# Samsung/iac

Hardware: AMD Instinct MI355X
Metric: Msamples/s rendered (3rd-order HOA->binaural, 48 kHz) (higher is better)
Workload: dtype f32

## Files before the change

iac_amd/__init__.py:

```python
from .hipabi import (
    FMT_F32,
    FMT_S16,
    FMT_S24,
    FMT_S32,
    KIND_DMX,
    KIND_FIR,
    KIND_H2M,
    KIND_M2M,
    PROJ_AUTO,
    PROJ_EXACT,
    PROJ_MFMA,
    SS,
    Batch,
    BatchConfig,
    DemixConfig,
    DemixFrame,
    DemixState,
    DmxFrame,
    DmxState,
    FANOUT_MAX,
    FanoutReport,
    RenderArgs,
    Resampler,
    StreamGains,
    StreamState,
    stream_gains,
    dmx_matrix,
    fir_matrix,
    IamfHipError,
    LpcmLayout,
    LpcmInput,
    Matrix,
    build,
    get_h2m_matrix,
    get_m2m_matrix,
    layout_channels,
    lib,
    lib_path,
    lpcm_unpack,
    render_fanout,
    render_fanout_lpcm,
    render_fanout_range,
    ROUTE,
    RouteRow,
    route_instances,
    route_instances_ext,
    route_reset,
    route_tally,
    route_tally_ext,
)
```

iac_amd/csrc/iamf_render.hip:

```cpp
#include <hip/hip_runtime.h>

#include <math.h>
#include <stdint.h>
#include <atomic>
#include <stdio.h>
#include <stdlib.h>
#include <string.h>

#include <new>
#include <type_traits>
#include <vector>

#include "../../include/iamf_hip.h"

#define IAMF_FFT_HOST_TABLES

#include "render_entry.hpp"

namespace {

#include "render_common.hpp"
#include "render_downmix.hpp"
#include "render_fir.hpp"
#include "render_fir16.hpp"
#include "render_fir_fft.hpp"
#include "render_fast.hpp"
#include "render_fir_launch.hpp"
#include "render_fanout.hpp"
#include "render_generic.hpp"
#include "render_nolim.hpp"
#include "render_wide.hpp"
#include "render_lfe.hpp"
#include "stream_state.hpp"

__global__ __launch_bounds__(256) void restride_kernel(const uint8_t *src, int64_t src_stream_stride, uint8_t *dst,
                                                       int64_t dst_stream_stride, int n, int ch, int sc, int bps, int stream0) {
  const int s = blockIdx.y + stream0;
  const int64_t p = (int64_t)blockIdx.x * 256 + threadIdx.x;
  const int64_t n_out = (int64_t)n * sc + (ch > sc ? ch - sc : 0);
  if (p >= n_out) return;
  const int c0 = (int)(p % sc);
  const int64_t i = p / sc;
  const uint8_t *from = nullptr;
  for (int k = (ch - 1 - c0) / sc; k >= 0 && ch > c0; --k) {
    const int64_t ii = i - k;
    if (ii >= 0 && ii < n) {
      from = src + (int64_t)s * src_stream_stride + (ii * ch + c0 + (int64_t)sc * k) * bps;
      break;
    }
  }
  if (!from && p >= (int64_t)n * sc) return;
  uint8_t *to = dst + (int64_t)s * dst_stream_stride + p * bps;
  for (int b = 0; b < bps; ++b) to[b] = from ? from[b] : 0;
}


#define HIPCHK(expr)                                                                   \
  do {                                                                                 \
    hipError_t _e = (expr);                                                            \
    if (_e != hipSuccess) {                                                            \
      fprintf(stderr, "iamf_hip: %s failed: %s (%s:%d)\n", #expr, hipGetErrorString(_e), \
              __FILE__, __LINE__);                                                     \
      return IAMF_HIP_ERR_DEVICE;                                                      \
    }                                                                                  \
  } while (0)

struct TableEntry {
  uint32_t kind, in_id, out_id;
  int32_t channels, lfe1, lfe2, m, n;
  uint32_t offset;
};

extern "C" const uint8_t _binary_rdr_tables_bin_start[];
extern "C" const uint8_t _binary_rdr_tables_bin_end[];
extern "C" const uint8_t _binary_rdr_tables_tv_bin_start[];
extern "C" const uint8_t _binary_rdr_tables_tv_bin_end[];

struct Tables {
  int n = 0;
  const TableEntry *ents = nullptr;
  const float *data = nullptr;
  bool ok = false;
  explicit Tables(bool tv) {
    const uint8_t *b = tv ? _binary_rdr_tables_tv_bin_start : _binary_rdr_tables_bin_start;
    const size_t sz = tv ? (size_t)(_binary_rdr_tables_tv_bin_end - _binary_rdr_tables_tv_bin_start)
                         : (size_t)(_binary_rdr_tables_bin_end - _binary_rdr_tables_bin_start);
    if (sz < 12 || memcmp(b, "IARDRTB1", 8) != 0) return;
    uint32_t cnt;
    memcpy(&cnt, b + 8, 4);
    n = (int)cnt;
    ents = reinterpret_cast<const TableEntry *>(b + 12);
    data = reinterpret_cast<const float *>(b + 12 + sizeof(TableEntry) * cnt);
    ok = true;
  }
};

const Tables &tables(bool tv) {
  static Tables t(false), t_tv(true);
  return tv ? t_tv : t;
}

int find_matrix(int kind, int in_id, int out_id, iamf_hip_matrix *out, bool tv = false) {
  const Tables &t = tables(tv);
  if (!t.ok || !out) return -1;
  for (int i = 0; i < t.n; ++i) {
    const TableEntry &e = t.ents[i];
    if ((int)e.kind == kind && (int)e.in_id == in_id && (int)e.out_id == out_id) {
      out->kind = kind;
      out->in_id = in_id;
      out->out_id = out_id;
      out->channels = e.channels;
      out->lfe1 = e.lfe1;
      out->lfe2 = e.lfe2;
      out->m = e.m;
      out->n = e.n;
      out->mat = t.data + e.offset;
      return 0;
    }
  }
  return -1;
}

float ease(float x) {
  if (1.0 < x) return 1.0f;
  if (x < 0) return 0.0f;
  return 1.0f - powf(x - 1, 2.0);
}

}

struct iamf_hip_batch {
  iamf_hip_batch_config cfg;
  int device = 0;
  hipEvent_t done = nullptr;
  bool rendered = false;
  int m = 0, n_feeds = 0;
  int32_t src_feed[kMaxOut];
  uint32_t nz_mask[6] = {0, 0, 0, 0, 0, 0};
  int sparse = 0;
  int32_t *d_src_feed = nullptr;
  float thr = 0.f;
  int n_atk = 0, n_end = 0;
  std::vector<int64_t> spos;
  std::vector<uint8_t> sflushed;
  bool any_rendered = false;
  bool lp_scale_ok = false;
  float *d_matrix = nullptr, *d_gains = nullptr, *d_ctab = nullptr, *d_ring_y = nullptr,
        *d_ring_pm = nullptr;
  LimState *d_lim = nullptr;
  std::vector<float> h_gains;
  bool has2 = false;
  int m2 = 0;
  float *d_matrix2 = nullptr, *d_gains2 = nullptr;
  int32_t *d_src_feed2 = nullptr, *d_dmx_tab = nullptr;
  bool dmx = false;
  int dmx_n_in = 0, dmx_n_out = 0;
  float *d_pre = nullptr;
  int pre_l = 0;
  std::vector<float> h_fm;
  float *d_matrix_pre = nullptr;
  uint32_t nz_mask_pre[6] = {0, 0, 0, 0, 0, 0};
  int sparse_pre = 0;
  bool demix = false;
  int demix_steps = 0, demix_skip = 0, demix_layout = 0, demix_gmask = 0, demix_w4 = 0;
  int32_t *d_demix_tab = nullptr;
  float *d_demix_ftab = nullptr;
  bool fir = false;
  int fir_taps = 0;
  float *d_fir_hist[2] = {nullptr, nullptr};
  void *d_fir_h16 = nullptr;
  float *d_fir_pq = nullptr, *d_fir_tw = nullptr;
  float *d_fir_zero = nullptr;
  float *d_fir_pre[2] = {nullptr, nullptr};
  size_t fir_pre_bytes = 0;
  float *d_fir_y = nullptr;
  size_t fir_y_floats = 0;
  float *d_lp_in = nullptr;
  size_t lp_in_floats = 0;
  float *d_fir_id = nullptr;
  int32_t *d_fir_id_feed = nullptr;
  float fir_inv_scale = 1.f;
  int fir_cur = 0;
  bool lfe = false;
  float lfe_a1 = 0.f, lfe_a2 = 0.f, lfe_a3 = 0.f, lfe_b1 = 0.f, lfe_b2 = 0.f;
  double lfe_div = 0.0;
  float *d_lfe_state = nullptr, *d_lfe_next = nullptr, *d_lfe_u = nullptr;
  bool lfe_shared = false;
  size_t lfe_u_floats = 0;
  uint8_t *d_nat = nullptr;
  size_t nat_bytes = 0;
  uint8_t *d_dump = nullptr;
};

namespace {

bool on_batch_device(const iamf_hip_batch *b) {
  int dev = -1;
  return hipGetDevice(&dev) == hipSuccess && dev == b->device;
}

int quiesce(iamf_hip_batch *b) {
  if (b->rendered) HIPCHK(hipEventSynchronize(b->done));
  return IAMF_HIP_OK;
}

int reset_state(iamf_hip_batch *b) {
  const int ns = b->cfg.n_streams;
  std::vector<LimState> init((size_t)ns);
  for (auto &l : init) {
    l.g = 1.0f;
    l.gs = -1.0f;
    l.ge = -1.0f;
    l.n = b->n_end;
  }
  HIPCHK(hipMemcpy(b->d_lim, init.data(), sizeof(LimState) * ns, hipMemcpyHostToDevice));
  HIPCHK(hipMemset(b->d_ring_y, 0, sizeof(float) * (size_t)ns * b->cfg.out_channels * kSave));
  HIPCHK(hipMemset(b->d_ring_pm, 0, sizeof(float) * (size_t)ns * kSave));
  if (b->fir) {
    const size_t hb = sizeof(float) * (size_t)ns * b->m * 256;
    HIPCHK(hipMemset(b->d_fir_hist[0], 0, hb));
    HIPCHK(hipMemset(b->d_fir_hist[1], 0, hb));
    for (float *q : b->d_fir_pre)
      if (q) HIPCHK(hipMemset(q, 0, b->fir_pre_bytes));
  }
  if (b->lfe && !b->lfe_shared) {
    HIPCHK(hipMemset(b->d_lfe_state, 0, sizeof(float) * 4 * (size_t)ns));
    HIPCHK(hipMemset(b->d_lfe_next, 0, sizeof(float) * 2 * (size_t)ns));
  }
  b->spos.assign((size_t)ns, 0);
  b->sflushed.assign((size_t)ns, 0);
  b->any_rendered = false;
  return IAMF_HIP_OK;
}

template <int M>
void launch_m(const RenderParams &p, dim3 grid, size_t lds_bytes, hipStream_t st) {
  hipLaunchKernelGGL(render_kernel<M>, grid, dim3(kChunk), lds_bytes, st, p);
}

template <int M>
void launch_nolim_m(const RenderParams &p, hipStream_t st) {
  const int bytes = p.out_format == IAMF_HIP_FMT_S16 ? 2 : (p.out_format == IAMF_HIP_FMT_S24 ? 3 : 4);
  dim3 grid((unsigned)p.n_launch, (unsigned)((p.total + kNlChunk - 1) / kNlChunk));
  hipLaunchKernelGGL(render_nolim_kernel<M>, grid, dim3(256), (size_t)kNlChunk * p.out_ch * bytes, st, p);
}

template <int M, int OC>
void launch_fast_mc(const RenderParams &p, bool mixing, dim3 grid, hipStream_t st) {
  const size_t lds = sizeof(float) * (size_t)fast_lds_floats(OC, M);
  if (mixing) launch_big_lds<&render_fast_kernel<M, OC, 0, false, true>, 80 * 1024>(grid, dim3(256), lds, st, p);
  else launch_big_lds<&render_fast_kernel<M, OC>, 80 * 1024>(grid, dim3(256), lds, st, p);
}
template <int M>
void launch_fast_m(const RenderParams &p, bool mixing, dim3 grid, hipStream_t st) {
  if (p.out_ch == 1) launch_fast_mc<M, 1>(p, mixing, grid, st);
  else launch_fast_mc<M, 2>(p, mixing, grid, st);
}

template <int M, int OC>
void launch_fast_down_mc(const RenderParams &p, dim3 grid, hipStream_t st) {
  const size_t lds = sizeof(float) * (size_t)fast_lds_floats(OC, M);
  launch_big_lds<&render_fast_kernel<M, OC, 0, true>, 80 * 1024>(grid, dim3(256), lds, st, p);
}

template <int M>
void launch_wide_m(const RenderParams &p, dim3 grid, hipStream_t st) {
  const size_t lds = sizeof(float) * (size_t)wide_lds_floats(p.out_ch, M);
  if (p.use_mfma) launch_big_lds<&render_wide_kernel<M, true>, 80 * 1024>(grid, dim3(256), lds, st, p);
  else launch_big_lds<&render_wide_kernel<M, false>, 80 * 1024>(grid, dim3(256), lds, st, p);
}

int launch(const RenderParams &p, int m, size_t lds_bytes, hipStream_t st) {
  const Route r = pick_route(p, m);
  const dim3 grid((unsigned)p.n_launch);
  bool launched = false;
  switch (r.family) {
    case Family::Refused: return r.err;
    case Family::Lpcm: launched = iamf_hip_fast_lpcm_launch(&p, m, r.variant, st); break;
    case Family::FirSplit: {
      if (!dispatch(FirHomeM{}, m, [&](auto M) { launch_fft_m<M.value>(p, st); }) && !iamf_hip_fir_m2b_launch_fft(&p, m, st))
        return IAMF_HIP_ERR_INTERNAL;
      HIPCHK(hipGetLastError());
      RenderParams q = p;
      q.in = p.fir_y;
      q.in_stream_stride = 2 * (int64_t)p.total;
      q.in_frame_stride = 2 * (int64_t)p.total;
      q.frame_size = p.total;
      q.matrix = p.fir_id_matrix;
      q.src_feed = p.fir_id_feed;
      q.n_feeds = 2;
      q.fir_taps = 0;
      q.fir_hist = q.fir_hist_next = nullptr;
      launch_fast_m<2>(q, false, grid, st);
      launched = true;
      break;
    }
    case Family::FirFused:
      launched = dispatch(FirHomeM{}, m, [&](auto M) { launch_fir_m<M.value>(p, r.variant, st); }) ||
                 iamf_hip_fir_m2b_launch(&p, m, r.variant, st);
      break;
    case Family::FastDown:
      launched = dispatch(FastDownMC{}, mc(m, p.out_ch), [&](auto V) { launch_fast_down_mc<mc_m(V.value), mc_c(V.value)>(p, grid, st); });
      break;
    case Family::Wide4Lfe: launched = iamf_hip_wide4_lfe_launch(&p, m, st); break;
    case Family::Wide4Mix: launched = iamf_hip_wide4_mix_launch(&p, m, st); break;
    case Family::Wide4:
    case Family::Wide4Demix:
    case Family::Wide4Down: launched = iamf_hip_wide4_launch(&p, m, st); break;
    case Family::Nolim: launched = dispatch(NolimM{}, m, [&](auto M) { launch_nolim_m<M.value>(p, st); }); break;
    case Family::Fast: launched = dispatch(FastM{}, m, [&](auto M) { launch_fast_m<M.value>(p, r.variant != 0, grid, st); }); break;
    case Family::Wide: launched = dispatch(WideM{}, m, [&](auto M) { launch_wide_m<M.value>(p, grid, st); }); break;
    case Family::Generic: launched = dispatch(GenericM{}, m, [&](auto M) { launch_m<M.value>(p, grid, lds_bytes, st); }); break;
  }
  if (!launched) return IAMF_HIP_ERR_INTERNAL;
  HIPCHK(hipGetLastError());
  const RouteKey k = route_key(r, p, m);
  iamf_hip_route_count(k.family, k.variant, k.m, k.c, k.k);
  if (r.family == Family::FirSplit) iamf_hip_route_count(IAMF_HIP_ROUTE_FAST, 0, 2, 2, 0);
  return IAMF_HIP_OK;
}

const int kLayoutCount[9] = {1, 2, 6, 8, 10, 8, 10, 12, 6};
const int kLayoutCh[9][12] = {
    {kChMono},
    {kChL2, kChR2},
    {kChL7, kChR7, kChC, kChLFE, kChSL5, kChSR5},
    {kChL7, kChR7, kChC, kChLFE, kChSL5, kChSR5, kChHL, kChHR},
    {kChL7, kChR7, kChC, kChLFE, kChSL5, kChSR5, kChHFL, kChHFR, kChHBL, kChHBR},
    {kChL7, kChR7, kChC, kChLFE, kChSL7, kChSR7, kChBL7, kChBR7},
    {kChL7, kChR7, kChC, kChLFE, kChSL7, kChSR7, kChBL7, kChBR7, kChHL, kChHR},
    {kChL7, kChR7, kChC, kChLFE, kChSL7, kChSR7, kChBL7, kChBR7, kChHFL, kChHFR, kChHBL, kChHBR},
    {kChL3, kChR3, kChC, kChLFE, kChTL, kChTR},
};
const int kLayoutSurround[9] = {1, 2, 5, 5, 5, 7, 7, 7, 3};
const int kLayoutTop[9] = {0, 0, 0, 2, 4, 0, 2, 4, 2};

struct LpcmIn {
  const uint8_t *raw;
  int64_t stream_stride, frame_stride;
  int32_t off[16];
};
constexpr int kNotFused = INT32_MIN;

int lfe_prepass(iamf_hip_batch *b, const float *d_in, int64_t in_stream_stride, int64_t in_frame_stride, int ltotal,
                hipStream_t st, int s0, int cnt, int *t4_out) {
  const int ns = b->cfg.n_streams, nb = (ns + 63) / 64, t4 = (ltotal + 3) / 4;
  const size_t need_u = (size_t)nb * t4 * 64 * 4;
  if (need_u > b->lfe_u_floats) {
    HIPCHK(hipStreamSynchronize(st));
    (void)hipFree(b->d_lfe_u);
    b->d_lfe_u = nullptr;
    b->lfe_u_floats = 0;
    HIPCHK(hipMalloc(&b->d_lfe_u, sizeof(float) * need_u));
    b->lfe_u_floats = need_u;
  }
  LfeParams lp;
  memset(&lp, 0, sizeof(lp));
  lp.in = d_in;
  lp.in_stream_stride = in_stream_stride;
  lp.in_frame_stride = in_frame_stride;
  lp.pre_matrix = b->d_pre;
  lp.pre_l = b->pre_l;
  lp.pre_m = b->m;
  lp.frame_size = b->cfg.frame_size;
  lp.n_streams = ns;
  lp.total = ltotal;
  lp.t4 = t4;
  lp.a1 = b->lfe_a1; lp.a2 = b->lfe_a2; lp.a3 = b->lfe_a3; lp.b1 = b->lfe_b1; lp.b2 = b->lfe_b2;
  lp.state = b->d_lfe_state;
  lp.state_next = b->d_lfe_next;
  lp.u_t = reinterpret_cast<float4 *>(b->d_lfe_u);
  lp.s_first = s0;
  lp.s_count = cnt;
  hipLaunchKernelGGL(lfe_ff_kernel, dim3((unsigned)((t4 + kLfeTileQ - 1) / kLfeTileQ), (unsigned)nb), dim3(256), 0, st, lp);
  hipLaunchKernelGGL(lfe_chain_kernel, dim3((unsigned)nb), dim3(64), 0, st, lp);
  HIPCHK(hipGetLastError());
  *t4_out = t4;
  return IAMF_HIP_OK;
}

struct PreparedCall {
  RenderParams p;
  iamf_hip_render_args a;
  int m_eff;
  size_t lds;
  bool restride;
  int sc, bps;
  int64_t pos;
  int total, s0, cnt;
};

int render_prepare(iamf_hip_batch *b, const iamf_hip_render_args &a, int total, int s0, int cnt, const LpcmIn *lp, PreparedCall &pc) {
  if (!on_batch_device(b)) return IAMF_HIP_ERR_INVALID_STATE;
  if (lp && (b->fir || b->lfe || b->d_pre || b->demix || b->dmx || b->has2 || a.d_element_ramp || a.d_element2_ramp ||
             a.d_output_ramp || !b->lp_scale_ok || getenv("IAMF_HIP_LPCM_UNFUSED")))
    return kNotFused;
  if (s0 < 0 || cnt <= 0 || s0 + cnt > b->cfg.n_streams) return IAMF_HIP_ERR_BAD_ARG;
  if (a.lfe_pre_samples < 0 || a.lfe_post_samples < 0 ||
      ((a.lfe_pre_samples || a.lfe_post_samples) &&
       (a.n_frames != 1 || (int64_t)a.lfe_pre_samples + total + a.lfe_post_samples > b->cfg.frame_size)))
    return IAMF_HIP_ERR_BAD_ARG;
  const int64_t pos = b->spos[(size_t)s0];
  for (int i = s0; i < s0 + cnt; ++i)
    if (b->spos[(size_t)i] != pos || b->sflushed[(size_t)i]) return IAMF_HIP_ERR_INVALID_STATE;
  const bool whole = s0 == 0 && cnt == b->cfg.n_streams;
  if (!whole && b->fir) return IAMF_HIP_ERR_UNIMPLEMENTED;
  RenderParams &p = pc.p;
  memset(&p, 0, sizeof(p));
  p.stream0 = s0;
  p.n_launch = cnt;
  p.in = a.d_in;
  p.in_stream_stride = a.in_stream_stride;
  p.in_frame_stride = a.in_frame_stride;
  p.pcm = static_cast<uint8_t *>(a.d_pcm);
  p.pcm_stream_stride = a.pcm_stream_stride_bytes;
  p.matrix = b->d_matrix;
  p.gains = b->d_gains;
  p.ctab = b->d_ctab;
  p.lim = b->d_lim;
  p.ring_y = b->d_ring_y;
  p.ring_pm = b->d_ring_pm;
  p.pos0 = pos;
  p.total = total;
  p.frame_size = b->cfg.frame_size;
  p.n_streams = b->cfg.n_streams;
  p.n_feeds = b->n_feeds;
  p.out_ch = b->cfg.out_channels;
  p.og_ch = (b->cfg.out_gain_channels > 0 && b->cfg.out_gain_channels < b->cfg.out_channels) ? b->cfg.out_gain_channels : b->cfg.out_channels;
  p.out_format = b->cfg.out_format;
  p.limiter_on = b->cfg.limiter_enable ? 1 : 0;
  p.loudness_on = b->cfg.loudness_enable ? 1 : 0;
  bool tolerance = false;
  {
    const int proj = b->cfg.projection;
    const char *env = getenv("IAMF_HIP_PROJECTION");
    bool mf = proj == IAMF_HIP_PROJ_MFMA || (proj == IAMF_HIP_PROJ_AUTO && b->cfg.matrix.kind == IAMF_HIP_KIND_H2M);
    if (env && !strcmp(env, "exact")) mf = false;
    if (env && !strcmp(env, "mfma")) mf = true;
    p.use_mfma = (mf && b->n_feeds <= 32) ? 1 : 0;
    tolerance = mf;
  }
  p.n_atk = b->n_atk;
  p.n_end = b->n_end;
  p.thr = b->thr;
  p.src_feed = b->d_src_feed;
  p.dump = b->d_dump;
  for (int g = 0; g < 6; ++g) p.nz_mask[g] = b->nz_mask[g];
  p.sparse = getenv("IAMF_HIP_DENSE") ? 0 : b->sparse;
  if (b->has2 && a.d_in2) {
    p.in2 = a.d_in2;
    p.in2_stream_stride = a.in2_stream_stride;
    p.in2_frame_stride = a.in2_frame_stride;
    p.matrix2 = b->d_matrix2;
    p.src_feed2 = b->d_src_feed2;
    p.gains2 = b->d_gains2;
    p.m2 = b->m2;
  }
  p.elem_ramp = a.d_element_ramp;
  p.elem2_ramp = a.d_element2_ramp;
  p.out_ramp = a.d_output_ramp;
  p.ramp_stream_stride = a.ramp_stream_stride;
  if (b->dmx) {
    p.dmx_on = 1;
    p.dmx_frames = a.d_in ? a.d_dmx_frames : nullptr;
    p.dmx_n_in = b->dmx_n_in;
    p.dmx_n_out = b->dmx_n_out;
    p.dmx_tab = b->d_dmx_tab;
    p.dmx_in_layout = b->cfg.matrix.in_id;
    p.dmx_out_layout = b->cfg.matrix.out_id;
  }
  int m_eff = b->m;
  if (b->d_pre && a.d_in) {
    const int l = b->pre_l;
    if (tolerance && b->d_matrix_pre && FastM::has(l) && !p.in2) {
      p.matrix = b->d_matrix_pre;
      for (int g = 0; g < 6; ++g) p.nz_mask[g] = b->nz_mask_pre[g];
      p.sparse = getenv("IAMF_HIP_DENSE") ? 0 : b->sparse_pre;
      m_eff = l;
    } else {
      p.pre_matrix = b->d_pre;
      p.pre_l = b->pre_l;
    }
  }
  if (b->demix && a.d_in) {
    p.demix_on = 1;
    p.demix_steps = b->demix_steps;
    p.demix_skip = b->demix_skip;
    p.demix_tab = b->d_demix_tab;
    p.demix_ftab = b->d_demix_ftab;
    p.demix_frames = a.d_demix_frames;
    p.demix_i0 = a.n_frames == 1 ? a.demix_sample0 : 0;
    p.demix_layout = b->demix_layout;
    p.demix_gmask = b->demix_gmask;
    p.demix_w4 = b->demix_w4;
  }
  if (lp) {
    p.lpcm = lp->raw;
    p.lpcm_stream_stride = lp->stream_stride;
    p.lpcm_frame_stride = lp->frame_stride;
    for (int m = 0; m < 16; ++m) p.lpcm_off[m] = lp->off[m];
    if (pick_route(p, m_eff).family != Family::Lpcm) return kNotFused;
  }
  if (b->fir) {
    p.fir_taps = b->fir_taps;
    p.fir_hist = b->d_fir_hist[b->fir_cur];
    p.fir_hist_next = b->d_fir_hist[b->fir_cur ^ 1];
    p.fir_h16 = b->d_fir_h16;
    p.fir_inv_scale = b->fir_inv_scale;
    p.fir_pq = b->d_fir_pq;
    p.fir_tw = b->d_fir_tw;
    p.fir_zero = b->d_fir_zero;
    p.fir_pre = b->d_fir_pre[b->fir_cur];
    p.fir_pre_next = b->d_fir_pre[b->fir_cur ^ 1];
    if (a.d_in && b->d_fir_pq && (b->cfg.frame_size & 63) == 0 && !getenv("IAMF_HIP_FIR_FUSED") && !getenv("IAMF_HIP_FIR_F16") &&
        !getenv("IAMF_HIP_FIR_F32")) {
      const size_t need = (size_t)b->cfg.n_streams * 2 * (size_t)total;
      if (need > b->fir_y_floats) {
        HIPCHK(hipStreamSynchronize(static_cast<hipStream_t>(a.stream)));
        (void)hipFree(b->d_fir_y);
        b->d_fir_y = nullptr;
        b->fir_y_floats = 0;
        HIPCHK(hipMalloc(&b->d_fir_y, sizeof(float) * need));
        b->fir_y_floats = need;
      }
      p.fir_y = b->d_fir_y;
      p.fir_id_matrix = b->d_fir_id;
      p.fir_id_feed = b->d_fir_id_feed;
    }
  }
  if (b->lfe && a.d_in && total > 0) {
    const int lpre = a.lfe_pre_samples, lpost = a.lfe_post_samples;
    int t4 = 0;
    const int rc = lfe_prepass(b, a.d_in - lpre, a.in_stream_stride, a.in_frame_stride, lpre + total + lpost,
                               static_cast<hipStream_t>(a.stream), s0, cnt, &t4);
    if (rc) return rc;
    p.lfe = b->d_lfe_u;
    p.lfe_t4 = t4;
    p.lfe_k0 = lpre;
    p.lfe_div = b->lfe_div;
    for (int c = 0; c < b->cfg.out_channels && c < 32; ++c)
      if (b->src_feed[c] == -2) p.lfe_mask |= 1 << c;
  }
  const size_t lds = sizeof(float) * ((size_t)(p.out_ch + 2) * kRing + 3 * kChunk + kHead + 4 +
                                      ((b->dmx || b->demix) ? (size_t)kChCount * kChunk : 0));
  const int sc = b->cfg.pcm_stride_channels;
  const bool restride = sc > 0 && sc != p.out_ch;
  const int bps = iamf_hip_format_bytes(p.out_format);
  if (restride) {
    const size_t per_stream = (size_t)(total > kDelay ? total : kDelay) * p.out_ch * bps;
    const size_t need = per_stream * (size_t)p.n_streams;
    if (need > b->nat_bytes) {
      HIPCHK(hipStreamSynchronize(static_cast<hipStream_t>(a.stream)));
      (void)hipFree(b->d_nat);
      b->d_nat = nullptr;
      b->nat_bytes = 0;
      HIPCHK(hipMalloc(&b->d_nat, need));
      b->nat_bytes = need;
    }
    p.pcm = b->d_nat;
    p.pcm_stream_stride = (int64_t)per_stream;
  }
  pc.a = a;
  pc.m_eff = m_eff;
  pc.lds = lds;
  pc.restride = restride;
  pc.sc = sc;
  pc.bps = bps;
  pc.pos = pos;
  pc.total = total;
  pc.s0 = s0;
  pc.cnt = cnt;
  return IAMF_HIP_OK;
}

int render_launch(const PreparedCall &pc) {
  return launch(pc.p, pc.m_eff, pc.lds, static_cast<hipStream_t>(pc.a.stream));
}

int render_commit(iamf_hip_batch *b, const PreparedCall &pc) {
  const RenderParams &p = pc.p;
  const iamf_hip_render_args &a = pc.a;
  const bool restride = pc.restride;
  const int sc = pc.sc, bps = pc.bps, total = pc.total, s0 = pc.s0, cnt = pc.cnt;
  const int64_t pos = pc.pos;
  if (b->fir && p.in) b->fir_cur ^= 1;
  const int64_t before = p.limiter_on ? (pos > kDelay ? pos - kDelay : 0) : pos;
  for (int i = s0; i < s0 + cnt; ++i) b->spos[(size_t)i] = pos + total;
  b->any_rendered = true;
  const int64_t after = p.limiter_on ? (pos + total > kDelay ? pos + total - kDelay : 0) : pos + total;
  const int n_emit = (int)(after - before);
  if (restride && n_emit > 0) {
    const int64_t n_out = (int64_t)n_emit * sc + (p.out_ch > sc ? p.out_ch - sc : 0);
    hipLaunchKernelGGL(restride_kernel, dim3((unsigned)((n_out + 255) / 256), (unsigned)cnt), dim3(256), 0,
                       static_cast<hipStream_t>(a.stream), b->d_nat, p.pcm_stream_stride,
                       static_cast<uint8_t *>(a.d_pcm), a.pcm_stream_stride_bytes, n_emit, p.out_ch, sc, bps, s0);
    HIPCHK(hipGetLastError());
  }
  HIPCHK(hipEventRecord(b->done, static_cast<hipStream_t>(a.stream)));
  b->rendered = true;
  return n_emit;
}

int render_call(iamf_hip_batch *b, const iamf_hip_render_args &a, int total, int s0, int cnt, const LpcmIn *lp = nullptr) {
  PreparedCall pc;
  int r = render_prepare(b, a, total, s0, cnt, lp, pc);
  if (r != IAMF_HIP_OK) return r;
  r = render_launch(pc);
  if (r != IAMF_HIP_OK) return r;
  return render_commit(b, pc);
}

void build_feed_map(const iamf_hip_matrix &mx, int out_channels, std::vector<float> &fm, int32_t *src_feed) {
  for (int i = 0; i < kMaxOut; ++i) src_feed[i] = -1;
  for (int i = 0; i < mx.n; ++i) {
    int d = i;
    if (mx.kind == IAMF_HIP_KIND_H2M && (mx.lfe1 >= 0 || mx.lfe2 >= 0)) {
      if (mx.lfe1 >= 0 && mx.lfe1 <= i) ++d;
      if (mx.lfe2 >= 0 && mx.lfe2 <= i) ++d;
    }
    if (d < out_channels) src_feed[d] = i;
  }
  if (mx.kind == IAMF_HIP_KIND_H2M) {
    if (mx.lfe1 >= 0 && mx.lfe1 < out_channels) src_feed[mx.lfe1] = -1;
    if (mx.lfe2 >= 0 && mx.lfe2 < out_channels) src_feed[mx.lfe2] = -1;
  }
  fm.assign((size_t)mx.m * mx.n, 0.f);
  for (int f = 0; f < mx.n; ++f)
    for (int k = 0; k < mx.m; ++k)
      fm[(size_t)f * mx.m + k] = mx.kind == IAMF_HIP_KIND_H2M ? mx.mat[f * mx.m + k] : mx.mat[k * mx.n + f];
}

}

extern "C" {

int iamf_hip_get_h2m_matrix(int order, int out_id, iamf_hip_matrix *out) {
  return find_matrix(IAMF_HIP_KIND_H2M, order, out_id, out);
}

int iamf_hip_get_m2m_matrix(int in_id, int out_id, iamf_hip_matrix *out) {
  return find_matrix(IAMF_HIP_KIND_M2M, in_id, out_id, out);
}

int iamf_hip_get_m2m_matrix_variant(int variant, int in_id, int out_id, iamf_hip_matrix *out) {
  if (variant != IAMF_HIP_VARIANT_DEFAULT && variant != IAMF_HIP_VARIANT_SAMSUNG_TV) return -1;
  return find_matrix(IAMF_HIP_KIND_M2M, in_id, out_id, out, variant == IAMF_HIP_VARIANT_SAMSUNG_TV);
}

int iamf_hip_layout_channels(int out_id) {
  switch (out_id) {
    case IAMF_HIP_SS_A: return 2;
    case IAMF_HIP_SS_B: return 6;
    case IAMF_HIP_SS_C: return 8;
    case IAMF_HIP_SS_D: return 10;
    case IAMF_HIP_SS_E: return 11;
    case IAMF_HIP_SS_F: return 12;
    case IAMF_HIP_SS_G: return 14;
    case IAMF_HIP_SS_H: return 24;
    case IAMF_HIP_SS_I: return 8;
    case IAMF_HIP_SS_J: return 12;
    case IAMF_HIP_L_712: return 10;
    case IAMF_HIP_L_312: return 6;
    case IAMF_HIP_L_MONO: return 1;
    case IAMF_HIP_L_BINAURAL: return 2;
    default: return 0;
  }
}

int iamf_hip_format_bytes(int f) {
  switch (f) {
    case IAMF_HIP_FMT_S16: return 2;
    case IAMF_HIP_FMT_S24: return 3;
    case IAMF_HIP_FMT_S32: return 4;
    case IAMF_HIP_FMT_F32: return 4;
    default: return 0;
  }
}

const char *iamf_hip_version(void) { return "iamf_hip 0.1 (gfx950, HIP)"; }

int iamf_hip_batch_create(const iamf_hip_batch_config *cfg, iamf_hip_batch **out) {
  if (!cfg || !out) return IAMF_HIP_ERR_BAD_ARG;
  *out = nullptr;
  iamf_hip_matrix mx = cfg->matrix;
  const bool dmx = mx.kind == IAMF_HIP_KIND_DMX;
  const bool fir = mx.kind == IAMF_HIP_KIND_FIR;
  if (fir && (cfg->fir_taps < 1 || cfg->fir_taps > 256 || mx.n != 2 || cfg->out_channels != 2 ||
              !cfg->limiter_enable ||
              (!FirHomeM::has(mx.m) && !FirM2bM::has(mx.m))))
    return IAMF_HIP_ERR_BAD_ARG;
  if (dmx) {
    if (!iamf_hip_dmx_valid(mx.in_id, mx.out_id)) return IAMF_HIP_ERR_BAD_ARG;
    mx.m = kLayoutCount[mx.in_id];
    mx.n = kLayoutCount[mx.out_id];
  }
  if (cfg->n_streams <= 0 || cfg->frame_size <= 0 || cfg->sample_rate <= 0 || (!dmx && !mx.mat) ||
      mx.m <= 0 || mx.m > kMaxIn || mx.n <= 0 || mx.n > kMaxOut || cfg->out_channels <= 0 ||
      cfg->out_channels > kMaxOut || !iamf_hip_format_bytes(cfg->out_format) || cfg->projection < 0 ||
      cfg->projection > IAMF_HIP_PROJ_MFMA || (dmx && cfg->out_channels != mx.n) || cfg->pcm_stride_channels < 0 || cfg->out_gain_channels < 0 ||
      cfg->pcm_stride_channels > 64)
    return IAMF_HIP_ERR_BAD_ARG;
  int ndev = 0;
  HIPCHK(hipGetDeviceCount(&ndev));
  if (ndev <= 0) return IAMF_HIP_ERR_DEVICE;

  iamf_hip_batch *b = new (std::nothrow) iamf_hip_batch();
  if (!b) return IAMF_HIP_ERR_ALLOC_FAIL;
  b->cfg = *cfg;
  if (hipGetDevice(&b->device) != hipSuccess) {
    delete b;
    return IAMF_HIP_ERR_DEVICE;
  }
  b->m = mx.m;
  b->n_feeds = mx.n;
  b->dmx = dmx;

  b->fir = fir;
  b->fir_taps = fir ? cfg->fir_taps : 0;
  std::vector<float> fm(1, 0.f);
  int32_t dmx_tab[24];
  memset(dmx_tab, 0, sizeof(dmx_tab));
  if (dmx) {
    for (int i = 0; i < kMaxOut; ++i) b->src_feed[i] = -1;
    b->dmx_n_in = mx.m;
    b->dmx_n_out = mx.n;
    for (int i = 0; i < mx.m; ++i) dmx_tab[i] = kLayoutCh[mx.in_id][i];
    for (int i = 0; i < mx.n; ++i) dmx_tab[12 + i] = kLayoutCh[mx.out_id][i];
  } else if (fir) {
    for (int i = 0; i < kMaxOut; ++i) b->src_feed[i] = -1;
    fm.assign(mx.mat, mx.mat + (size_t)2 * mx.m * cfg->fir_taps);
  } else {
    build_feed_map(mx, cfg->out_channels, fm, b->src_feed);
    b->lp_scale_ok = true;
    for (float w : fm)
      if (w != 0.f && !(fabsf(w) >= 0x1p-100f && fabsf(w) <= 0x1p100f)) b->lp_scale_ok = false;
    if (cfg->lfe_hoa && mx.kind == IAMF_HIP_KIND_H2M && (mx.lfe1 >= 0 || mx.lfe2 >= 0)) {
      const float sample_rate = (float)cfg->sample_rate, cutoff_freq = 120;
      const float delta_time = 1 / sample_rate + 1.0e-10;
      const float c = 1.0f / (float)tanf(M_PI * cutoff_freq * delta_time);
      b->lfe = true;
      b->lfe_a1 = 1.0f / (1.0f + c + c * c);
      b->lfe_a2 = 2.0f * b->lfe_a1;
      b->lfe_a3 = b->lfe_a1;
      b->lfe_b1 = 2.0f * (1.0f - c * c) * b->lfe_a1;
      b->lfe_b2 = (1.0f - c + c * c) * b->lfe_a1;
      b->lfe_div = mx.n <= 2 ? 0.0 : sqrt((double)mx.n);
      if (mx.lfe1 >= 0 && mx.lfe1 < cfg->out_channels) b->src_feed[mx.lfe1] = -2;
      if (mx.lfe2 >= 0 && mx.lfe2 < cfg->out_channels) b->src_feed[mx.lfe2] = -2;
    }
    int set = 0, all = 0;
    for (int g = 0; g < 6 && 4 * g < cfg->out_channels; ++g)
      for (int k = 0; k < mx.m && k < 32; ++k) {
        bool nz = false;
        for (int c = 4 * g; c < 4 * g + 4 && c < cfg->out_channels; ++c)
          if (b->src_feed[c] >= 0 && fm[(size_t)b->src_feed[c] * mx.m + k] != 0.f) nz = true;
        ++all;
        if (nz) {
          ++set;
          b->nz_mask[g] |= 1u << k;
        }
      }
    b->sparse = 2 * set < all ? 1 : 0;
    b->h_fm = fm;
  }

  const float atk = 0.001f, rel = 0.200f;
  b->thr = (float)pow(10, cfg->limiter_threshold_db / 20);
  const float inc = (float)1 / (float)cfg->sample_rate;
  std::vector<float> T;
  T.push_back(0.0f);
  while (T.back() < rel + atk && T.size() < (1u << 22)) T.push_back(T.back() + inc);
  b->n_end = (int)T.size() - 1;
  b->n_atk = 0;
  while (b->n_atk < b->n_end && T[b->n_atk] < atk) ++b->n_atk;
  std::vector<float> ctab((size_t)b->n_end + 1, 1.0f);
  for (int k = 1; k <= b->n_end; ++k)
    ctab[k] = (k - 1) < b->n_atk ? ease(T[k] / atk) : ease((T[k] - atk) / rel);

  const int ns = cfg->n_streams;
  b->h_gains.assign((size_t)3 * ns, 1.0f);
#define CREATE_CHK(expr)                       \
  do {                                         \
    if ((expr) != hipSuccess) {                \
      iamf_hip_batch_destroy(b);               \
      return IAMF_HIP_ERR_DEVICE;              \
    }                                          \
  } while (0)
  CREATE_CHK(hipEventCreateWithFlags(&b->done, hipEventDisableTiming));
  CREATE_CHK(hipMalloc(&b->d_matrix, sizeof(float) * fm.size()));
  CREATE_CHK(hipMalloc(&b->d_gains, sizeof(float) * 3 * ns));
  CREATE_CHK(hipMalloc(&b->d_ctab, sizeof(float) * ctab.size()));
  CREATE_CHK(hipMalloc(&b->d_lim, sizeof(LimState) * ns));
  CREATE_CHK(hipMalloc(&b->d_ring_y, sizeof(float) * (size_t)ns * cfg->out_channels * kSave));
  CREATE_CHK(hipMalloc(&b->d_ring_pm, sizeof(float) * (size_t)ns * kSave));
  if (b->lfe) {
    CREATE_CHK(hipMalloc(&b->d_lfe_state, sizeof(float) * 4 * (size_t)ns));
    CREATE_CHK(hipMalloc(&b->d_lfe_next, sizeof(float) * 2 * (size_t)ns));
  }
  CREATE_CHK(hipMalloc(&b->d_dump, (size_t)ns * 256 * 16));
  CREATE_CHK(hipMalloc(&b->d_src_feed, sizeof(int32_t) * kMaxOut));
  CREATE_CHK(hipMemcpy(b->d_src_feed, b->src_feed, sizeof(int32_t) * kMaxOut, hipMemcpyHostToDevice));
  if (fir) {
    const size_t hb = sizeof(float) * (size_t)ns * mx.m * 256;
    CREATE_CHK(hipMalloc(&b->d_fir_hist[0], hb));
    CREATE_CHK(hipMalloc(&b->d_fir_hist[1], hb));
    CREATE_CHK(hipMemset(b->d_fir_hist[0], 0, hb));
    CREATE_CHK(hipMemset(b->d_fir_hist[1], 0, hb));
    const int taps = cfg->fir_taps;
    float hmax = 0.f;
    for (size_t i = 0; i < (size_t)2 * mx.m * taps; ++i) hmax = fmaxf(hmax, fabsf(mx.mat[i]));
    if (hmax > 0.f && hmax < 1e30f) {
      int e = 0;
      (void)frexpf(hmax, &e);
      const float scale = ldexpf(1.f, 14 - e);
      std::vector<_Float16> tab((size_t)mx.m * 2 * 2 * 8 * kF16Taps, (_Float16)0.f);
      for (int ch = 0; ch < mx.m; ++ch)
        for (int ear = 0; ear < 2; ++ear)
          for (int r = 0; r < 8; ++r)
            for (int n = 0; n < kF16Taps; ++n) {
              const int k = n + r - 15;
              if (k < 0 || k >= taps) continue;
              const float v = mx.mat[((size_t)ear * mx.m + ch) * taps + k] * scale;
              const _Float16 hi = (_Float16)v;
              const _Float16 lo = (_Float16)((v - (float)hi) * 2048.f);
              const size_t at = ((((size_t)ch * 2 + ear) * 2 + 0) * 8 + r) * kF16Taps + n;
              tab[at] = hi;
              tab[at + (size_t)8 * kF16Taps] = lo;
            }
      CREATE_CHK(hipMalloc(&b->d_fir_h16, tab.size() * sizeof(_Float16)));
      CREATE_CHK(hipMemcpy(b->d_fir_h16, tab.data(), tab.size() * sizeof(_Float16), hipMemcpyHostToDevice));
      b->fir_inv_scale = 1.f / (scale * kF16InScale);
    }
    {
      std::vector<float> pq, tw;
      fft_build_tables(mx.mat, mx.m, taps, pq, tw);
      CREATE_CHK(hipMalloc(&b->d_fir_pq, pq.size() * sizeof(float)));
      CREATE_CHK(hipMemcpy(b->d_fir_pq, pq.data(), pq.size() * sizeof(float), hipMemcpyHostToDevice));
      CREATE_CHK(hipMalloc(&b->d_fir_tw, tw.size() * sizeof(float)));
      CREATE_CHK(hipMemcpy(b->d_fir_tw, tw.data(), tw.size() * sizeof(float), hipMemcpyHostToDevice));
      const size_t zf = (size_t)(mx.m > 0 ? mx.m : 1) * (size_t)(cfg->frame_size > 64 ? cfg->frame_size : 64);
      CREATE_CHK(hipMalloc(&b->d_fir_zero, zf * sizeof(float)));
      CREATE_CHK(hipMemset(b->d_fir_zero, 0, zf * sizeof(float)));
      if (cfg->frame_size >= 1024 && cfg->frame_size % 256 == 0 && mx.m % 2 == 0) {
        const int g = cfg->frame_size / 256;
        b->fir_pre_bytes = sizeof(float) * (size_t)((ns + g - 1) / g) * mx.m * cfg->frame_size;
        for (float *&q : b->d_fir_pre) {
          CREATE_CHK(hipMalloc(&q, b->fir_pre_bytes));
          CREATE_CHK(hipMemset(q, 0, b->fir_pre_bytes));
        }
      }
      const float id[4] = {1.f, 0.f, 0.f, 1.f};
      int32_t idf[kMaxOut];
      for (int i = 0; i < kMaxOut; ++i) idf[i] = i < 2 ? i : -1;
      CREATE_CHK(hipMalloc(&b->d_fir_id, sizeof(id)));
      CREATE_CHK(hipMemcpy(b->d_fir_id, id, sizeof(id), hipMemcpyHostToDevice));
      CREATE_CHK(hipMalloc(&b->d_fir_id_feed, sizeof(idf)));
      CREATE_CHK(hipMemcpy(b->d_fir_id_feed, idf, sizeof(idf), hipMemcpyHostToDevice));
    }
  }
  CREATE_CHK(hipMalloc(&b->d_dmx_tab, sizeof(dmx_tab)));
  CREATE_CHK(hipMemcpy(b->d_dmx_tab, dmx_tab, sizeof(dmx_tab), hipMemcpyHostToDevice));
  CREATE_CHK(hipMemcpy(b->d_matrix, fm.data(), sizeof(float) * fm.size(), hipMemcpyHostToDevice));
  CREATE_CHK(hipMemcpy(b->d_gains, b->h_gains.data(), sizeof(float) * 3 * ns, hipMemcpyHostToDevice));
  CREATE_CHK(hipMemcpy(b->d_ctab, ctab.data(), sizeof(float) * ctab.size(), hipMemcpyHostToDevice));
#undef CREATE_CHK
  const int r = reset_state(b);
  if (r != IAMF_HIP_OK) {
    iamf_hip_batch_destroy(b);
    return r;
  }
  *out = b;
  return IAMF_HIP_OK;
}

void iamf_hip_batch_destroy(iamf_hip_batch *b) {
  if (!b) return;
  int cur = -1;
  const bool sw = hipGetDevice(&cur) == hipSuccess && cur != b->device && hipSetDevice(b->device) == hipSuccess;
  struct Restore {
    bool on;
    int dev;
    ~Restore() {
      if (on) (void)hipSetDevice(dev);
    }
  } restore{sw, cur};
  if (b->rendered) (void)hipEventSynchronize(b->done);
  if (b->done) (void)hipEventDestroy(b->done);
  (void)hipFree(b->d_matrix_pre);
  (void)hipFree(b->d_matrix);
  (void)hipFree(b->d_gains);
  (void)hipFree(b->d_ctab);
  (void)hipFree(b->d_lim);
  (void)hipFree(b->d_ring_y);
  (void)hipFree(b->d_ring_pm);
  (void)hipFree(b->d_src_feed);
  (void)hipFree(b->d_dmx_tab);
  (void)hipFree(b->d_pre);
  (void)hipFree(b->d_demix_tab);
  (void)hipFree(b->d_demix_ftab);
  (void)hipFree(b->d_fir_hist[0]);
  (void)hipFree(b->d_fir_hist[1]);
  (void)hipFree(b->d_fir_h16);
  (void)hipFree(b->d_fir_pq);
  (void)hipFree(b->d_fir_tw);
  (void)hipFree(b->d_fir_zero);
  (void)hipFree(b->d_fir_pre[0]);
  (void)hipFree(b->d_fir_pre[1]);
  (void)hipFree(b->d_fir_y);
  (void)hipFree(b->d_lp_in);
  (void)hipFree(b->d_fir_id);
  (void)hipFree(b->d_fir_id_feed);
  if (!b->lfe_shared) {
    (void)hipFree(b->d_lfe_state);
    (void)hipFree(b->d_lfe_next);
  }
  (void)hipFree(b->d_lfe_u);
  (void)hipFree(b->d_nat);
  (void)hipFree(b->d_dump);
  (void)hipFree(b->d_matrix2);
  (void)hipFree(b->d_gains2);
  (void)hipFree(b->d_src_feed2);
  delete b;
}

int iamf_hip_batch_set_gains(iamf_hip_batch *b, const float *eg, const float *og, const float *lg) {
  if (!b) return IAMF_HIP_ERR_BAD_ARG;
  if (!on_batch_device(b)) return IAMF_HIP_ERR_INVALID_STATE;
  {
    const int q = quiesce(b);
    if (q != IAMF_HIP_OK) return q;
  }
  const int ns = b->cfg.n_streams;
  const float *rows[3] = {eg, og, lg};
  for (int k = 0; k < 3; ++k) {
    if (!rows[k]) continue;
    memcpy(&b->h_gains[(size_t)k * ns], rows[k], sizeof(float) * ns);
    HIPCHK(hipMemcpy(b->d_gains + (size_t)k * ns, rows[k], sizeof(float) * ns, hipMemcpyHostToDevice));
  }
  return IAMF_HIP_OK;
}

static int range_args_check(const iamf_hip_batch *b, const iamf_hip_render_args *a, int32_t stream0, int32_t n_streams, int64_t *total_out) {
  *total_out = 0;
  if (!b || !a || !a->d_in || !a->d_pcm || a->n_frames < 0) return IAMF_HIP_ERR_BAD_ARG;
  if (stream0 < 0 || n_streams <= 0 || stream0 + n_streams > b->cfg.n_streams) return IAMF_HIP_ERR_BAD_ARG;
  if (a->n_frames == 0) return IAMF_HIP_OK;
  if (b->has2 && !a->d_in2) return IAMF_HIP_ERR_BAD_ARG;
  if (b->dmx && !a->d_dmx_frames) return IAMF_HIP_ERR_BAD_ARG;
  if (b->demix && a->d_in && (!a->d_demix_frames || a->demix_sample0 < 0 ||
                              a->demix_sample0 + (a->n_samples ? a->n_samples : 1) > b->cfg.frame_size))
    return IAMF_HIP_ERR_BAD_ARG;
  if ((a->d_element_ramp || a->d_element2_ramp || a->d_output_ramp) &&
      a->ramp_stream_stride < (int64_t)a->n_frames * b->cfg.frame_size && b->cfg.n_streams > 1)
    return IAMF_HIP_ERR_BAD_ARG;
  int64_t total = (int64_t)a->n_frames * b->cfg.frame_size;
  if (a->n_samples > 0) {
    if (a->n_frames != 1 || a->n_samples > b->cfg.frame_size) return IAMF_HIP_ERR_BAD_ARG;
    total = a->n_samples;
  }
  if (total > INT32_MAX) return IAMF_HIP_ERR_BAD_ARG;
  const int sc = b->cfg.pcm_stride_channels > 0 ? b->cfg.pcm_stride_channels : b->cfg.out_channels;
  const int64_t need = (total * sc + (b->cfg.out_channels > sc ? b->cfg.out_channels - sc : 0)) *
                       iamf_hip_format_bytes(b->cfg.out_format);
  if (b->cfg.n_streams > 1 && a->pcm_stream_stride_bytes < need) return IAMF_HIP_ERR_BUFFER_TOO_SMALL;
  *total_out = total;
  return IAMF_HIP_OK;
}

static int render_range_impl(iamf_hip_batch *b, const iamf_hip_render_args *a, int32_t stream0, int32_t n_streams, const LpcmIn *lp) {
  int64_t total = 0;
  const int rc = range_args_check(b, a, stream0, n_streams, &total);
  if (rc != IAMF_HIP_OK || total == 0) return rc;
  return render_call(b, *a, (int)total, stream0, n_streams, lp);
}

int iamf_hip_batch_render_range(iamf_hip_batch *b, const iamf_hip_render_args *a, int32_t stream0, int32_t n_streams) {
  return render_range_impl(b, a, stream0, n_streams, nullptr);
}

int iamf_hip_batch_render_lpcm(iamf_hip_batch *b, const iamf_hip_lpcm_input *in, const iamf_hip_render_args *args) {
  if (!b) return IAMF_HIP_ERR_BAD_ARG;
  return iamf_hip_batch_render_lpcm_range(b, in, args, 0, b->cfg.n_streams);
}

static int lpcm_form_check(const iamf_hip_batch *b, const iamf_hip_lpcm_input *in, int nf, int n_samples, bool *fusable_out,
                           int *first_out, int *count_out) {
  const iamf_hip_lpcm_layout &L = in->layout;
  const int fs = b->cfg.frame_size, ch = b->d_pre ? b->pre_l : b->m;
  if (L.sample_bytes < 2 || L.sample_bytes > 4 || L.channels != ch || ch > IAMF_HIP_LPCM_MAX_CHANNELS || L.frame_size != fs ||
      (fs & 3) || in->raw_frame_stride <= 0 || in->raw_stream_stride < (int64_t)nf * in->raw_frame_stride)
    return IAMF_HIP_ERR_BAD_ARG;
  const int first = in->first_sample, count = n_samples > 0 ? n_samples : fs;
  if (first < 0 || (first > 0 && (nf != 1 || n_samples <= 0)) || first + count > fs) return IAMF_HIP_ERR_BAD_ARG;
  bool fusable = L.sample_bytes == 2 && L.little_endian && ch <= 16 && (in->raw_frame_stride & 7) == 0 &&
                 (in->raw_stream_stride & 7) == 0 && (reinterpret_cast<uintptr_t>(in->d_raw) & 15) == 0;
  for (int c = 0; c < ch; ++c) {
    if (L.src_offset[c] < 0) {
      fusable = false;
      continue;
    }
    if (L.src_step[c] < L.sample_bytes ||
        (int64_t)L.src_offset[c] + (int64_t)(fs - 1) * L.src_step[c] + L.sample_bytes > in->raw_frame_stride)
      return IAMF_HIP_ERR_BAD_ARG;
    if (L.src_step[c] != 2 || ((L.src_offset[c] + 2 * first) & 7)) fusable = false;
  }
  *fusable_out = fusable;
  *first_out = first;
  *count_out = count;
  return IAMF_HIP_OK;
}

static void lpcm_in_of(const iamf_hip_lpcm_input *in, int ch, int first, LpcmIn &lp) {
  memset(&lp, 0, sizeof(lp));
  lp.raw = static_cast<const uint8_t *>(in->d_raw);
  lp.stream_stride = in->raw_stream_stride;
  lp.frame_stride = in->raw_frame_stride;
  for (int c = 0; c < ch; ++c) lp.off[c] = in->layout.src_offset[c] + 2 * first;
}

static int lpcm_unpack_range(iamf_hip_batch *b, const iamf_hip_lpcm_input *in, int nf, int first, int count, int32_t stream0,
                             int32_t n_streams, hipStream_t st, iamf_hip_render_args &a) {
  const iamf_hip_lpcm_layout &L = in->layout;
  const int fs = b->cfg.frame_size, ch = b->d_pre ? b->pre_l : b->m, ns = b->cfg.n_streams;
  const size_t need = (size_t)ns * nf * ch * fs;
  if (need > b->lp_in_floats) {
    const int q = quiesce(b);
    if (q != IAMF_HIP_OK) return q;
    HIPCHK(hipStreamSynchronize(st));
    (void)hipFree(b->d_lp_in);
    b->d_lp_in = nullptr;
    b->lp_in_floats = 0;
    HIPCHK(hipMalloc(&b->d_lp_in, sizeof(float) * need));
    HIPCHK(hipMemset(b->d_lp_in, 0, sizeof(float) * need));
    b->lp_in_floats = need;
  }
  const int fmax = 65535 / n_streams > 0 ? 65535 / n_streams : 0;
  if (fmax == 0) return IAMF_HIP_ERR_UNIMPLEMENTED;
  const int64_t lp_stream_stride = (int64_t)nf * ch * fs;
  for (int f = 0; f < nf; f += fmax) {
    const int r = iamf_hip_lpcm_unpack_frames(
        &L, static_cast<const uint8_t *>(in->d_raw) + (int64_t)stream0 * in->raw_stream_stride + (int64_t)f * in->raw_frame_stride,
        in->raw_stream_stride, in->raw_frame_stride, nf - f < fmax ? nf - f : fmax, nullptr, 0,
        b->d_lp_in + (int64_t)stream0 * lp_stream_stride + (size_t)f * ch * fs, lp_stream_stride, (int64_t)ch * fs, n_streams, st, first,
        count);
    if (r != IAMF_HIP_OK) return r;
  }
  a.d_in = b->d_lp_in;
  a.in_stream_stride = lp_stream_stride;
  a.in_frame_stride = (int64_t)ch * fs;
  return IAMF_HIP_OK;
}

int iamf_hip_batch_render_lpcm_range(iamf_hip_batch *b, const iamf_hip_lpcm_input *in, const iamf_hip_render_args *args,
                                     int32_t stream0, int32_t n_streams) {
  if (!b || !in || !args || !in->d_raw || args->d_in || !args->d_pcm || args->n_frames < 0) return IAMF_HIP_ERR_BAD_ARG;
  if (stream0 < 0 || n_streams <= 0 || stream0 + n_streams > b->cfg.n_streams) return IAMF_HIP_ERR_BAD_ARG;
  if (!on_batch_device(b)) return IAMF_HIP_ERR_INVALID_STATE;
  if (args->n_frames == 0) return 0;
  const int ch = b->d_pre ? b->pre_l : b->m, nf = args->n_frames;
  bool fusable = false;
  int first = 0, count = 0;
  const int fc = lpcm_form_check(b, in, nf, args->n_samples, &fusable, &first, &count);
  if (fc != IAMF_HIP_OK) return fc;
  iamf_hip_render_args a = *args;
  if (fusable) {
    LpcmIn lp;
    lpcm_in_of(in, ch, first, lp);
    a.d_in = reinterpret_cast<const float *>(in->d_raw);
    a.in_stream_stride = a.in_frame_stride = 0;
    const int r = render_range_impl(b, &a, stream0, n_streams, &lp);
    if (r != kNotFused) return r;
  }
  {
    a.d_in = reinterpret_cast<const float *>(in->d_raw);
    int64_t total = 0;
    const int rc = range_args_check(b, &a, stream0, n_streams, &total);
    if (rc != IAMF_HIP_OK || total == 0) return rc;
  }
  const int ur = lpcm_unpack_range(b, in, nf, first, count, stream0, n_streams, static_cast<hipStream_t>(args->stream), a);
  if (ur != IAMF_HIP_OK) return ur;
  return render_range_impl(b, &a, stream0, n_streams, nullptr);
}

int iamf_hip_batch_render_ex(iamf_hip_batch *b, const iamf_hip_render_args *a) {
  if (!b) return IAMF_HIP_ERR_BAD_ARG;
  return iamf_hip_batch_render_range(b, a, 0, b->cfg.n_streams);
}

int iamf_hip_batch_render(iamf_hip_batch *b, const float *d_in, int64_t in_stream_stride,
                          int64_t in_frame_stride, int32_t n_frames, void *d_pcm,
                          int64_t pcm_stream_stride_bytes, void *stream) {
  iamf_hip_render_args a;
  memset(&a, 0, sizeof(a));
  a.d_in = d_in;
  a.in_stream_stride = in_stream_stride;
  a.in_frame_stride = in_frame_stride;
  a.n_frames = n_frames;
  a.d_pcm = d_pcm;
  a.pcm_stream_stride_bytes = pcm_stream_stride_bytes;
  a.stream = stream;
  if (b && (b->has2 || b->dmx || b->demix)) return IAMF_HIP_ERR_BAD_ARG;
  return iamf_hip_batch_render_ex(b, &a);
}

static const int kFanFuseMax = IAMF_HIP_FANOUT_MAX;


static bool fan_members_distinct(iamf_hip_batch *const *batches, void *const *d_pcm, int n_batches) {
  for (int j = 0; j < n_batches; ++j) {
    if (!batches[j] || !d_pcm[j]) return false;
    for (int i = 0; i < j; ++i)
      if (batches[i] == batches[j]) return false;
  }
  return true;
}

static bool fan_member_like(const iamf_hip_batch *b, const iamf_hip_batch *b0) {
  return b->cfg.n_streams == b0->cfg.n_streams && b->cfg.frame_size == b0->cfg.frame_size && b->m == b0->m &&
         (b->d_pre ? b->pre_l : b->m) == (b0->d_pre ? b0->pre_l : b0->m) && !(b->has2 || b->dmx || b->demix);
}

static int fan_state_check(iamf_hip_batch *const *batches, int n_batches, int stream0, int n_streams) {
  const iamf_hip_batch *b0 = batches[0];
  for (int j = 0; j < n_batches; ++j) {
    const iamf_hip_batch *b = batches[j];
    for (int i = stream0; i < stream0 + n_streams; ++i)
      if (b->spos[(size_t)i] != b0->spos[(size_t)stream0] || b->sflushed[(size_t)i]) return IAMF_HIP_ERR_INVALID_STATE;
  }
  if (stream0 != 0 || n_streams != b0->cfg.n_streams)
    for (int j = 0; j < n_batches; ++j)
      if (batches[j]->fir) return IAMF_HIP_ERR_UNIMPLEMENTED;
  return IAMF_HIP_OK;
}

static FanMember fan_member_of(const RenderParams &p) {
  FanMember mb;
  mb.pcm = p.pcm;
  mb.pcm_stream_stride = p.pcm_stream_stride;
  mb.matrix = p.matrix;
  mb.gains = p.gains;
  mb.ctab = p.ctab;
  mb.lim = p.lim;
  mb.ring_y = p.ring_y;
  mb.ring_pm = p.ring_pm;
  mb.src_feed = p.src_feed;
  mb.out_ch = p.out_ch;
  mb.out_format = p.out_format;
  mb.loudness_on = p.loudness_on;
  mb.n_atk = p.n_atk;
  mb.n_end = p.n_end;
  mb.thr = p.thr;
  return mb;
}

static int fanout_range_impl(iamf_hip_batch *const *batches, int32_t n_batches, const float *d_in, int64_t in_stream_stride,
                             int64_t in_frame_stride, int32_t n_frames, int32_t n_samples, void *const *d_pcm,
                             const int64_t *pcm_stream_stride_bytes, void *stream, int32_t *n_emitted, int32_t *n_fused,
                             bool whole, int32_t stream0, int32_t n_streams) {
  if (n_batches < 1 || n_batches > IAMF_HIP_FANOUT_MAX) return IAMF_HIP_ERR_BAD_ARG;
  if (!batches || !d_in || !d_pcm || !pcm_stream_stride_bytes || !n_emitted) return IAMF_HIP_ERR_BAD_ARG;
  if (!whole && (stream0 < 0 || n_streams <= 0)) return IAMF_HIP_ERR_BAD_ARG;
  if (!fan_members_distinct(batches, d_pcm, n_batches)) return IAMF_HIP_ERR_BAD_ARG;
  iamf_hip_render_args args[IAMF_HIP_FANOUT_MAX];
  int64_t total = 0;
  const iamf_hip_batch *b0 = batches[0];
  if (whole) stream0 = 0, n_streams = b0->cfg.n_streams;
  for (int j = 0; j < n_batches; ++j) {
    const iamf_hip_batch *b = batches[j];
    if (!fan_member_like(b, b0)) return IAMF_HIP_ERR_BAD_ARG;
    iamf_hip_render_args &a = args[j];
    memset(&a, 0, sizeof(a));
    a.d_in = d_in;
    a.in_stream_stride = in_stream_stride;
    a.in_frame_stride = in_frame_stride;
    a.n_frames = n_frames;
    a.n_samples = n_samples;
    a.d_pcm = d_pcm[j];
    a.pcm_stream_stride_bytes = pcm_stream_stride_bytes[j];
    a.stream = stream;
    int64_t tj = 0;
    const int rc = range_args_check(b, &a, stream0, n_streams, &tj);
    if (rc != IAMF_HIP_OK) return rc;
    total = tj;
  }
  if (total == 0) {
    if (n_fused) *n_fused = 0;
    for (int j = 0; j < n_batches; ++j) n_emitted[j] = 0;
    return IAMF_HIP_OK;
  }
  for (int j = 0; j < n_batches; ++j)
// ... 768 lines not shown
```

iac_amd/csrc/iamf_render_fir_m2b.hip:

```cpp
#include <hip/hip_runtime.h>

#include <stdint.h>
#include <atomic>
#include <stdlib.h>
#include <string.h>

#include <type_traits>

#include "../../include/iamf_hip.h"
#include "render_entry.hpp"

namespace {

#include "render_common.hpp"
#include "render_downmix.hpp"
#include "render_fir.hpp"
#include "render_fir16.hpp"
#include "render_fir_fft.hpp"
#include "render_fast.hpp"
#include "render_fir_launch.hpp"

}

int iamf_hip_fir_m2b_launch_fft(const void *params, int m, hipStream_t st) {
  RenderParams p;
  memcpy(&p, params, sizeof(p));
  return dispatch(FirM2bM{}, m, [&](auto M) { launch_fft_m<M.value>(p, st); });
}

int iamf_hip_fir_m2b_launch(const void *params, int m, int stage, hipStream_t st) {
  RenderParams p;
  memcpy(&p, params, sizeof(p));
  return dispatch(FirM2bM{}, m, [&](auto M) { launch_fir_m<M.value>(p, stage, st); });
}
```

iac_amd/csrc/iamf_route.hip:

```cpp
#include <hip/hip_runtime.h>

#include <stdint.h>
#include <stdlib.h>
#include <string.h>

#include <algorithm>
#include <atomic>
#include <type_traits>

#include "../../include/iamf_hip.h"
#include "render_entry.hpp"

namespace {

#include "render_params.hpp"
#include "render_route.hpp"
#include "resample_route.hpp"

constexpr int kRouteCap = 1024;

constexpr uint32_t pack_key(int family, int variant, int m, int c, int k) {
  return (uint32_t)family << 24 | (uint32_t)variant << 20 | (uint32_t)m << 12 | (uint32_t)c << 4 | (uint32_t)k;
}

struct RouteTable {
  iamf_hip_route_row rows[kRouteCap];
  uint32_t key[kRouteCap];
  int32_t index[kRouteCap];
  int n = 0, dropped = 0;
  explicit RouteTable(bool ext) {
    const auto add = [&](int family, int variant, int m, int c, int k) {
      if (n == kRouteCap) {
        ++dropped;
        return;
      }
      iamf_hip_route_row &r = rows[n];
      memset(&r, 0, sizeof(r));
      r.family = family;
      r.variant = variant;
      r.m = m;
      r.c = c;
      r.k = k;
      key[n] = pack_key(family, variant, m, c, k);
      index[n] = n;
      ++n;
    };
    if (ext) {
      for_each_render_instance_ext(add);
    } else {
      for_each_render_instance(add);
      for_each_resample_instance(add);
    }
    int32_t order[kRouteCap];
    for (int i = 0; i < n; ++i) order[i] = i;
    std::sort(order, order + n, [&](int a, int b) { return key[a] < key[b]; });
    uint32_t sorted[kRouteCap];
    for (int i = 0; i < n; ++i) sorted[i] = key[order[i]];
    memcpy(key, sorted, sizeof(uint32_t) * n);
    memcpy(index, order, sizeof(int32_t) * n);
  }
  int find(uint32_t k) const {
    const uint32_t *e = key + n, *p = std::lower_bound(key, e, k);
    return (p != e && *p == k) ? index[p - key] : kRouteCap;
  }
};

const RouteTable &route_table() {
  static const RouteTable t(false);
  return t;
}

const RouteTable &route_table_ext() {
  static const RouteTable t(true);
  return t;
}

std::atomic<int64_t> g_launches[kRouteCap + 1];
std::atomic<int64_t> g_launches_ext[kRouteCap + 1];

int list_instances(const RouteTable &t, iamf_hip_route_row *rows, int cap) {
  for (int i = 0; rows && i < t.n && i < cap; ++i) rows[i] = t.rows[i];
  return t.n + t.dropped;
}

int tally_of(const RouteTable &t, std::atomic<int64_t> *launches, iamf_hip_route_row *rows, int cap, int reset) {
  int cnt = 0;
  for (int i = 0; i <= kRouteCap; ++i) {
    if (i >= t.n && i != kRouteCap) continue;
    const int64_t v = reset ? launches[i].exchange(0, std::memory_order_relaxed) : launches[i].load(std::memory_order_relaxed);
    if (v == 0) continue;
    if (rows && cnt < cap) {
      if (i < t.n) rows[cnt] = t.rows[i];
      else memset(&rows[cnt], 0, sizeof(rows[cnt]));
      rows[cnt].launches = v;
    }
    ++cnt;
  }
  return cnt;
}

}

void iamf_hip_route_count(int family, int variant, int m, int c, int k) {
  g_launches[route_table().find(pack_key(family, variant, m, c, k))].fetch_add(1, std::memory_order_relaxed);
}

void iamf_hip_route_count_ext(int family, int variant, int m, int c, int k) {
  g_launches_ext[route_table_ext().find(pack_key(family, variant, m, c, k))].fetch_add(1, std::memory_order_relaxed);
}

extern "C" {

int iamf_hip_route_instances(iamf_hip_route_row *rows, int cap) { return list_instances(route_table(), rows, cap); }

int iamf_hip_route_tally(iamf_hip_route_row *rows, int cap, int reset) {
  return tally_of(route_table(), g_launches, rows, cap, reset);
}

int iamf_hip_route_instances_ext(iamf_hip_route_row *rows, int cap) { return list_instances(route_table_ext(), rows, cap); }

int iamf_hip_route_tally_ext(iamf_hip_route_row *rows, int cap, int reset) {
  return tally_of(route_table_ext(), g_launches_ext, rows, cap, reset);
}

}
```

iac_amd/csrc/render_entry.hpp:

```cpp
#pragma once

#define IAMF_INTERNAL extern "C" __attribute__((visibility("hidden")))

IAMF_INTERNAL int iamf_hip_wide4_launch(const void *params, int m, hipStream_t st);
IAMF_INTERNAL int iamf_hip_wide4_mix_launch(const void *params, int m, hipStream_t st);
IAMF_INTERNAL int iamf_hip_wide4_lfe_launch(const void *params, int m, hipStream_t st);
IAMF_INTERNAL int iamf_hip_fanout_launch(const void *params, int m, int k, hipStream_t st);
IAMF_INTERNAL int iamf_hip_fanout_lp_launch(const void *params, int m, int k, hipStream_t st);
IAMF_INTERNAL int iamf_hip_fast_lpcm_launch(const void *params, int m, int early, hipStream_t st);
IAMF_INTERNAL int iamf_hip_fir_m2b_launch(const void *params, int m, int stage, hipStream_t st);
IAMF_INTERNAL int iamf_hip_fir_m2b_launch_fft(const void *params, int m, hipStream_t st);
IAMF_INTERNAL int iamf_hip_lpcm_unpack_frames(const iamf_hip_lpcm_layout *lay, const void *d_raw, int64_t raw_stream_stride,
                                              int64_t raw_frame_stride, int32_t n_frames, const int32_t *d_first_count,
                                              int64_t first_count_stride, float *d_out, int64_t out_stream_stride,
                                              int64_t out_frame_stride, int32_t n_streams, void *stream, int32_t uniform_first,
                                              int32_t uniform_count);
IAMF_INTERNAL void iamf_hip_route_count(int family, int variant, int m, int c, int k);
IAMF_INTERNAL void iamf_hip_route_count_ext(int family, int variant, int m, int c, int k);
```

iac_amd/csrc/render_fir_fft.hpp:

```cpp
#pragma once

#ifndef FFT_HD
#define FFT_HD __host__ __device__ __forceinline__
#endif

#ifndef IAMF_FFT_NT
#define IAMF_FFT_NT 1
#endif
#ifndef IAMF_FFT_X2_LDS
#define IAMF_FFT_X2_LDS 0
#endif
constexpr int kFftN = 1024;
constexpr int kFftHop = 768;
constexpr int kFftHops = 4;
constexpr int kFftSpan = kFftHop * kFftHops;
constexpr int kFftRow = 68;
constexpr int kFftScratch = 16 * kFftRow;

typedef float fft_c32 __attribute__((ext_vector_type(2)));

FFT_HD fft_c32 fft_mk(float re, float im) {
  fft_c32 r;
  r.x = re;
  r.y = im;
// ... 297 lines not shown
        const int e = (n * k) & (kFftN - 1);
        ar += hl * cr[e] - hr * ci[e];
        ai += hl * ci[e] + hr * cr[e];
      }
      gr[(size_t)c * kFftN + k] = ar;
      gi[(size_t)c * kFftN + k] = ai;
    }
  pq.assign((size_t)pairs * 16 * 64 * 4, 0.f);
  for (int p = 0; p < pairs; ++p) {
    const int a = 2 * p, b = 2 * p + 1;
    auto G = [&](int c, int k, double &re, double &im) {
      re = c < m ? gr[(size_t)c * kFftN + k] : 0.0;
      im = c < m ? gi[(size_t)c * kFftN + k] : 0.0;
    };
    for (int r = 0; r < 16; ++r)
      for (int lane = 0; lane < 64; ++lane) {
        const int k = fft_bin(lane, r), km = (kFftN - k) & (kFftN - 1);
        double ar, ai, br, bi;
        G(a, k, ar, ai);
        G(b, k, br, bi);
        const double pr = 0.5 * (ar + bi), pi = 0.5 * (ai - br);
        G(a, km, ar, ai);
        G(b, km, br, bi);
        const double qr = 0.5 * (ar - bi), qi = -0.5 * (ai + br);
        float *o = &pq[(((size_t)p * 16 + r) * 64 + lane) * 4];
        o[0] = (float)(pr / kFftN);
        o[1] = (float)(pi / kFftN);
        o[2] = (float)(qr / kFftN);
        o[3] = (float)(qi / kFftN);
      }
  }
  tw.assign((size_t)(16 * 64 + 16 * 4) * 2, 0.f);
  for (int k1 = 0; k1 < 16; ++k1)
    for (int lane = 0; lane < 64; ++lane) {
      const int e = (lane * k1) & (kFftN - 1);
      tw[((size_t)k1 * 64 + lane) * 2 + 0] = (float)cr[e];
      tw[((size_t)k1 * 64 + lane) * 2 + 1] = (float)ci[e];
    }
  for (int k2 = 0; k2 < 16; ++k2)
    for (int n3 = 0; n3 < 4; ++n3) {
      const int e = (16 * n3 * k2) & (kFftN - 1);
      tw[((size_t)16 * 64 + k2 * 4 + n3) * 2 + 0] = (float)cr[e];
      tw[((size_t)16 * 64 + k2 * 4 + n3) * 2 + 1] = (float)ci[e];
    }
  return pairs;
}
#endif

#if defined(__HIPCC__)
#ifndef IAMF_FFT_EXP
#define IAMF_FFT_EXP 0
#endif
constexpr int kFftLdsFloats = kFftHops * kFftScratch * 2 + (16 * 64 + 16 * 4) * 2;

constexpr int kFftTwFloats = (16 * 64 + 16 * 4) * 2;
struct FftTwiddles {
  const fft_c32 *tw1;
  const fft_c32 *tw2;
};
__device__ __forceinline__ void fft_load_twiddles(const float *tw, int t, float *tw_lds, FftTwiddles &o) {
  const fft_c32 *g = reinterpret_cast<const fft_c32 *>(tw);
  fft_c32 *l = reinterpret_cast<fft_c32 *>(tw_lds);
  for (int i = t; i < 16 * 64 + 16 * 4; i += 256) l[i] = g[i];
  o.tw1 = l + (t & 63);
  o.tw2 = l + 16 * 64 + (t & 3);
}

__device__ __forceinline__ void fft_wave_sync() {
  __builtin_amdgcn_fence(__ATOMIC_ACQ_REL, "wavefront");
  __builtin_amdgcn_wave_barrier();
}

template <int M, int N1A = 0, int N1B = 16>
__device__ __forceinline__ void fft_fetch(int pr, fft_c32 (&z)[16], unsigned ra_lo, unsigned ra_hi, unsigned zmask,
                                          unsigned hmask, unsigned cs_in, uint64_t a_zero, unsigned lo) {
  const int a = 2 * pr, b = 2 * pr + 1;
#pragma unroll
  for (int n1 = N1A; n1 < N1B; ++n1) {
    const uint64_t r0 = ((uint64_t)(unsigned)__builtin_amdgcn_readlane((int)ra_hi, n1) << 32) |
                        (unsigned)__builtin_amdgcn_readlane((int)ra_lo, n1);
    const uint64_t cs = ((zmask >> n1) & 1u) ? 0u : (((hmask >> n1) & 1u) ? 4u * kFirHist : cs_in);
    typedef const float __attribute__((address_space(1))) *gptr;
    const gptr sa = (gptr)(r0 + (uint64_t)a * cs);
    const gptr sb = (gptr)(b < M ? r0 + (uint64_t)b * cs : a_zero);
    float va, vb;
    if (IAMF_FFT_NT && n1 >= 4 && n1 < 12) {
      va = __builtin_nontemporal_load(sa + lo);
      vb = __builtin_nontemporal_load(sb + lo);
    } else {
      va = sa[lo];
      vb = sb[lo];
    }
    z[n1] = fft_mk(va, vb);
  }
}
__device__ __forceinline__ void fft_touch(fft_c32 (&z)[16]) {
  asm volatile(""
               : "+v"(z[0]), "+v"(z[1]), "+v"(z[2]), "+v"(z[3]), "+v"(z[4]), "+v"(z[5]), "+v"(z[6]), "+v"(z[7]), "+v"(z[8]),
                 "+v"(z[9]), "+v"(z[10]), "+v"(z[11]), "+v"(z[12]), "+v"(z[13]), "+v"(z[14]), "+v"(z[15]));
}

__device__ __forceinline__ const float *fft_y_ptr(const float *scratch_all, int e, int m) {
  const int hop = m / kFftHop;
  return scratch_all + hop * (kFftScratch * 2) + e * kFftHop + (m - hop * kFftHop);
}

template <int M, int N1A, int N1B>
__device__ __forceinline__ void fft_fetch2(int pr, fft_c32 (&z)[16], uint64_t base1, uint64_t base2p, int kseg, unsigned cs4,
                                           unsigned lo4) {
  typedef const char __attribute__((address_space(1))) *gbptr;
  typedef const float __attribute__((address_space(1))) *gptr;
  int k = kseg;
  asm volatile("" : "+s"(k));
  const unsigned oa = lo4 + (unsigned)(2 * pr) * cs4, ob = oa + cs4;
#pragma unroll
  for (int n1 = N1A; n1 < N1B; ++n1) {
    const gbptr base = (gbptr)(n1 < k ? base1 : base2p);
    const gptr sa = (gptr)(base + 256 * n1 + oa), sb = (gptr)(base + 256 * n1 + ob);
    float va, vb;
    if (IAMF_FFT_NT && n1 >= 4 && n1 < 12) {
      va = __builtin_nontemporal_load(sa);
      vb = __builtin_nontemporal_load(sb);
    } else {
      va = *sa;
      vb = *sb;
    }
    z[n1] = fft_mk(va, vb);
  }
}
template <int M, bool FAST2 = false>
__device__ __forceinline__ void fir_stage_fft(const RenderParams &p, const float *in_s, const float *hist, int c0,
                                              fft_c32 *scratch_all, const FftTwiddles &tw, float *gy = nullptr,
                                              const float *pre = nullptr) {
  const int t = threadIdx.x, lane = t & 63, lane_ = lane;
  const int w = __builtin_amdgcn_readfirstlane(t >> 6);
  const int b0 = c0 + kFftHop * w;
  if (b0 >= p.total) return;
  if (IAMF_FFT_EXP == 4) return;
  fft_c32 *S = scratch_all + w * kFftScratch;
  constexpr int kPairs = (M + 1) / 2;
  unsigned ra_lo, ra_hi, zmask, hmask;
  const uint64_t a_zero = reinterpret_cast<uint64_t>(p.fir_zero);
  {
    const int fs = p.frame_size;
    const int n1 = lane & 15;
    const int n = b0 - (kFftN - kFftHop) + 64 * n1;
    const int nn = n < 0 ? 0 : n;
    const int f = nn / fs, i = nn - f * fs;
    uint64_t ad = reinterpret_cast<uint64_t>(in_s) + 4 * (uint64_t)((int64_t)f * p.in_frame_stride + i);
    unsigned cs = 4u * (unsigned)fs;
    if (n < 0) {
      ad = reinterpret_cast<uint64_t>(hist) + 4 * (uint64_t)(kFirHist + n);
      cs = 4u * kFirHist;
    } else if (n >= p.total) {
      ad = a_zero;
      cs = 0;
    }
    ra_lo = (unsigned)ad;
    ra_hi = (unsigned)(ad >> 32);
    hmask = (unsigned)__builtin_amdgcn_readfirstlane((int)(unsigned)(__ballot(n < 0) & 0xffffu));
    zmask = (unsigned)__builtin_amdgcn_readfirstlane((int)(unsigned)(__ballot(n >= 0 && n >= p.total) & 0xffffu));
    (void)cs;
  }
  const unsigned cs_in = 4u * (unsigned)p.frame_size;
  const unsigned lo = (unsigned)lane;
  uint64_t base1 = 0, base2p = 0;
  int kseg = 16;
  if constexpr (FAST2) {
    const int fs = p.frame_size;
    const int n0 = b0 - (kFftN - kFftHop);
    int64_t nb = 0;
    if (n0 < 0) {
      base1 = reinterpret_cast<uint64_t>(pre);
    } else {
      const int f0 = n0 / fs, i0 = n0 - f0 * fs;
      base1 = reinterpret_cast<uint64_t>(in_s + (int64_t)f0 * p.in_frame_stride + i0);
      nb = (int64_t)(f0 + 1) * fs;
    }
    kseg = (int)((nb - n0) >> 6);
    const uint64_t b2 = nb >= p.total ? a_zero : reinterpret_cast<uint64_t>(in_s + (nb / fs) * p.in_frame_stride);
    base2p = b2 - 256ull * (uint64_t)kseg;
    base1 = ((uint64_t)(unsigned)__builtin_amdgcn_readfirstlane((int)(base1 >> 32)) << 32) | (unsigned)__builtin_amdgcn_readfirstlane((int)base1);
    base2p = ((uint64_t)(unsigned)__builtin_amdgcn_readfirstlane((int)(base2p >> 32)) << 32) | (unsigned)__builtin_amdgcn_readfirstlane((int)base2p);
    kseg = __builtin_amdgcn_readfirstlane(kseg);
  }
  const unsigned lo4 = 4u * lo;
#define FFT_FETCH(pr, z)                                                          \
  do {                                                                            \
    if constexpr (FAST2) fft_fetch2<M, 0, 16>(pr, z, base1, base2p, kseg, cs_in, lo4); \
    else fft_fetch<M>(pr, z, ra_lo, ra_hi, zmask, hmask, cs_in, a_zero, lo);      \
  } while (0)
#define FFT_FETCH_HALF(pr, z, A, B)                                               \
  do {                                                                            \
    if constexpr (FAST2) fft_fetch2<M, A, B>(pr, z, base1, base2p, kseg, cs_in, lo4); \
    else fft_fetch<M, A, B>(pr, z, ra_lo, ra_hi, zmask, hmask, cs_in, a_zero, lo); \
  } while (0)
  fft_c32 u[16], v[16], z[16];
#pragma unroll
  for (int r = 0; r < 16; ++r) u[r] = v[r] = fft_mk(0.f, 0.f);
  const float4 *pq = reinterpret_cast<const float4 *>(p.fir_pq);
  fft_c32 zb[16];
  auto pair_step = [&](int pr, fft_c32 (&za)[16]) {
    int lane = lane_;
    asm volatile("" : "+v"(lane));
    const fft_c32 *tw1 = tw.tw1 - lane_ + lane, *tw2 = tw.tw2 - (lane_ & 3) + (lane & 3);
    const float4 *tq = pq + pr * 16 * 64;
    float4 c[8];
#pragma unroll
    for (int r = 0; r < 8; ++r) c[r] = IAMF_FFT_EXP == 1 ? make_float4(0.5f, 0.25f, 0.125f, 0.0625f) : (tq + r * 64)[lo];
    fft_pin();
    fft_fwd_a_tab(za, tw1);
    if (IAMF_FFT_EXP != 3) {
      fft_x1_write(za, lane, S);
      fft_wave_sync();
      fft_x1_read(za, lane, S);
    }
    fft_fwd_b_tab(za, tw2);
    if (IAMF_FFT_EXP != 3) {
#if IAMF_FFT_X2_LDS
      fft_wave_sync();
      fft_x2_write(za, lane, S);
      fft_wave_sync();
      fft_x2_read(za, lane, S);
      fft_wave_sync();
#else
      fft_wave_sync();
      fft_x2_quads(za);
#endif
    }
    fft_fwd_c(za);
#pragma unroll
    for (int r = 0; r < 8; ++r) {
      u[r] = fft_cmac(u[r], za[r], fft_mk(c[r].x, c[r].y));
      v[r] = fft_cmac(v[r], za[r], fft_mk(c[r].z, c[r].w));
      c[r] = IAMF_FFT_EXP == 1 ? make_float4(0.5f, 0.25f, 0.125f, 0.0625f) : (tq + (8 + r) * 64)[lo];
    }
    fft_pin();
    const int prn = pr + 2 < kPairs ? pr + 2 : kPairs - 1;
    if (IAMF_FFT_EXP != 2) FFT_FETCH_HALF(prn, za, 0, 8);
    fft_pin();
#pragma unroll
    for (int r = 0; r < 8; ++r) {
      u[8 + r] = fft_cmac(u[8 + r], za[8 + r], fft_mk(c[r].x, c[r].y));
      v[8 + r] = fft_cmac(v[8 + r], za[8 + r], fft_mk(c[r].z, c[r].w));
    }
    fft_pin();
    if (IAMF_FFT_EXP != 2) FFT_FETCH_HALF(prn, za, 8, 16);
    fft_pin();
  };
  FFT_FETCH(0, z);
  FFT_FETCH(kPairs > 1 ? 1 : 0, zb);
  fft_touch(z);
  fft_touch(zb);
#pragma unroll 1
  for (int pr = 0; pr + 1 < kPairs; pr += 2) {
    pair_step(pr, z);
    pair_step(pr + 1, zb);
  }
  if constexpr (kPairs & 1) pair_step(kPairs - 1, z);
  fft_mirror_write(v, lane, S);
  fft_wave_sync();
  fft_mirror_read_add(u, lane, S);
  fft_wave_sync();
  fft_inv_c(u);
#if IAMF_FFT_X2_LDS
  fft_x2_write_back(u, lane, S);
  fft_wave_sync();
  fft_x2_read_back(u, lane, S);
#else
  fft_x2_quads(u);
#endif
  fft_inv_b_tab(u, tw.tw2);
  fft_wave_sync();
  fft_x1_write_back(u, lane, S);
  fft_wave_sync();
  fft_x1_read_back(u, lane, S);
  fft_inv_a_tab(u, tw.tw1);
  fft_wave_sync();
  if (gy) {
#pragma unroll
    for (int n1 = 4; n1 < 16; ++n1) {
      const int m = b0 + 64 * (n1 - 4);
      if (m < p.total) {
        __builtin_nontemporal_store(u[n1].x, gy + m + lane);
        __builtin_nontemporal_store(u[n1].y, gy + p.total + m + lane);
      }
    }
  } else {
    float *y = reinterpret_cast<float *>(S);
#pragma unroll
    for (int n1 = 4; n1 < 16; ++n1) {
      y[64 * (n1 - 4) + lane] = u[n1].x;
      y[kFftHop + 64 * (n1 - 4) + lane] = u[n1].y;
    }
  }
#undef FFT_FETCH
#undef FFT_FETCH_HALF
}

#ifndef IAMF_FFT_OCC
#define IAMF_FFT_OCC 2
#endif
template <int M, bool FAST2 = false>
__global__ __launch_bounds__(256, IAMF_FFT_OCC) void fir_fft_kernel(const RenderParams p, float *gy, int64_t gy_stream_stride) {
  extern __shared__ float fft_lds[];
  const int s = blockIdx.y + p.stream0, t = threadIdx.x;
  FftTwiddles tw;
  fft_load_twiddles(p.fir_tw, t, fft_lds + kFftHops * kFftScratch * 2, tw);
  __syncthreads();
  const float *in_s = p.in + (int64_t)s * p.in_stream_stride;
  const float *hist = p.fir_hist + (int64_t)s * M * kFirHist;
  const bool has_pre = p.fir_pre_next != nullptr;
  const int g256 = has_pre ? p.frame_size >> 8 : 1;
  const int64_t pre_off = has_pre ? ((int64_t)(s / g256) * M) * p.frame_size + (int64_t)(s % g256) * kFirHist : 0;
  fir_stage_fft<M, FAST2>(p, in_s, hist, kFftSpan * (int)blockIdx.x, reinterpret_cast<fft_c32 *>(fft_lds), tw,
                          gy + (int64_t)s * gy_stream_stride, FAST2 ? p.fir_pre + pre_off : nullptr);
  if (blockIdx.x == 0) {
    float *hn = p.fir_hist_next + (int64_t)s * M * kFirHist;
    for (int ch = 0; ch < M; ++ch) {
      const float x = fir_input(p, in_s, hist, ch, p.total - kFirHist + t);
      hn[ch * kFirHist + t] = x;
      if (has_pre) p.fir_pre_next[pre_off + (int64_t)ch * p.frame_size + t] = x;
    }
  }
}
#endif
```

iac_amd/csrc/render_fir_launch.hpp:

```cpp
#pragma once

template <int M>
void launch_fir_m(const RenderParams &p, int stage, hipStream_t st) {
  const dim3 grid((unsigned)p.n_launch);
  if (stage == 3) {
    static_assert(fast_lds_floats(2, M, 3) * 4 <= 80 * 1024, "two workgroups per CU");
    launch_big_lds<&render_fast_kernel<M, 2, 3>, 120 * 1024>(grid, dim3(256), sizeof(float) * (size_t)fast_lds_floats(2, M, 3), st, p);
  } else if (stage == 2) {
    static_assert(fast_lds_floats(2, M, 2) * 4 <= 80 * 1024, "two workgroups per CU");
    launch_big_lds<&render_fast_kernel<M, 2, 2>, 120 * 1024>(grid, dim3(256), sizeof(float) * (size_t)fast_lds_floats(2, M, 2), st, p);
  } else {
    launch_big_lds<&render_fast_kernel<M, 2, 1>, 120 * 1024>(grid, dim3(512), sizeof(float) * (size_t)fast_lds_floats(2, M, 1), st, p);
  }
}

template <int M>
void launch_fft_m(const RenderParams &p, hipStream_t st) {
  const dim3 g((unsigned)((p.total + kFftSpan - 1) / kFftSpan), (unsigned)p.n_launch);
  if ((M & 1) == 0 && p.fir_pre && p.fir_pre_next && p.total % p.frame_size == 0 && !getenv("IAMF_HIP_FIR_GENERAL_FETCH"))
    hipLaunchKernelGGL((fir_fft_kernel<M, (M & 1) == 0>), g, dim3(256), sizeof(float) * (size_t)kFftLdsFloats, st, p, p.fir_y, 2 * (int64_t)p.total);
  else
    hipLaunchKernelGGL((fir_fft_kernel<M, false>), g, dim3(256), sizeof(float) * (size_t)kFftLdsFloats, st, p, p.fir_y, 2 * (int64_t)p.total);
}
```

iac_amd/csrc/render_route.hpp:

```cpp
#pragma once

#ifdef __HIPCC__
#define IAMF_HD __host__ __device__
#else
#define IAMF_HD
#endif


#include "instance_lists.hpp"

using GenericM = Ints<1, 2, 4, 6, 8, 9, 10, 11, 12, 14, 16, 24>;
using NolimM = GenericM;
using FastM = Ints<1, 2, 4, 6, 8, 9, 10, 12, 14, 16, 24>;
using FastOC = Ints<1, 2>;
using WideM = FastM;
using FastDownMC = Ints<mc(8, 2), mc(8, 1), mc(6, 2), mc(6, 1), mc(2, 1)>;
using Wide4M = Ints<4, 6, 8, 9, 10, 12, 16>;
using Wide4C = Ints<6, 8, 10, 12, 14, 24>;
using Wide4DemixM = Ints<6, 8, 10, 12>;
using Wide4DemixC = Ints<6, 8, 10, 12, 24>;
using Wide4DownMC = Ints<mc(12, 10), mc(12, 8), mc(12, 6), mc(10, 8), mc(10, 6), mc(8, 6)>;
using Wide4MixC = Ints<6, 8, 10, 12>;
using Wide4LfeM = Ints<4, 9, 16>;
using FanM = Ints<4, 6, 8, 9, 12, 16>;
using FanK = Ints<2, 3, 4>;
using LpcmM = Ints<1, 4, 9, 16>;
using LpcmOC = Ints<1, 2>;
using FanLpM = Ints<4, 9, 16>;
using FanLpK = Ints<2, 3, 4>;
using FirHomeM = Ints<1, 4, 9, 16>;
using FirM2bM = Ints<2, 6, 8, 10, 12>;


constexpr int kFWin = 1088;
constexpr int kFIn2 = 4;

constexpr int kWChunk = 256;
constexpr int kWPos = 512;
constexpr int kWWin = 320;

IAMF_HD constexpr int wide_lds_floats(int c, int m) {
  return kWPos * c + 2 * kWPos + kWPos / 16 + 3 * kWChunk + 2 * kWWin + ((c + 3) & ~3) * m + 16;
}

constexpr int kNlChunk = 1024;
constexpr int kNlMaxFrameBytes = 60;

inline bool nolim_shape_ok(const RenderParams &p) {
  const int bytes = p.out_format == IAMF_HIP_FMT_S16 ? 2 : (p.out_format == IAMF_HIP_FMT_S24 ? 3 : 4);
  if ((p.frame_size & 3) || (p.total & 3) || p.total <= 0) return false;
  if ((reinterpret_cast<uintptr_t>(p.in) & 15) || (p.in_stream_stride & 3) || (p.in_frame_stride & 3)) return false;
  if ((reinterpret_cast<uintptr_t>(p.pcm) & 15) || (p.pcm_stream_stride & 15)) return false;
  if (((p.out_ch * bytes) & 3) || p.out_ch * bytes > kNlMaxFrameBytes) return false;
  return true;
}

inline int fir_stage_choice(const RenderParams &p) {
  if (getenv("IAMF_HIP_FIR_F32")) return 1;
  if (getenv("IAMF_HIP_FIR_F16") && p.fir_h16) return 2;
  if (p.fir_pq && p.fir_tw && p.fir_zero && (p.frame_size & 63) == 0)
    return (p.fir_y && p.fir_id_matrix && !getenv("IAMF_HIP_FIR_FUSED")) ? 4 : 3;
  return p.fir_h16 ? 2 : 1;
}


inline bool fast_shape_ok(const RenderParams &p, bool force_generic) {
  if (force_generic || p.og_ch < p.out_ch) return false;
  if (!p.limiter_on || !p.in || p.out_ch > 2 || p.n_end < kFWin) return false;
  if (p.pre_matrix || p.demix_on) return false;
  if (p.elem_ramp || p.elem2_ramp || p.out_ramp) {
    if (p.dmx_on || p.fir_taps > 0 || (p.ramp_stream_stride & 3) || (p.elem2_ramp && !p.in2)) return false;
    if ((reinterpret_cast<uintptr_t>(p.elem_ramp) | reinterpret_cast<uintptr_t>(p.elem2_ramp) |
         reinterpret_cast<uintptr_t>(p.out_ramp)) & 15)
      return false;
  }
  if (p.in2 && (p.dmx_on || p.fir_taps > 0 || p.m2 > kFIn2 || (reinterpret_cast<uintptr_t>(p.in2) & 15) ||
                (p.in2_stream_stride & 3) || (p.in2_frame_stride & 3)))
    return false;
  if (((p.pos0 & 15) && p.pos0 < kDelay) || (p.total & 63) || (p.frame_size & 3)) return false;
  if ((reinterpret_cast<uintptr_t>(p.in) & 15) || (p.in_stream_stride & 3) || (p.in_frame_stride & 3)) return false;
  if ((reinterpret_cast<uintptr_t>(p.pcm) & 15) || (p.pcm_stream_stride & 15)) return false;
  {
    const int64_t frames = (int64_t)p.total / p.frame_size + 2;
    if (frames * p.in_frame_stride * 4 + 100 * (int64_t)p.frame_size >= (int64_t)1 << 31) return false;
    if (p.lpcm && frames * p.lpcm_frame_stride + ((int64_t)1 << 24) >= (int64_t)1 << 31) return false;
  }
  return true;
}

inline bool wide_shape_ok(const RenderParams &p, int m, bool force_generic) {
  if (force_generic || p.og_ch < p.out_ch) return false;
  if (!p.limiter_on || !p.in || p.out_ch <= 2 || p.out_ch > kMaxOut || p.n_end < kWWin) return false;
  if (p.pre_matrix) return false;
  if (p.total & 63) return false;
  if ((reinterpret_cast<uintptr_t>(p.pcm) & 15) || (p.pcm_stream_stride & 15)) return false;
  return sizeof(float) * (size_t)wide_lds_floats(p.out_ch, m) <= 80 * 1024;
}

inline bool wide4_shape_ok(const RenderParams &p, bool mixing) {
  if (getenv("IAMF_HIP_NO_WIDE4")) return false;
  if (p.out_format != IAMF_HIP_FMT_S16 || ((p.total & 1023) && (p.total & 1023) < 256) ||
      (p.frame_size & 3) || p.n_end < 1088)
    return false;
  if ((reinterpret_cast<uintptr_t>(p.in) & 15) || (p.in_stream_stride & 3) || (p.in_frame_stride & 3)) return false;
  if (mixing) {
    if (p.in2 && (p.m2 > kFIn2 || (reinterpret_cast<uintptr_t>(p.in2) & 15) || (p.in2_stream_stride & 3) ||
                  (p.in2_frame_stride & 3)))
      return false;
    if ((p.ramp_stream_stride & 3) || (p.elem2_ramp && !p.in2) ||
        ((reinterpret_cast<uintptr_t>(p.elem_ramp) | reinterpret_cast<uintptr_t>(p.elem2_ramp) |
          reinterpret_cast<uintptr_t>(p.out_ramp)) & 15))
      return false;
  }
  return true;
}

enum class Family {
  Refused,
  Lpcm,
  FirSplit,
  FirFused,
  FastDown,
  Wide4Lfe,
  Wide4,
  Wide4Demix,
  Wide4Down,
  Wide4Mix,
  Nolim,
  Fast,
  Wide,
  Generic,
};
struct Route {
  Family family;
  int variant;
  int err;
};

inline Route pick_route(const RenderParams &p, int m) {
  const auto take = [](Family f, int variant = 0) { return Route{f, variant, IAMF_HIP_OK}; };
  const auto refuse = [](int err) { return Route{Family::Refused, 0, err}; };
  const bool force_generic = getenv("IAMF_HIP_FORCE_GENERIC") != nullptr;
  const bool mixing = p.in2 || p.elem_ramp || p.elem2_ramp || p.out_ramp;
  const bool staged = p.demix_on || p.dmx_on || mixing;
  const bool fast_shape = fast_shape_ok(p, force_generic);

  if (p.lpcm) {
    if (!LpcmM::has(m) || !LpcmOC::has(p.out_ch) || !fast_shape || p.dmx_on) return refuse(IAMF_HIP_ERR_INVALID_STATE);
    return take(Family::Lpcm, p.n_launch <= 1024 && !getenv("IAMF_HIP_LP_LATE"));
  }
  if (p.fir_taps > 0 && p.in) {
    if (((int64_t)(p.total / p.frame_size) + 1) * p.in_frame_stride >= (int64_t)1 << 31) return refuse(IAMF_HIP_ERR_BAD_ARG);
    if (!fast_shape || p.dmx_on) return refuse(IAMF_HIP_ERR_UNIMPLEMENTED);
    if (!FirHomeM::has(m) && !FirM2bM::has(m)) return refuse(IAMF_HIP_ERR_UNIMPLEMENTED);
    const int stage = fir_stage_choice(p);
    return stage == 4 ? take(Family::FirSplit) : take(Family::FirFused, stage);
  }
  if (p.dmx_on && p.dmx_frames && fast_shape && FastDownMC::has(mc(m, p.out_ch))) return take(Family::FastDown);

  const bool fast = !p.lfe && fast_shape && !p.dmx_on;
  const bool wide_shape = wide_shape_ok(p, m, force_generic);
  const bool wide4_shape = wide_shape && wide4_shape_ok(p, mixing);
  const bool pos16 = !(p.pos0 & 15);
  const bool pos_any = pos16 || p.pos0 >= kDelay;

  if (p.lfe) {
    if (!p.lfe_k0 && !staged && wide4_shape && pos16 && Wide4LfeM::has(m) && Wide4C::has(p.out_ch))
      return take(Family::Wide4Lfe, p.use_mfma != 0);
  } else if (wide4_shape && pos_any) {
    if (mixing) {
      if (!p.demix_on && !p.dmx_on && Wide4M::has(m) && Wide4MixC::has(p.out_ch)) return take(Family::Wide4Mix, p.use_mfma != 0);
    } else if (p.dmx_on) {
      if (p.dmx_frames && !p.demix_on && Wide4DownMC::has(mc(m, p.out_ch))) return take(Family::Wide4Down);
    } else if (p.demix_on) {
      if (p.demix_w4 && !p.use_mfma && (p.demix_i0 & 3) == 0 && Wide4DemixM::has(m) && Wide4DemixC::has(p.out_ch))
        return take(Family::Wide4Demix);
    } else if (Wide4M::has(m) && Wide4C::has(p.out_ch)) {
      return take(Family::Wide4, p.use_mfma != 0);
    }
  }
  if (!p.limiter_on && p.in && !p.lfe && !p.pre_matrix && !staged && p.fir_taps == 0 && p.og_ch >= p.out_ch && !force_generic &&
      nolim_shape_ok(p))
    return NolimM::has(m) ? take(Family::Nolim) : refuse(IAMF_HIP_ERR_UNIMPLEMENTED);
  if (fast && FastM::has(m)) return take(Family::Fast, mixing);
  if (!p.lfe && wide_shape && !staged && pos16 && WideM::has(m)) return take(Family::Wide, p.use_mfma != 0);
  return GenericM::has(m) ? take(Family::Generic) : refuse(IAMF_HIP_ERR_UNIMPLEMENTED);
}


template <class F>
void for_each_render_instance(F &&f) {
  for_each_int(GenericM{}, [&](int m) { f(IAMF_HIP_ROUTE_GENERIC, 0, m, 0, 0); });
  for_each_int(NolimM{}, [&](int m) { f(IAMF_HIP_ROUTE_NOLIM, 0, m, 0, 0); });
  for (int mixing = 0; mixing < 2; ++mixing)
    for_each_int(FastM{}, [&](int m) { for_each_int(FastOC{}, [&](int oc) { f(IAMF_HIP_ROUTE_FAST, mixing, m, oc, 0); }); });
  for_each_int(FastDownMC{}, [&](int v) { f(IAMF_HIP_ROUTE_FAST_DOWN, 0, mc_m(v), mc_c(v), 0); });
  for (int mfma = 0; mfma < 2; ++mfma) for_each_int(WideM{}, [&](int m) { f(IAMF_HIP_ROUTE_WIDE, mfma, m, 0, 0); });
  for (int mfma = 0; mfma < 2; ++mfma)
    for_each_int(Wide4M{}, [&](int m) { for_each_int(Wide4C{}, [&](int c) { f(IAMF_HIP_ROUTE_WIDE4, mfma, m, c, 0); }); });
  for_each_int(Wide4DemixM{}, [&](int m) { for_each_int(Wide4DemixC{}, [&](int c) { f(IAMF_HIP_ROUTE_WIDE4_DEMIX, 0, m, c, 0); }); });
  for_each_int(Wide4DownMC{}, [&](int v) { f(IAMF_HIP_ROUTE_WIDE4_DOWN, 0, mc_m(v), mc_c(v), 0); });
  for (int mfma = 0; mfma < 2; ++mfma)
    for_each_int(Wide4M{}, [&](int m) { for_each_int(Wide4MixC{}, [&](int c) { f(IAMF_HIP_ROUTE_WIDE4_MIX, mfma, m, c, 0); }); });
  for (int mfma = 0; mfma < 2; ++mfma)
    for_each_int(Wide4LfeM{}, [&](int m) { for_each_int(Wide4C{}, [&](int c) { f(IAMF_HIP_ROUTE_WIDE4_LFE, mfma, m, c, 0); }); });
  for (int early = 0; early < 2; ++early)
    for_each_int(LpcmM{}, [&](int m) { for_each_int(LpcmOC{}, [&](int oc) { f(IAMF_HIP_ROUTE_LPCM, early, m, oc, 0); }); });
  for_each_int(FanM{}, [&](int m) { for_each_int(FanK{}, [&](int k) { f(IAMF_HIP_ROUTE_FANOUT, 0, m, 0, k); }); });
  for (int home = 1; home >= 0; --home) {
    const auto firs = [&](int m) {
      f(IAMF_HIP_ROUTE_FIR_SPLIT, 0, m, 0, 0);
      for (int stage = 1; stage <= 3; ++stage) f(IAMF_HIP_ROUTE_FIR_FUSED, stage, m, 0, 0);
    };
    if (home) for_each_int(FirHomeM{}, firs);
    else for_each_int(FirM2bM{}, firs);
  }
}

template <class F>
void for_each_render_instance_ext(F &&f) {
  for_each_int(FanLpM{}, [&](int m) { for_each_int(FanLpK{}, [&](int k) { f(IAMF_HIP_ROUTE_FANOUT_LPCM, 0, m, 0, k); }); });
}

struct RouteKey {
  int family, variant, m, c, k;
};
inline RouteKey route_key(const Route &r, const RenderParams &p, int m) {
  switch (r.family) {
    case Family::Refused: break;
    case Family::Lpcm: return {IAMF_HIP_ROUTE_LPCM, r.variant, m, p.out_ch, 0};
    case Family::FirSplit: return {IAMF_HIP_ROUTE_FIR_SPLIT, 0, m, 0, 0};
    case Family::FirFused: return {IAMF_HIP_ROUTE_FIR_FUSED, r.variant, m, 0, 0};
    case Family::FastDown: return {IAMF_HIP_ROUTE_FAST_DOWN, 0, m, p.out_ch, 0};
    case Family::Wide4Lfe: return {IAMF_HIP_ROUTE_WIDE4_LFE, r.variant, m, p.out_ch, 0};
    case Family::Wide4: return {IAMF_HIP_ROUTE_WIDE4, r.variant, m, p.out_ch, 0};
    case Family::Wide4Demix: return {IAMF_HIP_ROUTE_WIDE4_DEMIX, 0, m, p.out_ch, 0};
    case Family::Wide4Down: return {IAMF_HIP_ROUTE_WIDE4_DOWN, 0, m, p.out_ch, 0};
    case Family::Wide4Mix: return {IAMF_HIP_ROUTE_WIDE4_MIX, r.variant, m, p.out_ch, 0};
    case Family::Nolim: return {IAMF_HIP_ROUTE_NOLIM, 0, m, 0, 0};
    case Family::Fast: return {IAMF_HIP_ROUTE_FAST, r.variant, m, p.out_ch, 0};
    case Family::Wide: return {IAMF_HIP_ROUTE_WIDE, r.variant, m, 0, 0};
    case Family::Generic: return {IAMF_HIP_ROUTE_GENERIC, 0, m, 0, 0};
  }
  return {IAMF_HIP_ROUTE_NONE, 0, 0, 0, 0};
}
```

iac_amd/hipabi.py:

```python
import ctypes as C
import os
import subprocess

ROOT = os.path.dirname(os.path.dirname(os.path.abspath(__file__)))
CSRC = os.path.join(ROOT, "iac_amd", "csrc")

FMT_S16, FMT_S24, FMT_S32, FMT_F32 = 16, 24, 32, -32
KIND_H2M, KIND_M2M, KIND_DMX, KIND_FIR = 0, 1, 2, 3
PROJ_AUTO, PROJ_EXACT, PROJ_MFMA = 0, 1, 2
SS = dict(A=0x020, B=0x050, C=0x250, D=0x450, E=0x451, F=0x370, G=0x490, H=0x9A3, I=0x070,
          J=0x470, STEREO=0x200, L51=0x510, L512=0x512, L514=0x514, L71=0x710, L714=0x714,
          MONO=0x100, L712=0x712, L312=0x312, BINAURAL=0x1020)

FP = C.POINTER(C.c_float)


class IamfHipError(RuntimeError):
    def __init__(self, code, what):
        super().__init__("%s failed with IAMF_HIP error %d" % (what, code))
        self.code = code


class Matrix(C.Structure):
    _fields_ = [("kind", C.c_int32), ("in_id", C.c_int32), ("out_id", C.c_int32),
                ("channels", C.c_int32), ("lfe1", C.c_int32), ("lfe2", C.c_int32),
                ("m", C.c_int32), ("n", C.c_int32), ("mat", FP)]


class BatchConfig(C.Structure):
    _fields_ = [("n_streams", C.c_int32), ("frame_size", C.c_int32), ("sample_rate", C.c_int32),
                ("out_channels", C.c_int32), ("out_format", C.c_int32), ("matrix", Matrix),
                ("limiter_enable", C.c_int32), ("limiter_threshold_db", C.c_float),
                ("loudness_enable", C.c_int32), ("projection", C.c_int32), ("fir_taps", C.c_int32), ("lfe_hoa", C.c_int32),
                ("pcm_stride_channels", C.c_int32), ("out_gain_channels", C.c_int32), ("reserved", C.c_int32 * 2)]


class DmxState(C.Structure):
    _fields_ = [("mode", C.c_int32), ("w_idx", C.c_int32), ("w_idx_offset", C.c_int32),
                ("reserved", C.c_int32), ("alpha", C.c_float), ("beta", C.c_float), ("gamma", C.c_float),
                ("delta", C.c_float), ("gamma_w", C.c_float)]


class DmxFrame(C.Structure):
    _fields_ = [("offset", C.c_int32), ("prev", C.c_float * 5), ("cur", C.c_float * 5)]


class RenderArgs(C.Structure):
    _fields_ = [("d_in", C.c_void_p), ("in_stream_stride", C.c_int64), ("in_frame_stride", C.c_int64),
                ("d_in2", C.c_void_p), ("in2_stream_stride", C.c_int64), ("in2_frame_stride", C.c_int64),
                ("d_element_ramp", C.c_void_p), ("d_element2_ramp", C.c_void_p),
                ("d_output_ramp", C.c_void_p), ("ramp_stream_stride", C.c_int64),
                ("d_dmx_frames", C.c_void_p), ("n_frames", C.c_int32), ("n_samples", C.c_int32),
                ("d_pcm", C.c_void_p), ("pcm_stream_stride_bytes", C.c_int64), ("stream", C.c_void_p),
                ("d_demix_frames", C.c_void_p), ("demix_sample0", C.c_int32), ("lfe_pre_samples", C.c_int32),
                ("lfe_post_samples", C.c_int32), ("reserved0", C.c_int32)]


class LpcmLayout(C.Structure):
    _fields_ = [("sample_bytes", C.c_int32), ("little_endian", C.c_int32), ("channels", C.c_int32), ("frame_size", C.c_int32),
                ("src_offset", C.c_int32 * 32), ("src_step", C.c_int32 * 32)]


class LpcmInput(C.Structure):
    _fields_ = [("d_raw", C.c_void_p), ("raw_stream_stride", C.c_int64), ("raw_frame_stride", C.c_int64),
                ("first_sample", C.c_int32), ("layout", LpcmLayout)]


class FanoutReport(C.Structure):
    _fields_ = [("n_fused", C.c_int32), ("input_fused", C.c_int32), ("n_unpacks", C.c_int32), ("reserved", C.c_int32)]


class RouteRow(C.Structure):
    _fields_ = [("family", C.c_int32), ("variant", C.c_int32), ("m", C.c_int32), ("c", C.c_int32), ("k", C.c_int32),
                ("reserved", C.c_int32), ("launches", C.c_int64)]


ROUTE = dict(NONE=0, GENERIC=1, NOLIM=2, FAST=3, FAST_DOWN=4, WIDE=5, WIDE4=6, WIDE4_DEMIX=7, WIDE4_DOWN=8, WIDE4_MIX=9,
             WIDE4_LFE=10, LPCM=11, FANOUT=12, FIR_SPLIT=13, FIR_FUSED=14, FANOUT_LPCM=15, RS_PLAIN=20, RS_TILE=21, RS_BLOCK=22, RS_DIRECT=23)
ROUTE_NAME = {v: k for k, v in ROUTE.items()}


class StreamGains(C.Structure):
    _fields_ = [("element_gain", FP), ("output_gain", FP), ("loudness_gain", FP), ("element2_gain", FP)]


class StreamState(C.Structure):
    _fields_ = [("magic", C.c_uint32), ("version", C.c_uint32), ("kind", C.c_uint32), ("signature", C.c_uint32),
                ("bytes", C.c_int64), ("cursor", C.c_int64 * 2)]


class DemixConfig(C.Structure):
    _fields_ = [("layout", C.c_int32), ("n_in", C.c_int32), ("chs_in", C.c_int32 * 12), ("n_gain", C.c_int32),
                ("gain_ch", C.c_int32 * 12), ("gain", C.c_float * 12), ("frame_offset", C.c_uint32)]


class DemixState(C.Structure):
    _fields_ = [("mode", C.c_int32), ("last_mode", C.c_int32), ("w_idx", C.c_int32), ("last_w_idx", C.c_int32),
                ("last_sfavg", C.c_float * 24)]


class DemixFrame(C.Structure):
    _fields_ = [("prev", C.c_float * 5), ("cur", C.c_float * 5), ("n_recon", C.c_int32),
                ("recon_ch", C.c_int32 * 12), ("recon_prev", C.c_float * 12), ("recon_cur", C.c_float * 12)]


def lib_path():
    return os.environ.get("IAMF_HIP_LIB") or os.path.join(ROOT, "iac_amd", "lib", "libiamf_hip.so")


def build(force=False):
    args = ["make", "-j4", "-C", CSRC]
    if force:
        subprocess.check_call(args + ["clean"], stdout=subprocess.DEVNULL)
    subprocess.check_call(args, stdout=subprocess.DEVNULL)
    return lib_path()


_lib = None


def lib():
    global _lib
    if _lib is None:
        path = lib_path()
        if not os.path.exists(path):
            raise ImportError("libiamf_hip.so is not built (run __graft_entry__.build()); "
                              "iac_amd has no CPU fallback")
        L = C.CDLL(path)
        L.iamf_hip_get_h2m_matrix.argtypes = [C.c_int, C.c_int, C.POINTER(Matrix)]
        L.iamf_hip_get_m2m_matrix.argtypes = [C.c_int, C.c_int, C.POINTER(Matrix)]
        L.iamf_hip_probe_traffic.argtypes = [C.c_int, C.c_int, C.c_int, C.c_int, C.c_void_p, C.c_int64, C.c_void_p,
                                             C.c_int64, C.c_void_p]
        L.iamf_hip_pick_buffer_pair.argtypes = [C.c_int, C.c_int, C.c_int, C.c_int, C.POINTER(C.c_void_p), C.c_int, C.c_int64,
                                                C.POINTER(C.c_void_p), C.c_int, C.c_int64, C.c_void_p,
                                                C.POINTER(C.c_int), C.POINTER(C.c_int), FP]
        L.iamf_hip_get_m2m_matrix_variant.argtypes = [C.c_int, C.c_int, C.c_int, C.POINTER(Matrix)]
        L.iamf_hip_layout_channels.argtypes = [C.c_int]
        L.iamf_hip_batch_create.argtypes = [C.POINTER(BatchConfig), C.POINTER(C.c_void_p)]
        L.iamf_hip_batch_destroy.argtypes = [C.c_void_p]
        L.iamf_hip_batch_destroy.restype = None
        L.iamf_hip_batch_set_gains.argtypes = [C.c_void_p, FP, FP, FP]
        L.iamf_hip_batch_render.argtypes = [C.c_void_p, C.c_void_p, C.c_int64, C.c_int64, C.c_int32,
                                            C.c_void_p, C.c_int64, C.c_void_p]
        L.iamf_hip_batch_flush.argtypes = [C.c_void_p, C.c_void_p, C.c_int64, C.c_void_p]
        L.iamf_hip_batch_render_fanout.argtypes = [C.POINTER(C.c_void_p), C.c_int32, C.c_void_p, C.c_int64, C.c_int64, C.c_int32,
                                                   C.POINTER(C.c_void_p), C.POINTER(C.c_int64), C.c_void_p,
                                                   C.POINTER(C.c_int32), C.POINTER(C.c_int32)]
        L.iamf_hip_batch_render_fanout_range.argtypes = L.iamf_hip_batch_render_fanout.argtypes + [C.c_int32, C.c_int32]
        L.iamf_hip_batch_render_fanout_lpcm.argtypes = [C.POINTER(C.c_void_p), C.c_int32, C.POINTER(LpcmInput), C.c_int32, C.c_int32,
                                                        C.POINTER(C.c_void_p), C.POINTER(C.c_int64), C.c_void_p, C.c_int32, C.c_int32,
                                                        C.POINTER(C.c_int32), C.POINTER(FanoutReport)]
        L.iamf_hip_batch_reset.argtypes = [C.c_void_p]
        L.iamf_hip_batch_render_range.argtypes = [C.c_void_p, C.POINTER(RenderArgs), C.c_int32, C.c_int32]
        L.iamf_hip_batch_flush_range.argtypes = [C.c_void_p, C.c_void_p, C.c_int64, C.c_void_p, C.c_int32, C.c_int32]
        L.iamf_hip_batch_set_gains_range.argtypes = [C.c_void_p, C.c_int32, C.c_int32, C.POINTER(StreamGains), C.c_void_p]
        L.iamf_hip_batch_restart_range.argtypes = [C.c_void_p, C.c_int32, C.c_int32, C.POINTER(StreamGains), C.c_void_p]
        L.iamf_hip_batch_stream_state_bytes.argtypes = [C.c_void_p]
        L.iamf_hip_batch_stream_state_bytes.restype = C.c_int64
        for name in ("iamf_hip_batch_export_range", "iamf_hip_batch_import_range", "iamf_hip_resampler_export_range",
                     "iamf_hip_resampler_import_range"):
            getattr(L, name).argtypes = [C.c_void_p, C.c_int32, C.c_int32, C.c_void_p, C.c_int64, C.POINTER(StreamState),
                                         C.c_void_p]
        L.iamf_hip_resampler_restart_range.argtypes = [C.c_void_p, C.c_int32, C.c_int32, C.c_void_p]
        L.iamf_hip_resampler_stream_state_bytes.argtypes = [C.c_void_p]
        L.iamf_hip_resampler_stream_state_bytes.restype = C.c_int64
        L.iamf_hip_format_bytes.argtypes = [C.c_int]
        L.iamf_hip_version.restype = C.c_char_p
        L.iamf_hip_batch_render_ex.argtypes = [C.c_void_p, C.POINTER(RenderArgs)]
        L.iamf_hip_batch_render_lpcm.argtypes = [C.c_void_p, C.POINTER(LpcmInput), C.POINTER(RenderArgs)]
        L.iamf_hip_batch_render_lpcm_range.argtypes = [C.c_void_p, C.POINTER(LpcmInput), C.POINTER(RenderArgs), C.c_int32, C.c_int32]
        L.iamf_hip_batch_set_second_element.argtypes = [C.c_void_p, C.POINTER(Matrix), FP]
        L.iamf_hip_resampler_create.argtypes = [C.c_int, C.c_int, C.c_int, C.c_int, C.POINTER(C.c_void_p)]
        L.iamf_hip_resampler_destroy.argtypes = [C.c_void_p]
        L.iamf_hip_resampler_destroy.restype = None
        L.iamf_hip_resampler_out_capacity.argtypes = [C.c_void_p, C.c_int]
        L.iamf_hip_resampler_flush_capacity.argtypes = [C.c_void_p]
        L.iamf_hip_resampler_process.argtypes = [C.c_void_p, C.c_void_p, C.c_int64, C.c_int, C.c_void_p, C.c_int64,
                                                 C.c_void_p]
        L.iamf_hip_resampler_flush.argtypes = [C.c_void_p, C.c_void_p, C.c_int64, C.c_void_p]
        L.iamf_hip_resampler_process_range.argtypes = [C.c_void_p, C.c_void_p, C.c_int64, C.c_int, C.c_void_p, C.c_int64,
                                                       C.c_void_p, C.c_int32, C.c_int32]
        L.iamf_hip_resampler_flush_range.argtypes = [C.c_void_p, C.c_void_p, C.c_int64, C.c_void_p, C.c_int32, C.c_int32]
        L.iamf_hip_resampler_same_state.argtypes = [C.c_void_p, C.c_int32, C.c_int32]
        L.iamf_hip_stream_signal.argtypes = [C.c_void_p, C.c_void_p, C.c_uint32]
        L.iamf_hip_deinterleave_f32.argtypes = [C.c_void_p, C.c_int64, C.c_int32, C.c_int32, C.c_int32, C.c_void_p, C.c_int64,
                                                C.c_int64, C.c_void_p]
        L.iamf_hip_batch_set_projection.argtypes = [C.c_void_p, FP, C.c_int]
        L.iamf_hip_batch_share_lfe_state.argtypes = [C.c_void_p, C.c_void_p]
        L.iamf_hip_batch_lfe_advance.argtypes = [C.c_void_p, C.c_void_p, C.c_int64, C.c_int32, C.c_void_p, C.c_int32, C.c_int32]
        L.iamf_hip_lpcm_unpack.argtypes = [C.POINTER(LpcmLayout), C.c_void_p, C.c_int64, C.c_void_p, C.c_int64, C.c_void_p,
                                           C.c_int64, C.c_int32, C.c_void_p]
        L.iamf_hip_batch_set_demixer.argtypes = [C.c_void_p, C.POINTER(DemixConfig)]
        L.iamf_hip_demix_state_init.argtypes = [C.POINTER(DemixState)]
        L.iamf_hip_demix_state_init.restype = None
        L.iamf_hip_demix_set_info.argtypes = [C.POINTER(DemixState), C.c_int, C.c_int]
        L.iamf_hip_demix_frame_fill.argtypes = [C.POINTER(DemixState), C.c_int, C.POINTER(C.c_int32), FP,
                                                C.POINTER(DemixFrame)]
        L.iamf_hip_demix_frame_fill.restype = None
        L.iamf_hip_dmx_valid.argtypes = [C.c_int, C.c_int]
        L.iamf_hip_dmx_layout_channels.argtypes = [C.c_int]
        L.iamf_hip_dmx_state_init.argtypes = [C.POINTER(DmxState)]
        L.iamf_hip_dmx_state_init.restype = None
        L.iamf_hip_dmx_set_mode_weight.argtypes = [C.POINTER(DmxState), C.c_int, C.c_int]
        L.iamf_hip_dmx_coefficients.argtypes = [C.POINTER(DmxState), FP]
        L.iamf_hip_dmx_coefficients.restype = None
        L.iamf_hip_route_instances.argtypes = [C.POINTER(RouteRow), C.c_int]
        L.iamf_hip_route_tally.argtypes = [C.POINTER(RouteRow), C.c_int, C.c_int]
        L.iamf_hip_route_instances_ext.argtypes = [C.POINTER(RouteRow), C.c_int]
        L.iamf_hip_route_tally_ext.argtypes = [C.POINTER(RouteRow), C.c_int, C.c_int]
        L.iamf_hip_shard_split.argtypes = [C.c_int, C.c_int, C.c_int, C.POINTER(C.c_int), C.POINTER(C.c_int)]
        L.iamf_hip_shard_create.argtypes = [C.POINTER(BatchConfig), C.POINTER(C.c_int), C.c_int, C.POINTER(C.c_void_p)]
        L.iamf_hip_shard_destroy.argtypes = [C.c_void_p]
        L.iamf_hip_shard_destroy.restype = None
        L.iamf_hip_shard_devices.argtypes = [C.c_void_p]
        L.iamf_hip_shard_info.argtypes = [C.c_void_p, C.c_int, C.POINTER(C.c_int), C.POINTER(C.c_int), C.POINTER(C.c_int)]
        L.iamf_hip_shard_batch.argtypes = [C.c_void_p, C.c_int]
        L.iamf_hip_shard_batch.restype = C.c_void_p
        L.iamf_hip_shard_render_stream.argtypes = [C.c_void_p, C.c_int]
        L.iamf_hip_shard_render_stream.restype = C.c_void_p
        L.iamf_hip_shard_render.argtypes = [C.c_void_p, C.POINTER(C.c_void_p), C.c_int64, C.c_int64, C.c_int32,
                                            C.POINTER(C.c_void_p), C.c_int64]
        L.iamf_hip_shard_flush.argtypes = [C.c_void_p, C.POINTER(C.c_void_p), C.c_int64]
        L.iamf_hip_shard_gather.argtypes = [C.c_void_p, C.c_int, C.c_void_p, C.c_int64, C.POINTER(C.c_void_p), C.c_int64]
        L.iamf_hip_shard_gather_rows.argtypes = [C.c_void_p, C.c_int, C.c_void_p, C.c_int64, C.POINTER(C.c_void_p), C.c_int64, C.c_int64]
        L.iamf_hip_shard_times.argtypes = [C.c_void_p, C.c_int, C.POINTER(C.c_int64), C.POINTER(C.c_int64), C.POINTER(C.c_int64),
                                           C.POINTER(C.c_double), C.POINTER(C.c_double)]
        L.iamf_hip_shard_sync.argtypes = [C.c_void_p]
        L.iamf_hip_shard_rccl_version.restype = C.c_char_p
        _lib = L
    return _lib


def get_h2m_matrix(order, out_id):
    m = Matrix()
    if lib().iamf_hip_get_h2m_matrix(order, out_id, C.byref(m)) != 0:
        raise KeyError((order, hex(out_id)))
    return m


def get_m2m_matrix(in_id, out_id, variant=0):
    m = Matrix()
    if lib().iamf_hip_get_m2m_matrix_variant(variant, in_id, out_id, C.byref(m)) != 0:
        raise KeyError((hex(in_id), hex(out_id)))
    return m


def dmx_matrix(in_layout, out_layout):
    m = Matrix()
    m.kind, m.in_id, m.out_id = KIND_DMX, in_layout, out_layout
    m.channels = m.n = lib().iamf_hip_dmx_layout_channels(out_layout)
    m.m = lib().iamf_hip_dmx_layout_channels(in_layout)
    m.lfe1 = m.lfe2 = -1
    return m


def fir_matrix(hrir):
    import numpy as np
    h = np.ascontiguousarray(hrir, dtype=np.float32)
    m = Matrix()
    m.kind, m.in_id, m.out_id, m.channels, m.lfe1, m.lfe2 = KIND_FIR, 0, SS["BINAURAL"], 2, -1, -1
    m.m, m.n = h.shape[1], 2
    m.mat = h.ctypes.data_as(FP)
    m._keep = h
    return m


def lpcm_unpack(layout, d_raw, raw_stream_stride, d_first_count, d_out, out_stream_stride, n_streams, stream=None,
                first_count_stride=2):
    r = lib().iamf_hip_lpcm_unpack(C.byref(layout), d_raw, raw_stream_stride, d_first_count, first_count_stride, d_out,
                                   out_stream_stride, n_streams, stream)
    if r < 0:
        raise IamfHipError(r, "iamf_hip_lpcm_unpack")
    return r


def route_instances():
    L = lib()
    n = L.iamf_hip_route_instances(None, 0)
    rows = (RouteRow * max(n, 1))()
    n = min(n, L.iamf_hip_route_instances(rows, n))
    return [(ROUTE_NAME[r.family], r.variant, r.m, r.c, r.k) for r in rows[:n]]


def route_tally(reset=True):
    L = lib()
    cap = L.iamf_hip_route_instances(None, 0) + 1
    rows = (RouteRow * cap)()
    n = L.iamf_hip_route_tally(rows, cap, 1 if reset else 0)
    return {(ROUTE_NAME[r.family], r.variant, r.m, r.c, r.k): r.launches for r in rows[:min(n, cap)]}


def route_reset():
    lib().iamf_hip_route_tally(None, 0, 1)


def route_instances_ext():
    L = lib()
    n = L.iamf_hip_route_instances_ext(None, 0)
    rows = (RouteRow * max(n, 1))()
    n = min(n, L.iamf_hip_route_instances_ext(rows, n))
    return [(ROUTE_NAME[r.family], r.variant, r.m, r.c, r.k) for r in rows[:n]]


def route_tally_ext(reset=True):
    L = lib()
    cap = L.iamf_hip_route_instances_ext(None, 0) + 1
    rows = (RouteRow * cap)()
    n = L.iamf_hip_route_tally_ext(rows, cap, 1 if reset else 0)
    return {(ROUTE_NAME[r.family], r.variant, r.m, r.c, r.k): r.launches for r in rows[:min(n, cap)]}


FANOUT_MAX = 4


def render_fanout(batches, d_in, in_stream_stride, in_frame_stride, n_frames, d_pcms, pcm_strides, stream=None):
    n = len(batches)
    if len(d_pcms) != n or len(pcm_strides) != n:
        raise ValueError("render_fanout: one PCM buffer and one stride per batch")
    hs = (C.c_void_p * n)(*[b.h for b in batches])
    pcms = (C.c_void_p * n)(*d_pcms)
    strides = (C.c_int64 * n)(*pcm_strides)
    emitted = (C.c_int32 * max(n, 1))()
    fused = C.c_int32(0)
    r = lib().iamf_hip_batch_render_fanout(hs, n, d_in, in_stream_stride, in_frame_stride, n_frames, pcms, strides, stream,
                                           emitted, C.byref(fused))
    if r < 0:
        raise IamfHipError(r, "iamf_hip_batch_render_fanout")
    return list(emitted[:n]), fused.value


def render_fanout_range(batches, d_in, in_stream_stride, in_frame_stride, n_frames, d_pcms, pcm_strides, stream0, n_streams,
                        stream=None):
    n = len(batches)
    if len(d_pcms) != n or len(pcm_strides) != n:
        raise ValueError("render_fanout_range: one PCM buffer and one stride per batch")
    hs = (C.c_void_p * n)(*[b.h for b in batches])
    pcms = (C.c_void_p * n)(*d_pcms)
    strides = (C.c_int64 * n)(*pcm_strides)
    emitted = (C.c_int32 * max(n, 1))()
    fused = C.c_int32(0)
    r = lib().iamf_hip_batch_render_fanout_range(hs, n, d_in, in_stream_stride, in_frame_stride, n_frames, pcms, strides, stream,
                                                 emitted, C.byref(fused), stream0, n_streams)
    if r < 0:
        raise IamfHipError(r, "iamf_hip_batch_render_fanout_range")
    return list(emitted[:n]), fused.value


def render_fanout_lpcm(batches, lpcm_input, n_frames, d_pcms, pcm_strides, stream=None, n_samples=0, stream0=0, n_streams=None,
                       report=None):
    n = len(batches)
    if len(d_pcms) != n or len(pcm_strides) != n:
        raise ValueError("render_fanout_lpcm: one PCM buffer and one stride per batch")
    if n_streams is None:
        n_streams = batches[0].cfg.n_streams if n else 1
    hs = (C.c_void_p * n)(*[b.h for b in batches])
    pcms = (C.c_void_p * n)(*d_pcms)
    strides = (C.c_int64 * n)(*pcm_strides)
    emitted = (C.c_int32 * max(n, 1))()
    rep = FanoutReport() if report is None else report
    r = lib().iamf_hip_batch_render_fanout_lpcm(hs, n, C.byref(lpcm_input), n_frames, n_samples, pcms, strides, stream, stream0,
                                                n_streams, emitted, C.byref(rep))
    if r < 0:
        raise IamfHipError(r, "iamf_hip_batch_render_fanout_lpcm")
    return list(emitted[:n]), (rep.n_fused, rep.input_fused, rep.n_unpacks)


def layout_channels(out_id):
    return lib().iamf_hip_layout_channels(out_id)


def _fparr(a):
    if a is None:
        return None
    arr = (C.c_float * len(a))(*[float(v) for v in a])
    return arr


def stream_gains(element=None, output=None, loudness=None, element2=None):
    g = StreamGains()
    g._keep = [_fparr(a) for a in (element, output, loudness, element2)]
    for name, arr in zip(("element_gain", "output_gain", "loudness_gain", "element2_gain"), g._keep):
        if arr is not None:
            setattr(g, name, C.cast(arr, FP))
    return g


def _export(fn, what, h, s0, cnt, d_state, stride, stream):
    tickets = (StreamState * max(cnt, 1))()
    r = fn(h, s0, cnt, d_state, stride, tickets, stream)
    if r != 0:
        raise IamfHipError(r, what)
    return list(tickets[:cnt])


def _import(fn, what, h, s0, cnt, d_state, stride, tickets, stream):
    arr = (StreamState * max(len(tickets), 1))(*tickets)
    r = fn(h, s0, cnt, d_state, stride, arr if len(tickets) >= cnt else None, stream)
    if r != 0:
        raise IamfHipError(r, what)


class Batch:

    def __init__(self, n_streams, matrix, out_channels, frame_size=1024, sample_rate=48000,
                 out_format=FMT_S16, limiter=True, threshold_db=-1.0, loudness=False, projection=PROJ_AUTO, fir_taps=0,
                 lfe_hoa=False, pcm_stride_channels=0):
        cfg = BatchConfig()
        cfg.n_streams = n_streams
        cfg.frame_size = frame_size
        cfg.sample_rate = sample_rate
        cfg.out_channels = out_channels
        cfg.out_format = out_format
        cfg.matrix = matrix
        cfg.limiter_enable = 1 if limiter else 0
        cfg.limiter_threshold_db = threshold_db
        cfg.loudness_enable = 1 if loudness else 0
        cfg.projection = projection
        cfg.fir_taps = fir_taps
        cfg.lfe_hoa = 1 if lfe_hoa else 0
        cfg.pcm_stride_channels = pcm_stride_channels
        self.cfg = cfg
        self.bytes_per_sample = lib().iamf_hip_format_bytes(out_format)
        h = C.c_void_p()
        r = lib().iamf_hip_batch_create(C.byref(cfg), C.byref(h))
        if r != 0:
            raise IamfHipError(r, "iamf_hip_batch_create")
        self.h = h

    def set_gains(self, element=None, output=None, loudness=None):
        r = lib().iamf_hip_batch_set_gains(self.h, _fparr(element), _fparr(output), _fparr(loudness))
        if r != 0:
            raise IamfHipError(r, "iamf_hip_batch_set_gains")

    def render(self, d_in, in_stream_stride, in_frame_stride, n_frames, d_pcm, pcm_stream_stride_bytes,
               stream=None):
        r = lib().iamf_hip_batch_render(self.h, d_in, in_stream_stride, in_frame_stride, n_frames,
                                        d_pcm, pcm_stream_stride_bytes, stream)
        if r < 0:
            raise IamfHipError(r, "iamf_hip_batch_render")
        return r

    def render_ex(self, args):
        r = lib().iamf_hip_batch_render_ex(self.h, C.byref(args))
        if r < 0:
            raise IamfHipError(r, "iamf_hip_batch_render_ex")
        return r

    def render_lpcm(self, lpcm_input, args):
        r = lib().iamf_hip_batch_render_lpcm(self.h, C.byref(lpcm_input), C.byref(args))
        if r < 0:
            raise IamfHipError(r, "iamf_hip_batch_render_lpcm")
        return r

    def render_lpcm_range(self, lpcm_input, args, stream0, n_streams):
        r = lib().iamf_hip_batch_render_lpcm_range(self.h, C.byref(lpcm_input), C.byref(args), stream0, n_streams)
        if r < 0:
            raise IamfHipError(r, "iamf_hip_batch_render_lpcm_range")
        return r

    def render_range(self, args, stream0, n_streams):
        r = lib().iamf_hip_batch_render_range(self.h, C.byref(args), stream0, n_streams)
        if r < 0:
            raise IamfHipError(r, "iamf_hip_batch_render_range")
        return r

    def flush_range(self, d_pcm, pcm_stream_stride_bytes, stream, stream0, n_streams):
        r = lib().iamf_hip_batch_flush_range(self.h, d_pcm, pcm_stream_stride_bytes, stream, stream0, n_streams)
        if r < 0:
            raise IamfHipError(r, "iamf_hip_batch_flush_range")
        return r

    def set_second_element(self, matrix, gains=None):
        r = lib().iamf_hip_batch_set_second_element(self.h, C.byref(matrix), _fparr(gains))
        if r != 0:
            raise IamfHipError(r, "iamf_hip_batch_set_second_element")

    def set_projection(self, matrix):
        rows = [list(r) for r in matrix]
        r = lib().iamf_hip_batch_set_projection(self.h, _fparr([v for row in rows for v in row]), len(rows))
        if r != 0:
            raise IamfHipError(r, "iamf_hip_batch_set_projection")

    def set_demixer(self, layout, chs_in, gains=(), frame_offset=0):
        c = DemixConfig()
        c.layout, c.n_in, c.n_gain, c.frame_offset = layout, len(chs_in), len(gains), frame_offset
        for i, ch in enumerate(chs_in):
            c.chs_in[i] = ch
        for i, (ch, g) in enumerate(gains):
            c.gain_ch[i], c.gain[i] = ch, g
        r = lib().iamf_hip_batch_set_demixer(self.h, C.byref(c))
        if r != 0:
            raise IamfHipError(r, "iamf_hip_batch_set_demixer")

    def flush(self, d_pcm, pcm_stream_stride_bytes, stream=None):
        r = lib().iamf_hip_batch_flush(self.h, d_pcm, pcm_stream_stride_bytes, stream)
        if r < 0:
            raise IamfHipError(r, "iamf_hip_batch_flush")
        return r

    def reset(self):
        r = lib().iamf_hip_batch_reset(self.h)
        if r != 0:
            raise IamfHipError(r, "iamf_hip_batch_reset")

    def set_gains_range(self, s0, cnt, gains, stream=None):
        r = lib().iamf_hip_batch_set_gains_range(self.h, s0, cnt, C.byref(gains) if gains is not None else None, stream)
        if r != 0:
            raise IamfHipError(r, "iamf_hip_batch_set_gains_range")

    def restart_range(self, s0, cnt, gains=None, stream=None):
        r = lib().iamf_hip_batch_restart_range(self.h, s0, cnt, C.byref(gains) if gains is not None else None, stream)
        if r != 0:
            raise IamfHipError(r, "iamf_hip_batch_restart_range")

    def stream_state_bytes(self):
        r = lib().iamf_hip_batch_stream_state_bytes(self.h)
        if r < 0:
            raise IamfHipError(r, "iamf_hip_batch_stream_state_bytes")
        return r

    def export_range(self, s0, cnt, d_state, stride_bytes, stream=None):
        return _export(lib().iamf_hip_batch_export_range, "iamf_hip_batch_export_range", self.h, s0, cnt, d_state,
                       stride_bytes, stream)

    def import_range(self, s0, cnt, d_state, stride_bytes, tickets, stream=None):
        _import(lib().iamf_hip_batch_import_range, "iamf_hip_batch_import_range", self.h, s0, cnt, d_state, stride_bytes,
                tickets, stream)

    def close(self):
        if self.h:
            lib().iamf_hip_batch_destroy(self.h)
            self.h = None

    def __del__(self):
        try:
            self.close()
        except Exception:
            pass


class Resampler:

    def __init__(self, n_streams, channels, in_rate, out_rate):
        h = C.c_void_p()
        r = lib().iamf_hip_resampler_create(n_streams, channels, in_rate, out_rate, C.byref(h))
        if r != 0:
            raise IamfHipError(r, "iamf_hip_resampler_create")
        self.h = h

    def out_capacity(self, ns):
        return lib().iamf_hip_resampler_out_capacity(self.h, ns)

    def flush_capacity(self):
        return lib().iamf_hip_resampler_flush_capacity(self.h)

    def process(self, d_in, in_stride, ns, d_out, out_stride, stream=None):
        r = lib().iamf_hip_resampler_process(self.h, d_in, in_stride, ns, d_out, out_stride, stream)
        if r < 0:
            raise IamfHipError(r, "iamf_hip_resampler_process")
        return r

    def flush(self, d_out, out_stride, stream=None):
        r = lib().iamf_hip_resampler_flush(self.h, d_out, out_stride, stream)
        if r < 0:
            raise IamfHipError(r, "iamf_hip_resampler_flush")
        return r

    def process_range(self, d_in, in_stride, ns, d_out, out_stride, s0, cnt, stream=None):
        return lib().iamf_hip_resampler_process_range(self.h, d_in, in_stride, ns, d_out, out_stride, stream, s0, cnt)

    def flush_range(self, d_out, out_stride, s0, cnt, stream=None):
        return lib().iamf_hip_resampler_flush_range(self.h, d_out, out_stride, stream, s0, cnt)

    def same_state(self, a, b):
        return bool(lib().iamf_hip_resampler_same_state(self.h, a, b))

    def restart_range(self, s0, cnt, stream=None):
        r = lib().iamf_hip_resampler_restart_range(self.h, s0, cnt, stream)
        if r != 0:
            raise IamfHipError(r, "iamf_hip_resampler_restart_range")

    def stream_state_bytes(self):
        r = lib().iamf_hip_resampler_stream_state_bytes(self.h)
        if r < 0:
            raise IamfHipError(r, "iamf_hip_resampler_stream_state_bytes")
        return r

    def export_range(self, s0, cnt, d_state, stride_bytes, stream=None):
        return _export(lib().iamf_hip_resampler_export_range, "iamf_hip_resampler_export_range", self.h, s0, cnt, d_state,
                       stride_bytes, stream)

    def import_range(self, s0, cnt, d_state, stride_bytes, tickets, stream=None):
        _import(lib().iamf_hip_resampler_import_range, "iamf_hip_resampler_import_range", self.h, s0, cnt, d_state,
                stride_bytes, tickets, stream)

    def close(self):
        if self.h:
            lib().iamf_hip_resampler_destroy(self.h)
            self.h = None


def pick_buffer_pair(n_streams, chunks, rows, pieces, in_ptrs, in_stream_stride_bytes, out_ptrs, out_stream_stride_bytes,
                     stream=None):
    import numpy as np
    n_in, n_out = len(in_ptrs), len(out_ptrs)
    ins = (C.c_void_p * n_in)(*in_ptrs)
    outs = (C.c_void_p * n_out)(*out_ptrs)
    bi, bo = C.c_int(-1), C.c_int(-1)
    ms = np.zeros((n_in, n_out), dtype=np.float32)
    r = lib().iamf_hip_pick_buffer_pair(n_streams, chunks, rows, pieces, ins, n_in, in_stream_stride_bytes, outs, n_out,
                                        out_stream_stride_bytes, C.c_void_p(stream or 0), C.byref(bi), C.byref(bo),
                                        ms.ctypes.data_as(FP))
    if r != 0:
        raise RuntimeError("iamf_hip_pick_buffer_pair: %d" % r)
# ... 3 lines not shown
```

include/iamf_hip.h:

```cpp
#ifndef IAMF_HIP_H
#define IAMF_HIP_H

#include <stddef.h>
#include <stdint.h>

#ifdef __cplusplus
extern "C" {
#endif

enum {
  IAMF_HIP_OK = 0,
  IAMF_HIP_ERR_BAD_ARG = -1,
  IAMF_HIP_ERR_BUFFER_TOO_SMALL = -2,
  IAMF_HIP_ERR_INTERNAL = -3,
  IAMF_HIP_ERR_INVALID_STATE = -5,
  IAMF_HIP_ERR_UNIMPLEMENTED = -6,
  IAMF_HIP_ERR_ALLOC_FAIL = -7,
  IAMF_HIP_ERR_DEVICE = -100
};

enum {
  IAMF_HIP_SS_A = 0x020, IAMF_HIP_SS_B = 0x050, IAMF_HIP_SS_C = 0x250, IAMF_HIP_SS_D = 0x450,
  IAMF_HIP_SS_E = 0x451, IAMF_HIP_SS_F = 0x370, IAMF_HIP_SS_G = 0x490, IAMF_HIP_SS_H = 0x9A3,
  IAMF_HIP_SS_I = 0x070, IAMF_HIP_SS_J = 0x470,
// ... 1 lines not shown
  IAMF_HIP_L_514 = 0x514, IAMF_HIP_L_71 = 0x710, IAMF_HIP_L_714 = 0x714,
  IAMF_HIP_L_MONO = 0x100, IAMF_HIP_L_712 = 0x712, IAMF_HIP_L_312 = 0x312,
  IAMF_HIP_L_BINAURAL = 0x1020
};

enum { IAMF_HIP_KIND_H2M = 0, IAMF_HIP_KIND_M2M = 1, IAMF_HIP_KIND_DMX = 2, IAMF_HIP_KIND_FIR = 3 };

enum { IAMF_HIP_PROJ_AUTO = 0, IAMF_HIP_PROJ_EXACT = 1, IAMF_HIP_PROJ_MFMA = 2 };

enum { IAMF_HIP_FMT_S16 = 16, IAMF_HIP_FMT_S24 = 24, IAMF_HIP_FMT_S32 = 32, IAMF_HIP_FMT_F32 = -32 };

typedef struct {
  int32_t kind;
  int32_t in_id;
  int32_t out_id;
  int32_t channels;
  int32_t lfe1, lfe2;
  int32_t m, n;
  const float *mat;
} iamf_hip_matrix;

int iamf_hip_get_h2m_matrix(int order, int out_id, iamf_hip_matrix *out);
int iamf_hip_get_m2m_matrix(int in_id, int out_id, iamf_hip_matrix *out);
enum { IAMF_HIP_VARIANT_DEFAULT = 0, IAMF_HIP_VARIANT_SAMSUNG_TV = 1 };
int iamf_hip_get_m2m_matrix_variant(int variant, int in_id, int out_id, iamf_hip_matrix *out);
int iamf_hip_layout_channels(int out_id);

typedef struct iamf_hip_batch iamf_hip_batch;

typedef struct {
  int32_t n_streams;
  int32_t frame_size;
  int32_t sample_rate;
  int32_t out_channels;
  int32_t out_format;
  iamf_hip_matrix matrix;
  int32_t limiter_enable;
  float limiter_threshold_db;
  int32_t loudness_enable;
  int32_t projection;
  int32_t fir_taps;
  int32_t lfe_hoa;
  int32_t pcm_stride_channels;
  int32_t out_gain_channels;
  int32_t reserved[2];
} iamf_hip_batch_config;

int iamf_hip_batch_create(const iamf_hip_batch_config *cfg, iamf_hip_batch **out);
void iamf_hip_batch_destroy(iamf_hip_batch *b);

int iamf_hip_batch_set_gains(iamf_hip_batch *b, const float *element_gain,
                             const float *output_gain, const float *loudness_gain);

int iamf_hip_batch_render(iamf_hip_batch *b, const float *d_in, int64_t in_stream_stride,
                          int64_t in_frame_stride, int32_t n_frames, void *d_pcm,
                          int64_t pcm_stream_stride_bytes, void *stream);

typedef struct {
  int32_t mode, w_idx;
  int32_t w_idx_offset;
  int32_t reserved;
  float alpha, beta, gamma, delta;
  float gamma_w;
} iamf_hip_dmx_state;

typedef struct {
  int32_t offset;
  float prev[5];
  float cur[5];
} iamf_hip_dmx_frame;

int iamf_hip_dmx_valid(int in_layout, int out_layout);
int iamf_hip_dmx_layout_channels(int layout);
void iamf_hip_dmx_state_init(iamf_hip_dmx_state *st);
int iamf_hip_dmx_set_mode_weight(iamf_hip_dmx_state *st, int mode, int w_idx);
void iamf_hip_dmx_coefficients(const iamf_hip_dmx_state *st, float out[5]);

int iamf_hip_batch_set_second_element(iamf_hip_batch *b, const iamf_hip_matrix *mx,
                                      const float *element2_gain);

int iamf_hip_batch_share_lfe_state(iamf_hip_batch *b, iamf_hip_batch *owner);
int iamf_hip_batch_lfe_advance(iamf_hip_batch *b, const float *d_in, int64_t in_stream_stride, int32_t n_samples, void *stream,
                               int32_t first, int32_t count);
int iamf_hip_batch_set_projection(iamf_hip_batch *b, const float *matrix, int l_in);

typedef struct iamf_hip_demix_config {
  int32_t layout;
  int32_t n_in;
  int32_t chs_in[12];
  int32_t n_gain;
  int32_t gain_ch[12];
  float gain[12];
  uint32_t frame_offset;
} iamf_hip_demix_config;

int iamf_hip_batch_set_demixer(iamf_hip_batch *b, const iamf_hip_demix_config *cfg);

typedef struct iamf_hip_demix_state {
  int32_t mode, last_mode, w_idx, last_w_idx;
  float last_sfavg[24];
} iamf_hip_demix_state;

typedef struct iamf_hip_demix_frame {
  float prev[5], cur[5];
  int32_t n_recon;
  int32_t recon_ch[12];
  float recon_prev[12], recon_cur[12];
} iamf_hip_demix_frame;

void iamf_hip_demix_state_init(iamf_hip_demix_state *st);
int iamf_hip_demix_set_info(iamf_hip_demix_state *st, int mode, int w_idx);
void iamf_hip_demix_frame_fill(iamf_hip_demix_state *st, int n_recon, const int32_t *recon_ch,
                               const float *recon_gain, iamf_hip_demix_frame *out);

typedef struct {
  const float *d_in;
  int64_t in_stream_stride, in_frame_stride;
  const float *d_in2;
  int64_t in2_stream_stride, in2_frame_stride;
  const float *d_element_ramp, *d_element2_ramp, *d_output_ramp;
  int64_t ramp_stream_stride;
  const iamf_hip_dmx_frame *d_dmx_frames;
  int32_t n_frames;
  int32_t n_samples;
  void *d_pcm;
  int64_t pcm_stream_stride_bytes;
  void *stream;
  const iamf_hip_demix_frame *d_demix_frames;
  int32_t demix_sample0;
  int32_t lfe_pre_samples, lfe_post_samples, reserved0;
} iamf_hip_render_args;

int iamf_hip_batch_render_ex(iamf_hip_batch *b, const iamf_hip_render_args *args);

int iamf_hip_batch_render_range(iamf_hip_batch *b, const iamf_hip_render_args *args, int32_t stream0, int32_t n_streams);
int iamf_hip_batch_flush_range(iamf_hip_batch *b, void *d_pcm, int64_t pcm_stream_stride_bytes, void *stream,
                               int32_t stream0, int32_t n_streams);

int iamf_hip_batch_flush(iamf_hip_batch *b, void *d_pcm, int64_t pcm_stream_stride_bytes,
                         void *stream);

#define IAMF_HIP_FANOUT_MAX 4
int iamf_hip_batch_render_fanout(iamf_hip_batch *const *batches, int32_t n_batches, const float *d_in,
                                 int64_t in_stream_stride, int64_t in_frame_stride, int32_t n_frames, void *const *d_pcm,
                                 const int64_t *pcm_stream_stride_bytes, void *stream, int32_t *n_emitted ,
                                 int32_t *n_fused );
int iamf_hip_batch_render_fanout_range(iamf_hip_batch *const *batches, int32_t n_batches, const float *d_in,
                                       int64_t in_stream_stride, int64_t in_frame_stride, int32_t n_frames, void *const *d_pcm,
                                       const int64_t *pcm_stream_stride_bytes, void *stream, int32_t *n_emitted ,
                                       int32_t *n_fused , int32_t stream0, int32_t n_streams);

typedef struct iamf_hip_resampler iamf_hip_resampler;
int iamf_hip_resampler_create(int n_streams, int channels, int in_rate, int out_rate,
                              iamf_hip_resampler **out);
void iamf_hip_resampler_destroy(iamf_hip_resampler *r);
int iamf_hip_resampler_out_capacity(const iamf_hip_resampler *r, int ns);
int iamf_hip_resampler_flush_capacity(const iamf_hip_resampler *r);
int iamf_hip_resampler_process(iamf_hip_resampler *r, const float *d_in, int64_t in_stream_stride,
                               int ns, float *d_out, int64_t out_stream_stride, void *stream);
int iamf_hip_resampler_flush(iamf_hip_resampler *r, float *d_out, int64_t out_stream_stride, void *stream);
int iamf_hip_resampler_process_range(iamf_hip_resampler *r, const float *d_in, int64_t in_stream_stride, int ns, float *d_out,
                                     int64_t out_stream_stride, void *stream, int32_t stream0, int32_t n_streams);
int iamf_hip_resampler_flush_range(iamf_hip_resampler *r, float *d_out, int64_t out_stream_stride, void *stream, int32_t stream0,
                                   int32_t n_streams);
int iamf_hip_resampler_same_state(const iamf_hip_resampler *r, int32_t stream_a, int32_t stream_b);

int iamf_hip_batch_reset(iamf_hip_batch *b);

typedef struct {
  const float *element_gain, *output_gain, *loudness_gain, *element2_gain;
} iamf_hip_stream_gains;

int iamf_hip_batch_set_gains_range(iamf_hip_batch *b, int32_t stream0, int32_t n_streams,
                                   const iamf_hip_stream_gains *gains, void *stream);
int iamf_hip_batch_restart_range(iamf_hip_batch *b, int32_t stream0, int32_t n_streams,
                                 const iamf_hip_stream_gains *gains , void *stream);

typedef struct {
  uint32_t magic, version;
  uint32_t kind;
  uint32_t signature;
  int64_t bytes;
  int64_t cursor[2];
} iamf_hip_stream_state;

int64_t iamf_hip_batch_stream_state_bytes(const iamf_hip_batch *b);
int iamf_hip_batch_export_range(iamf_hip_batch *b, int32_t stream0, int32_t n_streams, void *d_state,
                                int64_t state_stream_stride_bytes, iamf_hip_stream_state *tickets , void *stream);
int iamf_hip_batch_import_range(iamf_hip_batch *b, int32_t stream0, int32_t n_streams, const void *d_state,
                                int64_t state_stream_stride_bytes, const iamf_hip_stream_state *tickets, void *stream);

int iamf_hip_resampler_restart_range(iamf_hip_resampler *r, int32_t stream0, int32_t n_streams, void *stream);
int64_t iamf_hip_resampler_stream_state_bytes(const iamf_hip_resampler *r);
int iamf_hip_resampler_export_range(iamf_hip_resampler *r, int32_t stream0, int32_t n_streams, void *d_state,
                                    int64_t state_stream_stride_bytes, iamf_hip_stream_state *tickets, void *stream);
int iamf_hip_resampler_import_range(iamf_hip_resampler *r, int32_t stream0, int32_t n_streams, const void *d_state,
                                    int64_t state_stream_stride_bytes, const iamf_hip_stream_state *tickets, void *stream);

int iamf_hip_format_bytes(int out_format);
const char *iamf_hip_version(void);

int iamf_hip_probe_traffic(int n_streams, int chunks, int rows, int pieces, const void *d_in,
                           int64_t in_stream_stride_bytes, void *d_out, int64_t out_stream_stride_bytes,
                           void *stream);
int iamf_hip_pick_buffer_pair(int n_streams, int chunks, int rows, int pieces, const void *const *d_in_candidates,
                              int n_in, int64_t in_stream_stride_bytes, void *const *d_out_candidates, int n_out,
                              int64_t out_stream_stride_bytes, void *stream, int *best_in, int *best_out, float *ms);

int iamf_hip_selftest_shared_divisor(float divisor, uint64_t counts[3]);

int iamf_hip_decoder_set_hoa_lfe(void *decoder_handle, int enable);
int iamf_hip_decoder_set_variant(void *decoder_handle, int variant);

typedef struct iamf_hip_shard iamf_hip_shard;
int iamf_hip_shard_split(int n_streams, int n_devices, int index, int *first, int *count);
int iamf_hip_shard_create(const iamf_hip_batch_config *cfg, const int *devices, int n_devices, iamf_hip_shard **out);
void iamf_hip_shard_destroy(iamf_hip_shard *s);
int iamf_hip_shard_devices(const iamf_hip_shard *s);
int iamf_hip_shard_info(const iamf_hip_shard *s, int index, int *device, int *first, int *count);
iamf_hip_batch *iamf_hip_shard_batch(iamf_hip_shard *s, int index);
void *iamf_hip_shard_render_stream(iamf_hip_shard *s, int index);
int iamf_hip_shard_render(iamf_hip_shard *s, const float *const *d_in, int64_t in_stream_stride, int64_t in_frame_stride,
                          int32_t n_frames, void *const *d_pcm, int64_t pcm_stream_stride_bytes);
int iamf_hip_shard_flush(iamf_hip_shard *s, void *const *d_pcm, int64_t pcm_stream_stride_bytes);
int iamf_hip_shard_gather(iamf_hip_shard *s, int root_index, void *d_dst, int64_t dst_stream_stride_bytes,
                          void *const *d_pcm, int64_t pcm_stream_stride_bytes);
int iamf_hip_shard_gather_rows(iamf_hip_shard *s, int root_index, void *d_dst, int64_t dst_stream_stride_bytes,
                               void *const *d_pcm, int64_t pcm_stream_stride_bytes, int64_t bytes_per_stream);
int iamf_hip_shard_sync(iamf_hip_shard *s);
int iamf_hip_shard_times(iamf_hip_shard *s, int index, int64_t *last_sent_bytes, int64_t *total_sent_bytes,
                         int64_t *last_received_bytes, double *last_gather_ms, double *total_gather_ms);
const char *iamf_hip_shard_rccl_version(void);

#define IAMF_HIP_LPCM_MAX_CHANNELS 32
typedef struct iamf_hip_lpcm_layout {
  int32_t sample_bytes;
  int32_t little_endian;
  int32_t channels;
  int32_t frame_size;
  int32_t src_offset[IAMF_HIP_LPCM_MAX_CHANNELS];
  int32_t src_step[IAMF_HIP_LPCM_MAX_CHANNELS];
} iamf_hip_lpcm_layout;
int iamf_hip_lpcm_unpack(const iamf_hip_lpcm_layout *layout, const void *d_raw, int64_t raw_stream_stride,
                         const int32_t *d_first_count, int64_t first_count_stride, float *d_out, int64_t out_stream_stride,
                         int32_t n_streams, void *stream);

typedef struct iamf_hip_lpcm_input {
  const void *d_raw;
  int64_t raw_stream_stride, raw_frame_stride;
  int32_t first_sample;
  iamf_hip_lpcm_layout layout;
} iamf_hip_lpcm_input;
int iamf_hip_batch_render_lpcm(iamf_hip_batch *b, const iamf_hip_lpcm_input *in, const iamf_hip_render_args *args);
int iamf_hip_batch_render_lpcm_range(iamf_hip_batch *b, const iamf_hip_lpcm_input *in, const iamf_hip_render_args *args,
                                     int32_t stream0, int32_t n_streams);

typedef struct iamf_hip_fanout_report {
  int32_t n_fused;
  int32_t input_fused;
  int32_t n_unpacks;
  int32_t reserved;
} iamf_hip_fanout_report;
int iamf_hip_batch_render_fanout_lpcm(iamf_hip_batch *const *batches, int32_t n_batches, const iamf_hip_lpcm_input *in,
                                      int32_t n_frames, int32_t n_samples, void *const *d_pcm,
                                      const int64_t *pcm_stream_stride_bytes, void *stream, int32_t stream0, int32_t n_streams,
                                      int32_t *n_emitted , iamf_hip_fanout_report *report );

int iamf_hip_upload_by_kernel(const void *h_pinned, void *d_dst, size_t bytes, void *stream);
int iamf_hip_stream_signal(void *stream, volatile uint32_t *h_pinned_flag, uint32_t seq);
int iamf_hip_deinterleave_f32(const float *d_src, int64_t src_stream_stride, int32_t channels, int32_t n_streams,
                              int32_t n_samples, float *d_dst, int64_t dst_stream_stride, int64_t dst_channel_stride, void *stream);

enum {
  IAMF_HIP_ROUTE_NONE = 0,
  IAMF_HIP_ROUTE_GENERIC = 1,
  IAMF_HIP_ROUTE_NOLIM = 2,
  IAMF_HIP_ROUTE_FAST = 3,
  IAMF_HIP_ROUTE_FAST_DOWN = 4,
  IAMF_HIP_ROUTE_WIDE = 5,
  IAMF_HIP_ROUTE_WIDE4 = 6,
  IAMF_HIP_ROUTE_WIDE4_DEMIX = 7,
  IAMF_HIP_ROUTE_WIDE4_DOWN = 8,
  IAMF_HIP_ROUTE_WIDE4_MIX = 9,
  IAMF_HIP_ROUTE_WIDE4_LFE = 10,
  IAMF_HIP_ROUTE_LPCM = 11,
  IAMF_HIP_ROUTE_FANOUT = 12,
  IAMF_HIP_ROUTE_FIR_SPLIT = 13,
  IAMF_HIP_ROUTE_FIR_FUSED = 14,
  IAMF_HIP_ROUTE_FANOUT_LPCM = 15,
  IAMF_HIP_ROUTE_RS_PLAIN = 20,
  IAMF_HIP_ROUTE_RS_TILE = 21,
  IAMF_HIP_ROUTE_RS_BLOCK = 22,
  IAMF_HIP_ROUTE_RS_DIRECT = 23
};
typedef struct {
  int32_t family, variant, m, c, k;
  int32_t reserved;
  int64_t launches;
} iamf_hip_route_row;
int iamf_hip_route_instances(iamf_hip_route_row *rows, int cap);
int iamf_hip_route_tally(iamf_hip_route_row *rows, int cap, int reset);
int iamf_hip_route_instances_ext(iamf_hip_route_row *rows, int cap);
int iamf_hip_route_tally_ext(iamf_hip_route_row *rows, int cap, int reset);

typedef struct iamf_hip_decoder_group iamf_hip_decoder_group;
int iamf_hip_decoder_group_create(void *const *handles, int n, int host_threads, iamf_hip_decoder_group **out);
int iamf_hip_decoder_group_times(const iamf_hip_decoder_group *g, double *seconds4, int64_t *rounds);
int iamf_hip_decoder_group_decode(iamf_hip_decoder_group *g, const uint8_t *const *data, const int32_t *sizes,
                                  uint32_t *rsizes, void *const *pcm, int32_t *results);
void iamf_hip_decoder_group_destroy(iamf_hip_decoder_group *g);

#define IAMF_HIP_GROUP_MAX_IN_FLIGHT 2
int iamf_hip_decoder_group_submit(iamf_hip_decoder_group *g, const uint8_t *const *data, const int32_t *sizes,
                                  uint32_t *rsizes, void *const *pcm, int32_t *results, uint64_t *ticket);
int iamf_hip_decoder_group_poll(iamf_hip_decoder_group *g, uint64_t ticket);
int iamf_hip_decoder_group_complete(iamf_hip_decoder_group *g, uint64_t ticket);

#ifdef __cplusplus
}
#endif
#endif
```

Baseline: 86950.

## Slice FIR-split FFT stage and overlap a wave-level limiter on a side stream

Measured after the change: 87310 (median of 2 runs). About the same (+0.4%).

```diff
diff --git a/iac_amd/__init__.py b/iac_amd/__init__.py
--- a/iac_amd/__init__.py
+++ b/iac_amd/__init__.py
@@ -37,6 +37,7 @@
     layout_channels,
     lib,
     lib_path,
+    limiter_wave_launches,
     lpcm_unpack,
     render_fanout,
     render_fanout_lpcm,
diff --git a/iac_amd/csrc/iamf_render.hip b/iac_amd/csrc/iamf_render.hip
--- a/iac_amd/csrc/iamf_render.hip
+++ b/iac_amd/csrc/iamf_render.hip
@@ -181,6 +181,9 @@
   int32_t *d_fir_id_feed = nullptr;
   float fir_inv_scale = 1.f;
   int fir_cur = 0;
+  hipStream_t fir_side = nullptr;
+  hipEvent_t fir_ev[kFirMaxSlices + 2] = {};
+  bool id_matrix = false;
   bool lfe = false;
   float lfe_a1 = 0.f, lfe_a2 = 0.f, lfe_a3 = 0.f, lfe_b1 = 0.f, lfe_b2 = 0.f;
   double lfe_div = 0.0;
@@ -270,16 +273,28 @@
   else launch_big_lds<&render_wide_kernel<M, false>, 80 * 1024>(grid, dim3(256), lds, st, p);
 }
 
-int launch(const RenderParams &p, int m, size_t lds_bytes, hipStream_t st) {
+struct BatchSide {
+  hipStream_t fir_side = nullptr;
+  const hipEvent_t *fir_ev = nullptr;
+  bool id_matrix = false;
+};
+
+bool launch_fir_stage(const RenderParams &p, int m, hipStream_t st, int pass0, int npass) {
+  return dispatch(FirHomeM{}, m, [&](auto M) { launch_fft_m<M.value>(p, st, pass0, npass); }) ||
+         iamf_hip_fir_m2b_launch_fft(&p, m, st, pass0, npass);
+}
+
+int launch(const RenderParams &p, int m, size_t lds_bytes, hipStream_t st, const BatchSide &side = BatchSide{}) {
   const Route r = pick_route(p, m);
   const dim3 grid((unsigned)p.n_launch);
   bool launched = false;
+  bool wave = false;
   switch (r.family) {
     case Family::Refused: return r.err;
     case Family::Lpcm: launched = iamf_hip_fast_lpcm_launch(&p, m, r.variant, st); break;
     case Family::FirSplit: {
-      if (!dispatch(FirHomeM{}, m, [&](auto M) { launch_fft_m<M.value>(p, st); }) && !iamf_hip_fir_m2b_launch_fft(&p, m, st))
-        return IAMF_HIP_ERR_INTERNAL;
+      const int sp = (side.fir_side && fft_two_base_ok(p, m)) ? fir_slice_passes(p, kFftSpan) : 0;
+      if (!launch_fir_stage(p, m, st, 0, sp ? sp : -1)) return IAMF_HIP_ERR_INTERNAL;
       HIPCHK(hipGetLastError());
       RenderParams q = p;
       q.in = p.fir_y;
@@ -291,8 +306,30 @@
       q.n_feeds = 2;
       q.fir_taps = 0;
       q.fir_hist = q.fir_hist_next = nullptr;
-      launch_fast_m<2>(q, false, grid, st);
-      launched = true;
+      if (!sp) {
+        launch_fast_m<2>(q, false, grid, st);
+        launched = true;
+        break;
+      }
+      const int passes = (p.total + kFftSpan - 1) / kFftSpan;
+      const hipEvent_t *ev = side.fir_ev;
+      HIPCHK(hipEventRecord(ev[0], st));
+      HIPCHK(hipStreamWaitEvent(side.fir_side, ev[0], 0));
+      for (int p0 = 0, j = 0; p0 < passes; p0 += sp, ++j) {
+        const int np = passes - p0 < sp ? passes - p0 : sp;
+        if (p0 && !launch_fir_stage(p, m, st, p0, np)) return IAMF_HIP_ERR_INTERNAL;
+        HIPCHK(hipGetLastError());
+        HIPCHK(hipEventRecord(ev[1 + j], st));
+        HIPCHK(hipStreamWaitEvent(side.fir_side, ev[1 + j], 0));
+        const int off = p0 * kFftSpan;
+        const int cnt = p.total - off < np * kFftSpan ? p.total - off : np * kFftSpan;
+        if (!iamf_hip_limiter_wave_launch(&q, off, cnt, side.fir_side)) return IAMF_HIP_ERR_INTERNAL;
+        HIPCHK(hipGetLastError());
+        iamf_hip_limiter_wave_count();
+      }
+      HIPCHK(hipEventRecord(ev[1 + kFirMaxSlices], side.fir_side));
+      HIPCHK(hipStreamWaitEvent(st, ev[1 + kFirMaxSlices], 0));
+      launched = wave = true;
       break;
     }
     case Family::FirFused:
@@ -308,15 +345,22 @@
     case Family::Wide4Demix:
     case Family::Wide4Down: launched = iamf_hip_wide4_launch(&p, m, st); break;
     case Family::Nolim: launched = dispatch(NolimM{}, m, [&](auto M) { launch_nolim_m<M.value>(p, st); }); break;
-    case Family::Fast: launched = dispatch(FastM{}, m, [&](auto M) { launch_fast_m<M.value>(p, r.variant != 0, grid, st); }); break;
+    case Family::Fast:
+      if (!r.variant && side.id_matrix && m == p.out_ch && getenv("IAMF_HIP_LIMITER_WAVE")) {
+        launched = wave = iamf_hip_limiter_wave_launch(&p, 0, p.total, st);
+        if (launched) iamf_hip_limiter_wave_count();
+        break;
+      }
+      launched = dispatch(FastM{}, m, [&](auto M) { launch_fast_m<M.value>(p, r.variant != 0, grid, st); });
+      break;
     case Family::Wide: launched = dispatch(WideM{}, m, [&](auto M) { launch_wide_m<M.value>(p, grid, st); }); break;
     case Family::Generic: launched = dispatch(GenericM{}, m, [&](auto M) { launch_m<M.value>(p, grid, lds_bytes, st); }); break;
   }
   if (!launched) return IAMF_HIP_ERR_INTERNAL;
   HIPCHK(hipGetLastError());
   const RouteKey k = route_key(r, p, m);
-  iamf_hip_route_count(k.family, k.variant, k.m, k.c, k.k);
-  if (r.family == Family::FirSplit) iamf_hip_route_count(IAMF_HIP_ROUTE_FAST, 0, 2, 2, 0);
+  if (r.family != Family::Fast || !wave) iamf_hip_route_count(k.family, k.variant, k.m, k.c, k.k);
+  if (r.family == Family::FirSplit && !wave) iamf_hip_route_count(IAMF_HIP_ROUTE_FAST, 0, 2, 2, 0);
   return IAMF_HIP_OK;
 }
 
@@ -388,6 +432,7 @@
   int sc, bps;
   int64_t pos;
   int total, s0, cnt;
+  BatchSide side;
 };
 
 int render_prepare(iamf_hip_batch *b, const iamf_hip_render_args &a, int total, int s0, int cnt, const LpcmIn *lp, PreparedCall &pc) {
@@ -560,6 +605,9 @@
     p.pcm = b->d_nat;
     p.pcm_stream_stride = (int64_t)per_stream;
   }
+  pc.side.fir_side = b->fir_side;
+  pc.side.fir_ev = b->fir_ev;
+  pc.side.id_matrix = b->id_matrix;
   pc.a = a;
   pc.m_eff = m_eff;
   pc.lds = lds;
@@ -574,7 +622,7 @@
 }
 
 int render_launch(const PreparedCall &pc) {
-  return launch(pc.p, pc.m_eff, pc.lds, static_cast<hipStream_t>(pc.a.stream));
+  return launch(pc.p, pc.m_eff, pc.lds, static_cast<hipStream_t>(pc.a.stream), pc.side);
 }
 
 int render_commit(iamf_hip_batch *b, const PreparedCall &pc) {
@@ -762,6 +810,10 @@
       }
     b->sparse = 2 * set < all ? 1 : 0;
     b->h_fm = fm;
+    b->id_matrix = mx.m == cfg->out_channels && mx.m <= 2 && b->n_feeds == mx.m;
+    for (int c = 0; b->id_matrix && c < mx.m; ++c)
+      for (int k = 0; k < mx.m; ++k)
+        if (b->src_feed[c] != c || fm[(size_t)c * mx.m + k] != (k == c ? 1.f : 0.f)) b->id_matrix = false;
   }
 
   const float atk = 0.001f, rel = 0.200f;
@@ -856,6 +908,8 @@
       CREATE_CHK(hipMemcpy(b->d_fir_id, id, sizeof(id), hipMemcpyHostToDevice));
       CREATE_CHK(hipMalloc(&b->d_fir_id_feed, sizeof(idf)));
       CREATE_CHK(hipMemcpy(b->d_fir_id_feed, idf, sizeof(idf), hipMemcpyHostToDevice));
+      CREATE_CHK(hipStreamCreateWithFlags(&b->fir_side, hipStreamNonBlocking));
+      for (hipEvent_t &e : b->fir_ev) CREATE_CHK(hipEventCreateWithFlags(&e, hipEventDisableTiming));
     }
   }
   CREATE_CHK(hipMalloc(&b->d_dmx_tab, sizeof(dmx_tab)));
@@ -886,6 +940,9 @@
   } restore{sw, cur};
   if (b->rendered) (void)hipEventSynchronize(b->done);
   if (b->done) (void)hipEventDestroy(b->done);
+  if (b->fir_side) (void)hipStreamDestroy(b->fir_side);
+  for (hipEvent_t e : b->fir_ev)
+    if (e) (void)hipEventDestroy(e);
   (void)hipFree(b->d_matrix_pre);
   (void)hipFree(b->d_matrix);
   (void)hipFree(b->d_gains);
diff --git a/iac_amd/csrc/iamf_render_fir_m2b.hip b/iac_amd/csrc/iamf_render_fir_m2b.hip
--- a/iac_amd/csrc/iamf_render_fir_m2b.hip
+++ b/iac_amd/csrc/iamf_render_fir_m2b.hip
@@ -19,13 +19,23 @@
 #include "render_fir_fft.hpp"
 #include "render_fast.hpp"
 #include "render_fir_launch.hpp"
+#include "render_limiter_wave.hpp"
 
 }
 
-int iamf_hip_fir_m2b_launch_fft(const void *params, int m, hipStream_t st) {
+int iamf_hip_fir_m2b_launch_fft(const void *params, int m, hipStream_t st, int pass0, int npass) {
   RenderParams p;
   memcpy(&p, params, sizeof(p));
-  return dispatch(FirM2bM{}, m, [&](auto M) { launch_fft_m<M.value>(p, st); });
+  return dispatch(FirM2bM{}, m, [&](auto M) { launch_fft_m<M.value>(p, st, pass0, npass); });
+}
+
+int iamf_hip_limiter_wave_launch(const void *params, int off, int cnt, hipStream_t st) {
+  RenderParams p;
+  memcpy(&p, params, sizeof(p));
+  if (p.out_ch == 2) launch_limiter_wave<2>(p, off, cnt, st);
+  else if (p.out_ch == 1) launch_limiter_wave<1>(p, off, cnt, st);
+  else return 0;
+  return 1;
 }
 
 int iamf_hip_fir_m2b_launch(const void *params, int m, int stage, hipStream_t st) {
diff --git a/iac_amd/csrc/iamf_route.hip b/iac_amd/csrc/iamf_route.hip
--- a/iac_amd/csrc/iamf_route.hip
+++ b/iac_amd/csrc/iamf_route.hip
@@ -77,6 +77,7 @@
 
 std::atomic<int64_t> g_launches[kRouteCap + 1];
 std::atomic<int64_t> g_launches_ext[kRouteCap + 1];
+std::atomic<int64_t> g_limiter_wave;
 
 int list_instances(const RouteTable &t, iamf_hip_route_row *rows, int cap) {
   for (int i = 0; rows && i < t.n && i < cap; ++i) rows[i] = t.rows[i];
@@ -105,6 +106,8 @@
   g_launches[route_table().find(pack_key(family, variant, m, c, k))].fetch_add(1, std::memory_order_relaxed);
 }
 
+void iamf_hip_limiter_wave_count(void) { g_limiter_wave.fetch_add(1, std::memory_order_relaxed); }
+
 void iamf_hip_route_count_ext(int family, int variant, int m, int c, int k) {
   g_launches_ext[route_table_ext().find(pack_key(family, variant, m, c, k))].fetch_add(1, std::memory_order_relaxed);
 }
@@ -117,6 +120,10 @@
   return tally_of(route_table(), g_launches, rows, cap, reset);
 }
 
+int64_t iamf_hip_limiter_wave_launches(int reset) {
+  return reset ? g_limiter_wave.exchange(0, std::memory_order_relaxed) : g_limiter_wave.load(std::memory_order_relaxed);
+}
+
 int iamf_hip_route_instances_ext(iamf_hip_route_row *rows, int cap) { return list_instances(route_table_ext(), rows, cap); }
 
 int iamf_hip_route_tally_ext(iamf_hip_route_row *rows, int cap, int reset) {
diff --git a/iac_amd/csrc/render_entry.hpp b/iac_amd/csrc/render_entry.hpp
--- a/iac_amd/csrc/render_entry.hpp
+++ b/iac_amd/csrc/render_entry.hpp
@@ -9,11 +9,13 @@
 IAMF_INTERNAL int iamf_hip_fanout_lp_launch(const void *params, int m, int k, hipStream_t st);
 IAMF_INTERNAL int iamf_hip_fast_lpcm_launch(const void *params, int m, int early, hipStream_t st);
 IAMF_INTERNAL int iamf_hip_fir_m2b_launch(const void *params, int m, int stage, hipStream_t st);
-IAMF_INTERNAL int iamf_hip_fir_m2b_launch_fft(const void *params, int m, hipStream_t st);
+IAMF_INTERNAL int iamf_hip_fir_m2b_launch_fft(const void *params, int m, hipStream_t st, int pass0, int npass);
+IAMF_INTERNAL int iamf_hip_limiter_wave_launch(const void *params, int off, int cnt, hipStream_t st);
 IAMF_INTERNAL int iamf_hip_lpcm_unpack_frames(const iamf_hip_lpcm_layout *lay, const void *d_raw, int64_t raw_stream_stride,
                                               int64_t raw_frame_stride, int32_t n_frames, const int32_t *d_first_count,
                                               int64_t first_count_stride, float *d_out, int64_t out_stream_stride,
                                               int64_t out_frame_stride, int32_t n_streams, void *stream, int32_t uniform_first,
                                               int32_t uniform_count);
 IAMF_INTERNAL void iamf_hip_route_count(int family, int variant, int m, int c, int k);
+IAMF_INTERNAL void iamf_hip_limiter_wave_count(void);
 IAMF_INTERNAL void iamf_hip_route_count_ext(int family, int variant, int m, int c, int k);
diff --git a/iac_amd/csrc/render_fir_fft.hpp b/iac_amd/csrc/render_fir_fft.hpp
--- a/iac_amd/csrc/render_fir_fft.hpp
+++ b/iac_amd/csrc/render_fir_fft.hpp
@@ -623,7 +623,7 @@
 #define IAMF_FFT_OCC 2
 #endif
 template <int M, bool FAST2 = false>
-__global__ __launch_bounds__(256, IAMF_FFT_OCC) void fir_fft_kernel(const RenderParams p, float *gy, int64_t gy_stream_stride) {
+__global__ __launch_bounds__(256, IAMF_FFT_OCC) void fir_fft_kernel(const RenderParams p, float *gy, int64_t gy_stream_stride, int pass0) {
   extern __shared__ float fft_lds[];
   const int s = blockIdx.y + p.stream0, t = threadIdx.x;
   FftTwiddles tw;
@@ -634,9 +634,10 @@
   const bool has_pre = p.fir_pre_next != nullptr;
   const int g256 = has_pre ? p.frame_size >> 8 : 1;
   const int64_t pre_off = has_pre ? ((int64_t)(s / g256) * M) * p.frame_size + (int64_t)(s % g256) * kFirHist : 0;
-  fir_stage_fft<M, FAST2>(p, in_s, hist, kFftSpan * (int)blockIdx.x, reinterpret_cast<fft_c32 *>(fft_lds), tw,
+  const int pass = (int)blockIdx.x + pass0;
+  fir_stage_fft<M, FAST2>(p, in_s, hist, kFftSpan * pass, reinterpret_cast<fft_c32 *>(fft_lds), tw,
                           gy + (int64_t)s * gy_stream_stride, FAST2 ? p.fir_pre + pre_off : nullptr);
-  if (blockIdx.x == 0) {
+  if (pass == 0) {
     float *hn = p.fir_hist_next + (int64_t)s * M * kFirHist;
     for (int ch = 0; ch < M; ++ch) {
       const float x = fir_input(p, in_s, hist, ch, p.total - kFirHist + t);
diff --git a/iac_amd/csrc/render_fir_launch.hpp b/iac_amd/csrc/render_fir_launch.hpp
--- a/iac_amd/csrc/render_fir_launch.hpp
+++ b/iac_amd/csrc/render_fir_launch.hpp
@@ -14,11 +14,16 @@
   }
 }
 
+inline bool fft_two_base_ok(const RenderParams &p, int m) {
+  return (m & 1) == 0 && p.fir_pre && p.fir_pre_next && p.total % p.frame_size == 0 && !getenv("IAMF_HIP_FIR_GENERAL_FETCH");
+}
+
 template <int M>
-void launch_fft_m(const RenderParams &p, hipStream_t st) {
-  const dim3 g((unsigned)((p.total + kFftSpan - 1) / kFftSpan), (unsigned)p.n_launch);
-  if ((M & 1) == 0 && p.fir_pre && p.fir_pre_next && p.total % p.frame_size == 0 && !getenv("IAMF_HIP_FIR_GENERAL_FETCH"))
-    hipLaunchKernelGGL((fir_fft_kernel<M, (M & 1) == 0>), g, dim3(256), sizeof(float) * (size_t)kFftLdsFloats, st, p, p.fir_y, 2 * (int64_t)p.total);
+void launch_fft_m(const RenderParams &p, hipStream_t st, int pass0 = 0, int npass = -1) {
+  if (npass < 0) npass = (p.total + kFftSpan - 1) / kFftSpan - pass0;
+  const dim3 g((unsigned)npass, (unsigned)p.n_launch);
+  if (fft_two_base_ok(p, M))
+    hipLaunchKernelGGL((fir_fft_kernel<M, (M & 1) == 0>), g, dim3(256), sizeof(float) * (size_t)kFftLdsFloats, st, p, p.fir_y, 2 * (int64_t)p.total, pass0);
   else
-    hipLaunchKernelGGL((fir_fft_kernel<M, false>), g, dim3(256), sizeof(float) * (size_t)kFftLdsFloats, st, p, p.fir_y, 2 * (int64_t)p.total);
+    hipLaunchKernelGGL((fir_fft_kernel<M, false>), g, dim3(256), sizeof(float) * (size_t)kFftLdsFloats, st, p, p.fir_y, 2 * (int64_t)p.total, pass0);
 }
diff --git a/iac_amd/csrc/render_limiter_wave.hpp b/iac_amd/csrc/render_limiter_wave.hpp
--- /dev/null
+++ b/iac_amd/csrc/render_limiter_wave.hpp
@@ -0,0 +1,306 @@
+#pragma once
+
+constexpr int kLwChunk = 256;
+constexpr int kLwRing = 512;
+constexpr int kLwWin = 320;
+
+__host__ __device__ constexpr int limiter_wave_lds_floats(int oc) {
+  return oc * kLwRing + 2 * kLwRing + 2 * (kLwRing / 16) + 2 * kLwChunk + 2 * kLwWin;
+}
+static_assert(limiter_wave_lds_floats(2) * 4 <= 18 * 1024, "four of them beside two stage workgroups on a CU");
+
+__device__ __forceinline__ void lw_sync() {
+  __builtin_amdgcn_fence(__ATOMIC_ACQ_REL, "wavefront");
+  __builtin_amdgcn_wave_barrier();
+}
+
+template <int OC>
+__global__ __launch_bounds__(64, 8) void limiter2_wave_kernel(const RenderParams p, const int off, const int cnt) {
+  extern __shared__ float lw_lds[];
+  constexpr int R = kLwRing;
+  constexpr int NB = R / 16;
+  float *ring_y = lw_lds;
+  float *ring_pm = ring_y + OC * R;
+  float *ring_suf = ring_pm + R;
+  float *ring_bm = ring_suf + R;
+  float *arr_p = ring_bm + 2 * NB;
+  float *arr_g = arr_p + kLwChunk;
+  float *win = arr_g + kLwChunk;
+  float *head = win + kLwWin;
+
+  const int s = blockIdx.x + p.stream0;
+  const int t = threadIdx.x;
+  const int q = t & 3;
+  const int n_atk = p.n_atk, n_end = p.n_end;
+  const int fs = p.frame_size;
+  const float thr = p.thr;
+  const int64_t pos_in = p.pos0 + off;
+  int base = (int)((pos_in & ~(int64_t)15) % R);
+
+  auto put4 = [&](int rp, float4 y0, float4 y1, float4 pm, float4 &pre_ex) {
+    const float i0 = pm.x, i1 = fmaxf(i0, pm.y), i2 = fmaxf(i1, pm.z), i3 = fmaxf(i2, pm.w);
+    const float s3 = pm.w, s2 = fmaxf(pm.z, s3), s1 = fmaxf(pm.y, s2), s0 = fmaxf(pm.x, s1);
+    const float qa = dpp_quad_bcast0(i3), qb = dpp_quad_bcast1(i3), qc = dpp_quad_bcast2(i3), qd = dpp_quad_bcast3(i3);
+    const float before = fmaxf(fmaxf(q >= 1 ? qa : 0.f, q >= 2 ? qb : 0.f), q >= 3 ? qc : 0.f);
+    const float after = fmaxf(fmaxf(q <= 2 ? qd : 0.f, q <= 1 ? qc : 0.f), q <= 0 ? qb : 0.f);
+    pre_ex = make_float4(before, fmaxf(before, i0), fmaxf(before, i1), fmaxf(before, i2));
+    *reinterpret_cast<float4 *>(&ring_y[rp]) = y0;
+    if constexpr (OC == 2) *reinterpret_cast<float4 *>(&ring_y[R + rp]) = y1;
+    *reinterpret_cast<float4 *>(&ring_pm[rp]) = pm;
+    *reinterpret_cast<float4 *>(&ring_suf[rp]) = make_float4(fmaxf(s0, after), fmaxf(s1, after), fmaxf(s2, after), fmaxf(s3, after));
+    if (q == 0) ring_bm[rp >> 4] = ring_bm[(rp >> 4) + NB] = fmaxf(fmaxf(qa, qb), fmaxf(qc, qd));
+  };
+
+  {
+    const float *sy = p.ring_y + (int64_t)s * OC * kSave;
+    const float *spm = p.ring_pm + (int64_t)s * kSave;
+    const int rp = (base - kSave + 4 * t) & (R - 1);
+    float4 pre_ex;
+    put4(rp, *reinterpret_cast<const float4 *>(&sy[4 * t]), *reinterpret_cast<const float4 *>(&sy[(OC - 1) * kSave + 4 * t]),
+         *reinterpret_cast<const float4 *>(&spm[4 * t]), pre_ex);
+#pragma unroll
+    for (int r = 0; r < kLwWin / 64; ++r) {
+      const int i = t + 64 * r;
+      head[i] = p.ctab[i < n_end ? i : n_end];
+    }
+  }
+  const LimState ls = p.lim[s];
+  float g_cur = ls.g, gs = ls.gs, ge = ls.ge;
+  int n_st = ls.n;
+  const float eg = p.gains[s], og = p.gains[p.n_streams + s], lg = p.gains[2 * p.n_streams + s];
+  const bool eg_on = (eg != 1.f && eg > 0.f);
+  const bool og_on = (og != 1.f && og > 0.f);
+  const bool lg_on = p.loudness_on && (lg != 1.0f);
+  const float m_eg = eg_on ? eg : 1.f, m_og = og_on ? og : 1.f, m_lg = lg_on ? lg : 1.f;
+  const bool any_gain = eg_on || og_on || lg_on;
+
+  const int lead = p.pos0 > kDelay ? kDelay : (int)p.pos0;
+  const int bytes = p.out_format == IAMF_HIP_FMT_S16 ? 2 : (p.out_format == IAMF_HIP_FMT_S24 ? 3 : 4);
+  uint8_t *pcm = p.pcm + (int64_t)s * p.pcm_stream_stride;
+  const float *in_s = p.in + (int64_t)s * p.in_stream_stride;
+  const int end = off + cnt;
+
+  float4 x[OC];
+  auto load_x = [&](int k) {
+    const int f = k / fs, i = k - f * fs;
+    const int o = f * (int)p.in_frame_stride + i;
+#pragma unroll
+    for (int c = 0; c < OC; ++c) x[c] = ld_stream4(in_s + (o + c * fs));
+  };
+#pragma unroll
+  for (int c = 0; c < OC; ++c) x[c] = make_float4(0.f, 0.f, 0.f, 0.f);
+  if (4 * t < cnt) load_x(off + 4 * t);
+
+  float wv[kLwWin / 64];
+  auto fetch_window = [&](int n0) {
+#pragma unroll
+    for (int r = 0; r < kLwWin / 64; ++r) {
+      const int i = n0 + 1 + t + 64 * r;
+      wv[r] = 1.0f;
+      if (n0 < n_end) wv[r] = p.ctab[i < n_end ? i : n_end];
+    }
+  };
+  fetch_window(n_st);
+
+  for (int c0 = off; c0 < end; c0 += kLwChunk) {
+    const int ccnt = end - c0 < kLwChunk ? end - c0 : kLwChunk;
+    const int k = c0 + 4 * t;
+    const bool valid = 4 * t < ccnt;
+    const int rp = (base + 4 * t) & (R - 1);
+    const int rd = (base + 4 * t - kDelay) & (R - 1);
+
+#pragma unroll
+    for (int r = 0; r < kLwWin / 64; ++r) win[t + 64 * r] = wv[r];
+
+    float4 y[OC];
+    float4 pm = make_float4(0.f, 0.f, 0.f, 0.f);
+#pragma unroll
+    for (int c = 0; c < OC; ++c) {
+      float4 v = make_float4(0.f + x[c].x, 0.f + x[c].y, 0.f + x[c].z, 0.f + x[c].w);
+      if (any_gain) {
+        v.x = ((v.x * m_eg) * m_og) * m_lg;
+        v.y = ((v.y * m_eg) * m_og) * m_lg;
+        v.z = ((v.z * m_eg) * m_og) * m_lg;
+        v.w = ((v.w * m_eg) * m_og) * m_lg;
+      }
+      y[c] = v;
+      pm.x = fmaxf(pm.x, fabsf(v.x));
+      pm.y = fmaxf(pm.y, fabsf(v.y));
+      pm.z = fmaxf(pm.z, fabsf(v.z));
+      pm.w = fmaxf(pm.w, fabsf(v.w));
+    }
+    if (k + kLwChunk < end) load_x(k + kLwChunk);
+
+    float4 pre_ex;
+    if (valid) put4(rp, y[0], y[OC - 1], pm, pre_ex);
+    else pre_ex = make_float4(0.f, 0.f, 0.f, 0.f);
+    lw_sync();
+
+    float4 pk4;
+    {
+      const float *bm = ring_bm + ((rp >> 4) + NB - 14 + (q < 3 ? 4 * q : 10));
+      float w14 = fmaxf(fmaxf(bm[0], bm[1]), fmaxf(bm[2], bm[3]));
+      w14 = fmaxf(w14, __int_as_float(__builtin_amdgcn_update_dpp(0, __float_as_int(w14), 0xB1, 0xf, 0xf, true)));
+      w14 = fmaxf(w14, __int_as_float(__builtin_amdgcn_update_dpp(0, __float_as_int(w14), 0x4E, 0xf, 0xf, true)));
+      const float4 so = *reinterpret_cast<const float4 *>(&ring_suf[rd]);
+      pk4.x = fmaxf(fmaxf(so.x, w14), pre_ex.x);
+      pk4.y = fmaxf(fmaxf(so.y, w14), pre_ex.y);
+      pk4.z = fmaxf(fmaxf(so.z, w14), pre_ex.z);
+      pk4.w = fmaxf(fmaxf(so.w, w14), pre_ex.w);
+      *reinterpret_cast<float4 *>(&arr_p[4 * t]) = pk4;
+    }
+    lw_sync();
+
+    const int n_chunk = n_st;
+    auto look = [&](int ci) {
+      const int d = ci - n_chunk - 1;
+      return (d >= 0 && d < kLwWin) ? win[d] : head[ci < kLwWin ? ci : kLwWin - 1];
+    };
+    const int nblk = ccnt >> 6;
+    const int last_lane = (ccnt >> 2) - 1;
+    float4 g = make_float4(1.f, 1.f, 1.f, 1.f);
+    int bs = 0;
+    while (true) {
+      int kfirst = kBig;
+      const int o0 = 4 * t - 64 * bs;
+      if (o0 >= 0) {
+        const int n0 = __builtin_amdgcn_readfirstlane(n_st);
+        const int last = n0 + (ccnt - 64 * bs) - 1;
+        float gh[4] = {1.f, 1.f, 1.f, 1.f};
+        if (n0 < n_end) {
+          const float *tb = (bs == 0 ? win : head + (n0 + 1)) + o0;
+          const float cf[4] = {tb[0], tb[1], tb[2], tb[3]};
+          if (n0 >= n_atk && last < n_end) {
+            const float r1 = 1.0f - ge;
+#pragma unroll
+            for (int j = 0; j < 4; ++j) gh[j] = ge + cf[j] * r1;
+          } else {
+            const int nb = n0 + o0;
+            const float a1 = gs - ge, r1 = 1.0f - ge;
+#pragma unroll
+            for (int j = 0; j < 4; ++j) {
+              const float ga = gs - cf[j] * a1, gr = ge + cf[j] * r1;
+              gh[j] = nb + j < n_atk ? ga : (nb + j < n_end ? gr : 1.0f);
+            }
+          }
+        }
+        g = make_float4(gh[0], gh[1], gh[2], gh[3]);
+        const float px = pk4.x * g.x, py = pk4.y * g.y, pz = pk4.z * g.z, pw = pk4.w * g.w;
+        if (valid && fmaxf(fmaxf(px, py), fmaxf(pz, pw)) > thr) {
+          if (pw > thr) kfirst = 4 * t + 3;
+          if (pz > thr) kfirst = 4 * t + 2;
+          if (py > thr) kfirst = 4 * t + 1;
+          if (px > thr) kfirst = 4 * t + 0;
+        }
+      }
+      const unsigned long long any = __ballot(kfirst != kBig);
+      if (any == 0ull) {
+        g_cur = readlane_f(g.w, last_lane);
+        n_st = n_st + (ccnt - 64 * bs) < n_end ? n_st + (ccnt - 64 * bs) : n_end;
+        break;
+      }
+      const int b0 = __builtin_amdgcn_readlane(kfirst, __builtin_ctzll(any)) >> 6;
+      int ln = n_st + 64 * (b0 - bs) < n_end ? n_st + 64 * (b0 - bs) : n_end;
+      const int be = limiter_wave(arr_p, arr_g, look, b0, nblk, ln, gs, ge, g_cur, thr, n_atk, n_end, true);
+      lw_sync();
+      if (4 * t >= 64 * b0 && 4 * t < 64 * be) g = *reinterpret_cast<const float4 *>(&arr_g[4 * t]);
+      n_st = ln;
+      bs = be;
+      if (bs >= nblk) break;
+    }
+
+    if (c0 + kLwChunk < end) fetch_window(n_st);
+
+    const int j0 = lead + k - kDelay;
+    if (valid && j0 >= 0) {
+      float4 o[OC];
+#pragma unroll
+      for (int c = 0; c < OC; ++c) {
+        const float4 d = *reinterpret_cast<const float4 *>(&ring_y[c * R + rd]);
+        o[c] = make_float4(d.x * g.x, d.y * g.y, d.z * g.z, d.w * g.w);
+      }
+      uint8_t *dst = pcm + j0 * (OC * bytes);
+      if (p.out_format == IAMF_HIP_FMT_S16) {
+        int v[OC][4];
+#pragma unroll
+        for (int c = 0; c < OC; ++c) {
+          v[c][0] = (int)to_scaled(o[c].x, 32768.f, -32768.f, 32767.f);
+          v[c][1] = (int)to_scaled(o[c].y, 32768.f, -32768.f, 32767.f);
+          v[c][2] = (int)to_scaled(o[c].z, 32768.f, -32768.f, 32767.f);
+          v[c][3] = (int)to_scaled(o[c].w, 32768.f, -32768.f, 32767.f);
+        }
+        if (OC == 2) {
+          uint4 w;
+          w.x = (uint32_t)(v[0][0] & 0xffff) | ((uint32_t)v[OC - 1][0] << 16);
+          w.y = (uint32_t)(v[0][1] & 0xffff) | ((uint32_t)v[OC - 1][1] << 16);
+          w.z = (uint32_t)(v[0][2] & 0xffff) | ((uint32_t)v[OC - 1][2] << 16);
+          w.w = (uint32_t)(v[0][3] & 0xffff) | ((uint32_t)v[OC - 1][3] << 16);
+          *reinterpret_cast<uint4 *>(dst) = w;
+        } else {
+          uint2 w;
+          w.x = (uint32_t)(v[0][0] & 0xffff) | ((uint32_t)v[0][1] << 16);
+          w.y = (uint32_t)(v[0][2] & 0xffff) | ((uint32_t)v[0][3] << 16);
+          *reinterpret_cast<uint2 *>(dst) = w;
+        }
+      } else if (p.out_format == IAMF_HIP_FMT_S24) {
+#pragma unroll
+        for (int c = 0; c < OC; ++c) {
+          const float ov[4] = {o[c].x, o[c].y, o[c].z, o[c].w};
+#pragma unroll
+          for (int j = 0; j < 4; ++j) {
+            const int vv = (int)to_scaled(ov[j], 8388608.f, -8388608.f, 8388607.f);
+            uint8_t *d3 = dst + (j * OC + c) * 3;
+            d3[0] = (uint8_t)(vv & 0xff);
+            d3[1] = (uint8_t)((vv >> 8) & 0xff);
+            d3[2] = (uint8_t)(((vv >> 16) & 0x7f) | ((vv >> 24) & 0x80));
+          }
+        }
+      } else if (p.out_format == IAMF_HIP_FMT_S32) {
+        int32_t *d32 = reinterpret_cast<int32_t *>(dst);
+#pragma unroll
+        for (int c = 0; c < OC; ++c) {
+          const float ov[4] = {o[c].x, o[c].y, o[c].z, o[c].w};
+#pragma unroll
+          for (int j = 0; j < 4; ++j)
+            d32[j * OC + c] = (int32_t)(long long)to_scaled(ov[j], 2147483648.f, -2147483648.f, 2147483647.f);
+        }
+      } else {
+        float *df = reinterpret_cast<float *>(dst);
+#pragma unroll
+        for (int c = 0; c < OC; ++c) {
+          df[0 * OC + c] = o[c].x;
+          df[1 * OC + c] = o[c].y;
+          df[2 * OC + c] = o[c].z;
+          df[3 * OC + c] = o[c].w;
+        }
+      }
+    }
+    base = (base + ccnt) & (R - 1);
+    lw_sync();
+  }
+
+  {
+    float *sy = p.ring_y + (int64_t)s * OC * kSave;
+    float *spm = p.ring_pm + (int64_t)s * kSave;
+    int te = 4 * t;
+    asm volatile("" : "+v"(te));
+    const int rp = (base - kSave + te) & (R - 1);
+#pragma unroll
+    for (int c = 0; c < OC; ++c) *reinterpret_cast<float4 *>(&sy[c * kSave + te]) = *reinterpret_cast<const float4 *>(&ring_y[c * R + rp]);
+    *reinterpret_cast<float4 *>(&spm[te]) = *reinterpret_cast<const float4 *>(&ring_pm[rp]);
+    if (t == 0) {
+      LimState o;
+      o.g = g_cur;
+      o.gs = gs;
+      o.ge = ge;
+      o.n = n_st;
+      p.lim[s] = o;
+    }
+  }
+}
+
+template <int OC>
+void launch_limiter_wave(const RenderParams &p, int off, int cnt, hipStream_t st) {
+  hipLaunchKernelGGL(limiter2_wave_kernel<OC>, dim3((unsigned)p.n_launch), dim3(64),
+                     sizeof(float) * (size_t)limiter_wave_lds_floats(OC), st, p, off, cnt);
+}
diff --git a/iac_amd/csrc/render_route.hpp b/iac_amd/csrc/render_route.hpp
--- a/iac_amd/csrc/render_route.hpp
+++ b/iac_amd/csrc/render_route.hpp
@@ -61,6 +61,25 @@
   if (p.fir_pq && p.fir_tw && p.fir_zero && (p.frame_size & 63) == 0)
     return (p.fir_y && p.fir_id_matrix && !getenv("IAMF_HIP_FIR_FUSED")) ? 4 : 3;
   return p.fir_h16 ? 2 : 1;
+}
+
+constexpr int kFirSlices = 4;
+constexpr int kFirMinSlicePasses = 2;
+constexpr int kFirMaxSlices = 8;
+inline int fir_slice_passes(const RenderParams &p, int span) {
+  if (getenv("IAMF_HIP_FIR_SERIAL")) return 0;
+  const int passes = (p.total + span - 1) / span;
+  int sp = (passes + kFirSlices - 1) / kFirSlices;
+  if (sp < kFirMinSlicePasses) sp = kFirMinSlicePasses;
+  if (const char *e = getenv("IAMF_HIP_FIR_SLICE_FRAMES")) {
+    const long n = atol(e);
+    if (n <= 0) return 0;
+    const int64_t want = (n * (int64_t)p.frame_size + span - 1) / span;
+    sp = want < passes ? (int)want : passes;
+  }
+  const int least = (passes + kFirMaxSlices - 1) / kFirMaxSlices;
+  if (sp < least) sp = least;
+  return passes > sp ? sp : 0;
 }
 
 
diff --git a/iac_amd/hipabi.py b/iac_amd/hipabi.py
--- a/iac_amd/hipabi.py
+++ b/iac_amd/hipabi.py
@@ -208,6 +208,9 @@
         L.iamf_hip_route_tally.argtypes = [C.POINTER(RouteRow), C.c_int, C.c_int]
         L.iamf_hip_route_instances_ext.argtypes = [C.POINTER(RouteRow), C.c_int]
         L.iamf_hip_route_tally_ext.argtypes = [C.POINTER(RouteRow), C.c_int, C.c_int]
+        if hasattr(L, "iamf_hip_limiter_wave_launches"):
+            L.iamf_hip_limiter_wave_launches.argtypes = [C.c_int]
+            L.iamf_hip_limiter_wave_launches.restype = C.c_int64
         L.iamf_hip_shard_split.argtypes = [C.c_int, C.c_int, C.c_int, C.POINTER(C.c_int), C.POINTER(C.c_int)]
         L.iamf_hip_shard_create.argtypes = [C.POINTER(BatchConfig), C.POINTER(C.c_int), C.c_int, C.POINTER(C.c_void_p)]
         L.iamf_hip_shard_destroy.argtypes = [C.c_void_p]
@@ -310,6 +313,10 @@
     return {(ROUTE_NAME[r.family], r.variant, r.m, r.c, r.k): r.launches for r in rows[:min(n, cap)]}
 
 
+def limiter_wave_launches(reset=True):
+    return int(lib().iamf_hip_limiter_wave_launches(1 if reset else 0))
+
+
 FANOUT_MAX = 4
 
 
diff --git a/include/iamf_hip.h b/include/iamf_hip.h
--- a/include/iamf_hip.h
+++ b/include/iamf_hip.h
@@ -327,6 +327,7 @@
 int iamf_hip_route_tally(iamf_hip_route_row *rows, int cap, int reset);
 int iamf_hip_route_instances_ext(iamf_hip_route_row *rows, int cap);
 int iamf_hip_route_tally_ext(iamf_hip_route_row *rows, int cap, int reset);
+int64_t iamf_hip_limiter_wave_launches(int reset);
 
 typedef struct iamf_hip_decoder_group iamf_hip_decoder_group;
 int iamf_hip_decoder_group_create(void *const *handles, int n, int host_threads, iamf_hip_decoder_group **out);
```
